# DTUWindEnergy/WindGym

Hardware: AMD Instinct MI355X
Metric: env-steps/sec (whole node), 16-turbine farm x 4096 envs (higher is better)
Workload: dtype f32

## Files before the change

### windgym_amd/build.py

```python
from __future__ import annotations

import glob
import os
import subprocess

HERE = os.path.dirname(os.path.abspath(__file__))
CSRC = os.path.join(HERE, "csrc")
LIB = os.path.join(HERE, "libwindgym_hip.so")
SOURCES = ["wg_flow.hip", "wg_env.hip", "wg_envb.hip", "wg_kernels.hip", "wg_api.hip", "wg_mann.hip", "wg_steady.hip", "wg_policy.hip", "wg_ppo.hip"]


def _headers():
    hs = sorted(glob.glob(os.path.join(CSRC, "*.h")) + glob.glob(os.path.join(CSRC, "*.inc")))
    return hs + [os.path.join(HERE, "..", "include", "windgym_hip.h")]


def needs_build() -> bool:
    if not os.path.exists(LIB):
        return True
    t = os.path.getmtime(LIB)
    return any(os.path.getmtime(f) > t for f in [os.path.join(CSRC, f) for f in SOURCES] + _headers())


def build(force: bool = False, verbose: bool = False, out: str | None = None) -> str:
    if out is None:
        if not force and not needs_build():
            return LIB
        out = LIB
    import tempfile
    hipcc = os.environ.get("HIPCC", "/opt/rocm/bin/hipcc")
    extra = os.environ.get("WG_HIPCC_FLAGS", "").split()
    flags = ["--offload-arch=gfx950", "-O3", "-std=c++17", "-fPIC"] + extra + ["-Wno-unused-result", "-Wno-unused-value"]
    if verbose:
        flags.insert(0, "-Rpass-analysis=kernel-resource-usage")
    with tempfile.TemporaryDirectory(prefix="wg_build_") as tmp:
        objs, procs = [], []
        for src in SOURCES:
            obj = os.path.join(tmp, src.replace(".hip", ".o"))
            cmd = [hipcc] + flags + ["-c", os.path.join(CSRC, src), "-o", obj]
            if verbose:
                print(" ".join(cmd))
            procs.append((cmd, subprocess.Popen(cmd)))
            objs.append(obj)
        for cmd, pr in procs:
            if pr.wait() != 0:
                for _, other in procs:
                    if other.poll() is None:
                        other.kill()
                raise subprocess.CalledProcessError(pr.returncode, cmd)
        subprocess.run([hipcc, "--offload-arch=gfx950", "-shared", "-fPIC", "-o", out] + objs + ["-lhipfft"], check=True)
    return out


if __name__ == "__main__":
    import argparse
    ap = argparse.ArgumentParser(description=__doc__)
    ap.add_argument("-v", action="store_true", help="print the compile commands and every kernel's resource usage")
    ap.add_argument("--out", metavar="PATH", help="write a variant library to PATH instead of the in-tree one")
    args = ap.parse_args()
    print(build(force=True, verbose=args.v, out=args.out))
```

### windgym_amd/csrc/wg_api.hip

```cpp
#include <hip/hip_runtime.h>

#include <algorithm>
#include <cmath>
#include <cstdio>
#include <cstdlib>
#include <cstring>
#include <memory>
#include <mutex>
#include <string>
#include <vector>

#include "wg_plan.h"
#include "wg_steady.h"
#include "wg_policy.h"
#include "wg_internal.h"

static const char* wg_hook(const char* name) {
    static const bool on = [] { const char* v = getenv("WG_DEBUG_HOOKS"); return v && v[0] == '1' && v[1] == 0; }();
    if (!on) return nullptr;
    const char* v = getenv(name);
    if (v) {
        static std::string seen;
        static std::mutex seen_mu;
        std::lock_guard<std::mutex> lock(seen_mu);
        const std::string tag = std::string(name) + "=" + v + ";";
        if (seen.find(tag) == std::string::npos) {
            seen += tag;
            fprintf(stderr, "[windgym] WG_DEBUG_HOOKS: %s=%s\n", name, v);
        }
    }
    return v;
}
static WgHooks wg_hooks_read() {
    WgHooks k;
    const auto num = [](const char* name) { WgHookInt r; if (const char* v = wg_hook(name)) { r.set = true; r.v = atoi(v); } return r; };
    k.flow_block = num("WG_FLOW_BLOCK"); k.flow_res = num("WG_FLOW_RES"); k.flow_env = num("WG_FLOW_ENV");
    k.env_wpe = num("WG_ENV_WPE"); k.env_split = num("WG_ENV_SPLIT"); k.step_fused = num("WG_STEP_FUSED");
    k.sums = num("WG_SUMS"); k.lds_pad = num("WG_LDS_PAD"); k.lf_cap = num("WG_LF_CAP"); k.pstride_pad = num("WG_PSTRIDE_PAD");
    k.step_graph = num("WG_STEP_GRAPH");
    k.first_obs_gl_only = wg_hook("WG_FIRST_OBS_GL_ONLY") != nullptr;
    k.no_box8 = wg_hook("WG_NO_BOX8") != nullptr;
    k.debug = wg_hook("WG_DEBUG") != nullptr;
    if (const char* v = wg_hook("WG_TIMELINE_OUT")) { k.timeline = true; k.timeline_out = v; }
    return k;
}

static thread_local std::string g_err;
static int fail(int code, const std::string& msg) {
    g_err = msg;
    return code;
}
extern "C" int wg_set_last_error_(int code, const char* msg) { return fail(code, msg ? msg : ""); }
#define HIPCHK(x)                                                                                   \
    do {                                                                                            \
        hipError_t _e = (x);                                                                        \
        if (_e != hipSuccess)                                                                       \
            return fail(WG_ERR_HIP, std::string(#x) + ": " + hipGetErrorString(_e));                \
    } while (0)

struct Alloc {
    void* ptr;
    size_t bytes;
};

struct wg_env_s {
    WgPlan plan;
    WgHooks hooks;
    WgParams p;
    WgPtrs d;
    FlowP fp;
    FlowPtrs fd;
    unsigned long long flow_steps_mark = 0, particles_mark = 0, added_mark = 0;
    double added_per_launch = 0.0;
    long n_step_launches = 0;
    void* box4 = nullptr;
    void* box4c = nullptr;
    int* box_ids_dev = nullptr;
    void* abox4 = nullptr;
    void* box8 = nullptr;
    void* abox8 = nullptr;
    double* wind_dev = nullptr;
    int device;
    std::vector<Alloc> allocs;
    std::vector<size_t> state_idx;
    uint8_t* mask_dev = nullptr;
    uint64_t* seeds_dev = nullptr;
    bool timing = false;
    int timing_period = 1, timing_phase = 0;
    std::vector<hipEvent_t> ev;
    std::vector<int> ev_kind;
    size_t ev_used = 0;
    struct StepGraph {
        const void* key[5];
        hipGraph_t graph;
        hipGraphExec_t exec;
        unsigned long long last_use;
    };
    std::vector<StepGraph> graphs;
    hipStream_t cap_stream = nullptr;
    int graph_mode = 0;
    unsigned long long graph_clock = 0;
    int* unready_dev = nullptr;
    WgParams* p_dev = nullptr;
    WgPtrs* d_dev = nullptr;
    float* flat_scratch = nullptr;
};

static const size_t WG_MAX_STEP_GRAPHS = 32;
static const size_t WG_MAX_TIMING_EVENTS = 4096;

static void drop_step_graphs(wg_env_s* h) {
    if (!h->graphs.empty()) { hipSetDevice(h->device); hipDeviceSynchronize(); }
    for (auto& g : h->graphs) {
        hipGraphExecDestroy(g.exec);
        hipGraphDestroy(g.graph);
    }
    h->graphs.clear();
}

static int sync_dev_params(wg_env_s* h) {
    hipError_t e = hipMemcpy(h->p_dev, &h->p, sizeof(WgParams), hipMemcpyHostToDevice);
    if (e == hipSuccess) e = hipMemcpy(h->d_dev, &h->d, sizeof(WgPtrs), hipMemcpyHostToDevice);
    if (e != hipSuccess) return fail(WG_ERR_HIP, std::string("hipMemcpy(params): ") + hipGetErrorString(e));
    return 0;
}

static int use_device(wg_env_s* h) {
    int cur = -1;
    if (hipGetDevice(&cur) != hipSuccess || cur != h->device) {
        hipError_t e = hipSetDevice(h->device);
        if (e != hipSuccess) return fail(WG_ERR_HIP, std::string("hipSetDevice: ") + hipGetErrorString(e));
    }
    return 0;
}

template <typename T>
static int dev_alloc(wg_env_s* h, T** out, size_t n, bool state, bool zero = true) {
    size_t bytes = sizeof(T) * (n ? n : 1);
    void* ptr = nullptr;
    hipError_t e = hipMalloc(&ptr, bytes);
    if (e != hipSuccess) return fail(WG_ERR_NOMEM, std::string("hipMalloc: ") + hipGetErrorString(e));
    if (zero) {
        e = hipMemset(ptr, 0, bytes);
        if (e != hipSuccess) return fail(WG_ERR_HIP, std::string("hipMemset: ") + hipGetErrorString(e));
    }
    h->allocs.push_back({ptr, bytes});
    if (state) h->state_idx.push_back(h->allocs.size() - 1);
    *out = (T*)ptr;
    return 0;
}
template <typename T, typename S>
static int dev_upload(wg_env_s* h, const T** out, const S* src, size_t n) {
    std::vector<T> tmp(n ? n : 1);
    for (size_t i = 0; i < n; ++i) tmp[i] = (T)src[i];
    T* p = nullptr;
    int rc = dev_alloc(h, &p, n, false, false);
    if (rc) return rc;
    HIPCHK(hipMemcpy(p, tmp.data(), sizeof(T) * (n ? n : 1), hipMemcpyHostToDevice));
    *out = p;
    return 0;
}

extern "C" const char* wg_last_error(void) { return g_err.c_str(); }
extern "C" int wg_abi_version(void) { return WG_ABI_VERSION; }

struct HandleGuard {
    void operator()(wg_env_s* h) const { wg_destroy(h); }
};

static int create_alloc(wg_env_s* h) {
    const WgParams& p = h->p;
    WgPtrs& d = h->d;
    const size_t n_slots = (size_t)p.B * 2 * p.F, n_ctx = (size_t)p.B * 2, pstride = (size_t)h->fp.pstride;
    int rc = 0;
#define A(field, n, st) if (!rc) rc = dev_alloc(h, &d.field, (n), (st))
    A(py, n_slots * pstride, true);
    if (p.turb_mode != WG_TURB_NONE) {
        A(pz, n_slots * pstride, true); A(vlp, n_slots * pstride, true); A(wlp, n_slots * pstride, true);
    }
    A(yaw, n_slots * p.N, true); A(u, n_slots * p.N, true); A(v, n_slots * p.N, true); A(w, n_slots * p.N, true);
    A(ti_loc, n_slots * p.N, true); A(power, n_slots * p.N, true); A(ct, n_slots * p.N, true);
    A(bnd, n_slots * p.N * 4, true);
    A(slot, n_slots, true); A(ctx, n_ctx, true); A(env, (size_t)p.B, true);
    A(xr, n_ctx * p.N, true); A(yr, n_ctx * p.N, true); A(jneed, n_ctx * p.N, true);
    A(roff, n_ctx * (p.N + 1), true); A(qown, n_ctx * (size_t)(p.NP / 4), true);
    A(ring, n_ctx * p.ring_stride, true); A(fring, n_ctx * p.fring_stride, true);
    A(cur_ws, n_ctx * p.N, true); A(cur_wd, n_ctx * p.N, true);
    A(pend_farm, n_ctx * p.power_avg, true); A(pend_base, n_ctx * p.power_avg, true);
    A(farm_pow, (size_t)p.B * p.power_avg, true); A(base_pow, (size_t)p.B * p.power_avg, true);
    A(old_yaw, (size_t)p.B * p.N, true);
    A(step_farm_pow, (size_t)p.B, true); A(step_base_pow, (size_t)p.B, true);
    A(last_pow_agent, (size_t)p.B, true); A(last_pow_base, (size_t)p.B, true);
    A(metrics, (size_t)p.B * WG_N_METRICS, true);
    if (h->plan.first_obs) { A(next_obs, n_ctx * (size_t)p.obs_dim, false); A(next_obs_ok, n_ctx, false); }
    if (p.sums_mode) A(wsum, n_ctx * WG_N_SUMS * (size_t)(p.N + 1), true);
    A(status, 1, true);
#undef A
    if (!rc) rc = dev_alloc(h, &h->mask_dev, (size_t)p.B, false);
    if (!rc) rc = dev_alloc(h, &h->seeds_dev, (size_t)p.B, false);
    if (!rc) rc = dev_alloc(h, &h->unready_dev, 1, false);
    if (!rc) rc = dev_alloc(h, &h->p_dev, 1, false);
    if (!rc) rc = dev_alloc(h, &h->d_dev, 1, false);
    return rc;
}

static int create_alloc_record(wg_env_s* h) {
    const size_t n = (size_t)h->p.B * 2 * h->p.F * (size_t)h->fp.pstride;
    if (h->fp.rec_il) {
        if (int rc = dev_alloc(h, &h->d.rec_a, 2 * n, true)) return rc;
        h->d.rec_b = h->d.rec_a + 1;
        return 0;
    }
    if (int rc = dev_alloc(h, &h->d.rec_a, n, true)) return rc;
    return dev_alloc(h, &h->d.rec_b, n, true);
}

static int create_upload(wg_env_s* h, const wg_config* c) {
    const WgParams& p = h->p;
    WgPtrs& d = h->d;
    int rc = dev_upload<double>(h, &d.x_pos, c->x_pos, p.N);
    if (!rc) rc = dev_upload<double>(h, &d.y_pos, c->y_pos, p.N);
    if (!rc && c->yaw_defined) rc = dev_upload<double>(h, &d.yaw_defined, c->yaw_defined, p.N);
    if (!rc) {
        const int kmax = std::max(p.N, 3);
        std::vector<uint64_t> jump((size_t)(kmax + 1) * 4);
        wg_u128 A = 1, G = 0;
        for (int k = 0; k <= kmax; ++k) {
            jump[4 * (size_t)k] = (uint64_t)A; jump[4 * (size_t)k + 1] = (uint64_t)(A >> 64);
            jump[4 * (size_t)k + 2] = (uint64_t)G; jump[4 * (size_t)k + 3] = (uint64_t)(G >> 64);
            A = A * WG_PCG_MULT; G = G * WG_PCG_MULT + 1;
        }
        rc = dev_upload<uint64_t>(h, &d.pcg_jump, jump.data(), jump.size());
    }
    if (!rc) rc = dev_upload<float>(h, &d.rotor_dy, c->rotor_dy, p.S);
    if (!rc) rc = dev_upload<float>(h, &d.rotor_dz, c->rotor_dz, p.S);
    if (!rc) rc = dev_upload<float>(h, &d.tab_ws, c->tab_ws, p.n_tab);
    if (!rc) rc = dev_upload<float>(h, &d.tab_power, c->tab_power, p.n_tab);
    if (!rc) rc = dev_upload<float>(h, &d.tab_ct, c->tab_ct, p.n_tab);
    if (!rc) rc = dev_upload<double>(h, &d.tab_ws_d, c->tab_ws, p.n_tab);
    if (!rc) rc = dev_upload<double>(h, &d.tab_power_d, c->tab_power, p.n_tab);
    if (rc) return rc;
    std::vector<float> pu, cu;
    double x0 = 0, dx = 0;
    wg_uniform_table(c, &pu, &cu, &x0, &dx);
    rc = dev_upload<float>(h, &h->fd.tab_power, pu.data(), pu.size());
    if (!rc) rc = dev_upload<float>(h, &h->fd.tab_ct, cu.data(), cu.size());
    return rc;
}

static void create_flow_ptrs(wg_env_s* h) {
    const WgPtrs& d = h->d;
    FlowPtrs& g = h->fd;
    g.py = d.py; g.rec_a = d.rec_a; g.rec_b = d.rec_b;
    g.pz = d.pz; g.vlp = d.vlp; g.wlp = d.wlp;
    g.bnd = d.bnd;
    g.yaw = d.yaw; g.u = d.u; g.v = d.v; g.w = d.w; g.ti_loc = d.ti_loc; g.power = d.power; g.ct = d.ct;
    g.slot = d.slot; g.ctx = d.ctx; g.env = d.env; g.xr = d.xr; g.yr = d.yr; g.jneed = d.jneed;
    g.ring = d.ring; g.fring = d.fring; g.cur_ws = d.cur_ws; g.cur_wd = d.cur_wd;
    g.pend_farm = d.pend_farm; g.pend_base = d.pend_base; g.old_yaw = d.old_yaw;
    g.step_farm_pow = d.step_farm_pow; g.step_base_pow = d.step_base_pow;
    g.rotor_dy = d.rotor_dy; g.rotor_dz = d.rotor_dz;
    g.gp = h->p_dev; g.gd = h->d_dev; g.env_rw = d.env;
    g.roff = d.roff; g.qown = d.qown; g.status = d.status;
}

static void apply_step_path(wg_env_s* h) {
    wg_plan_step_path(h->plan, h->fp.box_cells, (long long)h->fp.anx * h->fp.any * h->fp.anz, &h->fp.envw, &h->fp.env_fused);
}

extern "C" int wg_create(const wg_config* c, int device, wg_handle* out) {
    if (!c || !out) return fail(WG_ERR_INVALID, "null argument");
    std::string err;
    if (int rc = wg_validate_config(c, &err)) return fail(rc, err);
    HIPCHK(hipSetDevice(device));
    int lds_limit = 65536;
    {
        int v = 0;
        if (hipDeviceGetAttribute(&v, hipDeviceAttributeMaxSharedMemoryPerBlock, device) == hipSuccess && v > 0)
            lds_limit = std::min(v, 65536);
    }
    std::unique_ptr<wg_env_s, HandleGuard> owner(new wg_env_s());
    wg_env_s* h = owner.get();
    h->device = device;
    h->hooks = wg_hooks_read();
    if (int rc = wg_plan_create(c, h->hooks, lds_limit, &h->plan, &err)) return fail(rc, err);
    h->p = h->plan.p;
    h->fp = h->plan.f;
    apply_step_path(h);

    if (int rc = create_alloc(h)) return rc;
    if (int rc = create_upload(h, c)) return rc;
    if (int rc = create_alloc_record(h)) return rc;
    create_flow_ptrs(h);
    if (h->hooks.timeline) {
        long long* dbgp = nullptr;
        if (!dev_alloc(h, &dbgp, (size_t)h->p.B * 2 * h->p.F * 16, false)) h->fd.dbg = dbgp;
    }
    wg_launch_create(&h->p, &h->d, nullptr);
    if (sync_dev_params(h)) return WG_ERR_HIP;
    {
        hipError_t e = hipDeviceSynchronize();
        if (e == hipSuccess) e = hipStreamCreateWithFlags(&h->cap_stream, hipStreamNonBlocking);
        if (e != hipSuccess) return fail(WG_ERR_HIP, std::string("wg_create: ") + hipGetErrorString(e));
    }
    if (h->hooks.step_graph.set) h->graph_mode = h->hooks.step_graph.v != 0;
    if (h->hooks.debug) {
        const FlowP& f = h->fp;
        fprintf(stderr, "[windgym] k_flow variant: %s%s, %d threads, LDS %d B per workgroup, slot stride %d floats\n",
                f.envw ? (f.turb_mode == WG_TURB_NONE ? "compact rings / pair-major, one wave per env (k_flow_env)" : "compact rings / sample-major, one wave per env (k_flow_envb)")
                       : (f.res ? "compact rings / pair-major" : "uniform rings / sample-major"),
                f.envw && f.env_split ? " + a pass wave for the running episode's context" : "",
                f.block, f.envw ? f.env_lds : f.lds_bytes, f.pstride);
        fprintf(stderr, "[windgym] plan: res %d block %d gl %d rec_il %d target_chunk %d lf_cap %d lds_bytes %d | envw %d env_wpe %d env_split %d env_fused %d "
                        "env_lds %d env_off_tab %d | sums_mode %d first_obs %d reset_launches %d\n",
                f.res, f.block, f.gl, f.rec_il, f.target_chunk, f.lf_cap, f.lds_bytes, f.envw, f.env_wpe, f.env_split, f.env_fused, f.env_lds,
                f.env_off_tab, h->p.sums_mode, h->plan.first_obs, h->plan.reset_launches);
    }
    *out = owner.release();
    return 0;
}

extern "C" int wg_destroy(wg_handle h) {
    if (!h) return 0;
    hipSetDevice(h->device);
    hipDeviceSynchronize();
    if (h->fd.dbg && h->hooks.timeline) {
        const size_t n = (size_t)h->p.B * 2 * h->p.F * 16;
        std::vector<long long> host(n);
        if (hipMemcpy(host.data(), h->fd.dbg, n * sizeof(long long), hipMemcpyDeviceToHost) == hipSuccess) {
            if (FILE* f = fopen(h->hooks.timeline_out.c_str(), "wb")) { fwrite(host.data(), sizeof(long long), n, f); fclose(f); }
        }
    }
    drop_step_graphs(h);
    if (h->cap_stream) hipStreamDestroy(h->cap_stream);
    for (auto& e : h->ev) hipEventDestroy(e);
    for (auto& a : h->allocs) hipFree(a.ptr);
    if (h->box4) hipFree(h->box4);
    if (h->box4c) hipFree(h->box4c);
    if (h->abox4) hipFree(h->abox4);
    if (h->box8) hipFree(h->box8);
    if (h->abox8) hipFree(h->abox8);
    delete h;
    return 0;
}

extern "C" int wg_obs_dim(wg_handle h, int* obs_dim, int* obs_dim_multi) {
    if (!h) return fail(WG_ERR_INVALID, "null handle");
    if (obs_dim) *obs_dim = h->p.obs_dim;
    if (obs_dim_multi) *obs_dim_multi = h->p.obs_dim_multi;
    return 0;
}
extern "C" int wg_hist_max(wg_handle h, int* hist_max) {
    if (!h || !hist_max) return fail(WG_ERR_INVALID, "null argument");
    *hist_max = h->p.hist_max;
    return 0;
}

static int build_stencil_records(wg_env_s* h, void** owned, const float4** kernel_ptr, const void* box4, int n_boxes, int nx, int ny, int nz) {
    *kernel_ptr = nullptr;
    if (!(h->fp.envw && h->fp.turb_mode != WG_TURB_NONE)) return 0;
    const auto skip = [h](const char* why) {
        if (h->hooks.debug) fprintf(stderr, "[windgym] stencil records not built (%s): k_flow_envb reads the brick-ordered box\n", why);
        return 0;
    };
    if (wg_hooks_read().no_box8) return skip("WG_NO_BOX8");
    const size_t n_cells = (size_t)nx * ny * nz, bytes = n_cells * 128 * (size_t)n_boxes;
    size_t free_b = 0, total_b = 0;
    if (hipMemGetInfo(&free_b, &total_b) != hipSuccess) return skip("hipMemGetInfo failed");
    if (n_cells >= ((size_t)1 << 28)) return skip("a box of 2^28 cells or more");
    if (bytes > total_b / 4 || bytes > free_b / 2) return skip("the pool's records exceed a quarter of the device memory or half of what is free");
    if (hipMalloc(owned, bytes) != hipSuccess) { *owned = nullptr; (void)hipGetLastError(); return skip("hipMalloc failed"); }
    for (int k = 0; k < n_boxes; ++k)
        wg_launch_box_stencil((const char*)box4 + (size_t)k * n_cells * 16, (char*)*owned + (size_t)k * n_cells * 128, nx, ny, nz, nullptr);
    HIPCHK(hipDeviceSynchronize());
    *kernel_ptr = (const float4*)*owned;
    return 0;
}

extern "C" int wg_set_turbulence_boxes(wg_handle h, const float* const* boxes_dev, int n_boxes, int nx, int ny, int nz,
                                       double dx, double dy, double dz) {
    if (!h) return fail(WG_ERR_INVALID, "null handle");
    if (!boxes_dev || n_boxes < 1 || n_boxes > 64 || nx < 2 || ny < 2 || nz < 2 || !(dx > 0) || !(dy > 0) || !(dz > 0))
        return fail(WG_ERR_INVALID, "turbulence box: null pointer, bad pool size (1..64) or bad dimensions");
    for (int k = 0; k < n_boxes; ++k)
        if (!boxes_dev[k]) return fail(WG_ERR_INVALID, "turbulence box: null pointer in the pool");
    HIPCHK(hipSetDevice(h->device));
    HIPCHK(hipDeviceSynchronize());
    drop_step_graphs(h);
    h->d.box = nullptr; h->fd.box4 = nullptr; h->fd.box4c = nullptr; h->fd.box8 = nullptr; h->fp.coarse = 0;
    if (h->box8) { void* q = h->box8; h->box8 = nullptr; HIPCHK(hipFree(q)); }
    if (h->box4) { void* q = h->box4; h->box4 = nullptr; HIPCHK(hipFree(q)); }
    if (h->box4c) { void* q = h->box4c; h->box4c = nullptr; HIPCHK(hipFree(q)); }
    const size_t n_cells = (size_t)nx * ny * nz;
    HIPCHK(hipMalloc(&h->box4, n_cells * 16 * (size_t)n_boxes));
    for (int k = 0; k < n_boxes; ++k)
        wg_launch_box_repack(boxes_dev[k], (char*)h->box4 + (size_t)k * n_cells * 16, nx, ny, nz, nullptr);
    HIPCHK(hipDeviceSynchronize());
    h->d.box = boxes_dev[0];
    h->p.n_boxes = n_boxes;
    h->p.bnx = nx; h->p.bny = ny; h->p.bnz = nz; h->p.bdx = dx; h->p.bdy = dy; h->p.bdz = dz;
    h->fd.box4 = (const float4*)h->box4;
    h->fp.bnx = nx; h->fp.bny = ny; h->fp.bnz = nz; h->fp.box_cells = (long long)n_cells;
    apply_step_path(h);
    h->fp.box_pow2 = ((nx & (nx - 1)) == 0) && ((ny & (ny - 1)) == 0) && ((nz & (nz - 1)) == 0);
    h->fp.coarse = (nx % 4 == 0 && ny % 4 == 0 && nz % 4 == 0 && nx >= 8 && ny >= 8 && nz >= 8);
    h->fd.box4c = nullptr;
    if (h->fp.coarse) {
        const int cx = nx / 4, cy = ny / 4, cz = nz / 4;
        const size_t c_cells = (size_t)cx * cy * cz;
        HIPCHK(hipMalloc(&h->box4c, c_cells * 16 * (size_t)n_boxes));
        for (int k = 0; k < n_boxes; ++k)
            wg_launch_box_coarsen((const char*)h->box4 + (size_t)k * n_cells * 16, (char*)h->box4c + (size_t)k * c_cells * 16,
                                  nx, ny, nz, nullptr);
        HIPCHK(hipDeviceSynchronize());
        h->fp.cnx = cx; h->fp.cny = cy; h->fp.cnz = cz; h->fp.cbox_cells = (long long)c_cells;
        h->fp.cbox_pow2 = ((cx & (cx - 1)) == 0) && ((cy & (cy - 1)) == 0) && ((cz & (cz - 1)) == 0);
        h->fd.box4c = (const float4*)h->box4c;
    }
    h->fp.inv_bdx = 1.0 / dx; h->fp.inv_bdy = 1.0 / dy; h->fp.inv_bdz = 1.0 / dz;
    h->fp.inv_bn[0] = 1.0 / nx; h->fp.inv_bn[1] = 1.0 / ny; h->fp.inv_bn[2] = 1.0 / nz;
    if (int rc = build_stencil_records(h, &h->box8, &h->fd.box8, h->box4, n_boxes, nx, ny, nz)) return rc;
    return sync_dev_params(h);
}

extern "C" int wg_set_added_turbulence_box(wg_handle h, const float* box_dev, int nx, int ny, int nz, double dx,
                                           double dy, double dz) {
    if (!h || !box_dev || nx < 2 || ny < 2 || nz < 2 || !(dx > 0) || !(dy > 0) || !(dz > 0))
        return fail(WG_ERR_INVALID, "added-turbulence box: null pointer or bad dimensions");
    HIPCHK(hipSetDevice(h->device));
    HIPCHK(hipDeviceSynchronize());
    drop_step_graphs(h);
    h->fd.abox4 = nullptr; h->fd.abox8 = nullptr;
    if (h->abox8) { void* q = h->abox8; h->abox8 = nullptr; HIPCHK(hipFree(q)); }
    if (h->abox4) { void* q = h->abox4; h->abox4 = nullptr; HIPCHK(hipFree(q)); }
    const size_t n_cells = (size_t)nx * ny * nz;
    HIPCHK(hipMalloc(&h->abox4, n_cells * 16));
    wg_launch_box_repack(box_dev, h->abox4, nx, ny, nz, nullptr);
    HIPCHK(hipDeviceSynchronize());
    h->fd.abox4 = (const float4*)h->abox4;
    h->fp.anx = nx; h->fp.any = ny; h->fp.anz = nz;
    apply_step_path(h);
    h->fp.abox_pow2 = ((nx & (nx - 1)) == 0) && ((ny & (ny - 1)) == 0) && ((nz & (nz - 1)) == 0);
    h->fp.inv_adx = 1.0 / dx; h->fp.inv_ady = 1.0 / dy; h->fp.inv_adz = 1.0 / dz;
    h->fp.inv_an[0] = 1.0 / nx; h->fp.inv_an[1] = 1.0 / ny; h->fp.inv_an[2] = 1.0 / nz;
    if (int rc = build_stencil_records(h, &h->abox8, &h->fd.abox8, h->abox4, 1, nx, ny, nz)) return rc;
    return 0;
}

extern "C" int wg_set_deficit_table(wg_handle h, const float* table_dev, int n_ct, double ct0, double ct1, int n_ti, double ti0,
                                    double ti1, int n_x, double x_max_D, int n_r, double r_max_R) {
    if (!h || !table_dev || n_ct < 2 || n_ti < 2 || n_x < 2 || n_r < 2 || !(ct1 > ct0) || !(ti0 > 0) || !(ti1 > ti0) || !(x_max_D > 0) ||
        !(r_max_R > 0))
        return fail(WG_ERR_INVALID, "wg_set_deficit_table: null pointer or bad grid");
    if ((long long)n_ct * n_ti * n_x * n_r >= (1ll << 30)) return fail(WG_ERR_INVALID, "wg_set_deficit_table: table too large");
    HIPCHK(hipSetDevice(h->device));
    HIPCHK(hipDeviceSynchronize());
    drop_step_graphs(h);
    FlowP& f = h->fp;
    h->fd.dtab = table_dev;
    f.an_ct = n_ct; f.an_ti = n_ti; f.an_x = n_x; f.an_r = n_r;
    f.an_ct0 = (float)ct0; f.an_inv_dct = (float)((n_ct - 1) / (ct1 - ct0));
    f.an_lti0 = (float)std::log(ti0); f.an_inv_dlti = (float)((n_ti - 1) / (std::log(ti1) - std::log(ti0)));
    f.an_inv_dx = (float)((n_x - 1) / x_max_D); f.an_inv_dr = (float)((n_r - 1) / r_max_R);
    return 0;
}

extern "C" int wg_set_turbulence_box(wg_handle h, const float* box_dev, int nx, int ny, int nz, double dx,
                                     double dy, double dz) {
    const float* one[1] = {box_dev};
    if (!box_dev) return fail(WG_ERR_INVALID, "turbulence box: null pointer or bad dimensions");
    return wg_set_turbulence_boxes(h, one, 1, nx, ny, nz, dx, dy, dz);
}

extern "C" int wg_set_wind(wg_handle h, const double* wind_host) {
    if (!h) return fail(WG_ERR_INVALID, "null handle");
    HIPCHK(hipSetDevice(h->device));
    HIPCHK(hipDeviceSynchronize());
    drop_step_graphs(h);
    if (!wind_host) { h->d.wind_override = nullptr; return sync_dev_params(h); }
    if (!h->wind_dev) {
        double* w = nullptr;
        int rc = dev_alloc(h, &w, (size_t)h->p.B * 3, false);
        if (rc) return rc;
        h->wind_dev = w;
    }
    HIPCHK(hipMemcpy(h->wind_dev, wind_host, sizeof(double) * 3 * (size_t)h->p.B, hipMemcpyHostToDevice));
    h->d.wind_override = h->wind_dev;
    return sync_dev_params(h);
}

extern "C" int wg_set_box_ids(wg_handle h, const int32_t* ids_host) {
    if (!h) return fail(WG_ERR_INVALID, "null handle");
    HIPCHK(hipSetDevice(h->device));
    HIPCHK(hipDeviceSynchronize());
    drop_step_graphs(h);
    if (!ids_host) { h->d.box_override = nullptr; return sync_dev_params(h); }
    if (h->p.turb_mode != WG_TURB_BOX_POOL || h->p.n_boxes < 1)
        return fail(WG_ERR_INVALID, "wg_set_box_ids: the handle has no box pool (turb_mode WG_TURB_BOX_POOL + wg_set_turbulence_boxes first)");
    for (int b = 0; b < h->p.B; ++b)
        if (ids_host[b] >= h->p.n_boxes)
            return fail(WG_ERR_INVALID, "wg_set_box_ids: env " + std::to_string(b) + " asks for box " + std::to_string(ids_host[b]) +
                                            " of a pool of " + std::to_string(h->p.n_boxes));
    if (!h->box_ids_dev) {
        int* w = nullptr;
        int rc = dev_alloc(h, &w, (size_t)h->p.B, false);
        if (rc) return rc;
        h->box_ids_dev = w;
    }
    HIPCHK(hipMemcpy(h->box_ids_dev, ids_host, sizeof(int) * (size_t)h->p.B, hipMemcpyHostToDevice));
    h->d.box_override = h->box_ids_dev;
    return sync_dev_params(h);
}

extern "C" int wg_set_wind_device(wg_handle h, const double* wind_dev) {
    if (!h) return fail(WG_ERR_INVALID, "null handle");
    if (h->d.wind_override != wind_dev) drop_step_graphs(h);
    h->d.wind_override = wind_dev;
    if (int rc = use_device(h)) return rc;
    return sync_dev_params(h);
}

extern "C" int wg_set_flow_script(wg_handle h, const float* uvw_dev, const float* power_dev, int n_rows) {
    if (!h) return fail(WG_ERR_INVALID, "null handle");
    drop_step_graphs(h);
    h->d.script_uvw = uvw_dev;
    h->d.script_power = power_dev;
    h->p.script_rows = n_rows;
    h->fd.script_uvw = uvw_dev;
    h->fd.script_power = power_dev;
    h->fp.script_rows = n_rows;
    if (int rc = use_device(h)) return rc;
    return sync_dev_params(h);
}

static bool time_begin(wg_env_s* h, int kind, hipStream_t st) {
    if (!h->timing || h->ev_used + 2 > h->ev.size()) return false;
    h->ev_kind[h->ev_used / 2] = kind;
    hipEventRecord(h->ev[h->ev_used], st);
    return true;
}
static void time_end(wg_env_s* h, hipStream_t st) {
    hipEventRecord(h->ev[h->ev_used + 1], st);
    h->ev_used += 2;
}

extern "C" int wg_reset(wg_handle h, const uint8_t* env_mask_host, const uint64_t* seeds_host, float* obs_dev,
                        void* stream) {
    if (!h) return fail(WG_ERR_INVALID, "null handle");
    hipStream_t st = (hipStream_t)stream;
    HIPCHK(hipSetDevice(h->device));
    if (h->p.turb_mode >= WG_TURB_BOX && !h->d.box)
        return fail(WG_ERR_INVALID, "turbtype Mann*: call wg_set_turbulence_box before wg_reset");
    if (h->fp.added && !h->fd.abox4)
        return fail(WG_ERR_INVALID, "added_turbulence: call wg_set_added_turbulence_box before wg_reset");
    if (h->fp.deficit_model == 2 && !h->fd.dtab)
        return fail(WG_ERR_INVALID, "deficit_model 2: call wg_set_deficit_table before wg_reset");
    const uint8_t* mask = nullptr;
    const uint64_t* seeds = nullptr;
    bool all = true;
    if (env_mask_host) {
        for (int b = 0; b < h->p.B; ++b) all = all && env_mask_host[b] != 0;
        HIPCHK(hipMemcpyAsync(h->mask_dev, env_mask_host, (size_t)h->p.B, hipMemcpyHostToDevice, st));
        mask = h->mask_dev;
    }
    if (seeds_host) {
        HIPCHK(hipMemcpyAsync(h->seeds_dev, seeds_host, sizeof(uint64_t) * (size_t)h->p.B, hipMemcpyHostToDevice, st));
        seeds = h->seeds_dev;
    }
    if (all) HIPCHK(hipMemsetAsync(h->d.status, 0, sizeof(int), st));
    wg_launch_init(&h->p, &h->d, mask, seeds, st);
    const int n_plan = h->d.script_uvw ? ((h->p.K * (std::max(h->p.fill_a, h->p.fill_b) + 1)) / h->plan.reset_chunk + 2)
                                       : h->plan.reset_launches;
    long launched = 0;
    int batch = n_plan;
    for (;;) {
        for (int i = 0; i < batch; ++i) wg_launch_flow(&h->fp, &h->fd, WG_MODE_RESET, nullptr, mask, h->plan.reset_chunk, st);
        {
            const hipError_t le = hipGetLastError();
            if (le != hipSuccess) return fail(WG_ERR_HIP, std::string("wg_reset: k_flow launch failed: ") + hipGetErrorString(le));
        }
        launched += batch;
        int unready = 0;
        HIPCHK(hipMemsetAsync(h->unready_dev, 0, sizeof(int), st));
        wg_launch_unready(&h->p, &h->d, mask, h->unready_dev, st);
        HIPCHK(hipMemcpyAsync(&unready, h->unready_dev, sizeof(int), hipMemcpyDeviceToHost, st));
        HIPCHK(hipStreamSynchronize(st));
        if (unready == 0) break;
        if (launched > 4000000L / h->plan.reset_chunk)
            return fail(WG_ERR_STATE, "wg_reset: episode development does not terminate (wind speed override ~ 0?)");
        batch = std::max(8, n_plan / 4);
    }
    wg_launch_glue(&h->p, &h->d, 1, mask, obs_dev, nullptr, nullptr, nullptr, st, h->p_dev, h->d_dev);
    HIPCHK(hipGetLastError());
    return 0;
}

static bool count_step(wg_env_s* h) {
    h->n_step_launches++;
    return h->timing && (h->timing_phase++ % h->timing_period == 0);
}

static void launch_step(wg_env_s* h, const float* actions_dev, float* obs_dev, float* reward_dev, uint8_t* truncated_dev,
                        float* final_obs_dev, hipStream_t st, bool sample) {
    if (h->fp.env_fused && h->fd.script_uvw == nullptr) {
        if (sample) sample = time_begin(h, 0, st);
        if (h->fp.turb_mode == WG_TURB_NONE) wg_launch_step_env(&h->fp, &h->fd, &h->p, &h->d, actions_dev, obs_dev, reward_dev, truncated_dev, final_obs_dev, st);
        else wg_launch_step_envb(&h->fp, &h->fd, &h->p, &h->d, actions_dev, obs_dev, reward_dev, truncated_dev, final_obs_dev, st);
        if (sample) time_end(h, st);
        return;
    }
    if (sample) sample = time_begin(h, 0, st);
    wg_launch_flow(&h->fp, &h->fd, WG_MODE_STEP, actions_dev, nullptr, 0, st);
    if (sample) { time_end(h, st); sample = time_begin(h, 1, st); }
    wg_launch_glue(&h->p, &h->d, 0, nullptr, obs_dev, reward_dev, truncated_dev, final_obs_dev, st, h->p_dev, h->d_dev);
    if (sample) time_end(h, st);
}

extern "C" int wg_step(wg_handle h, const float* actions_dev, float* obs_dev, float* reward_dev,
// ... 448 lines not shown
```

### windgym_amd/csrc/wg_device.h

```cpp
#pragma once
#include <hip/hip_runtime.h>

#include "wg_state.h"

#define WG_PI_D 3.14159265358979323846
#define WG_DEG2RAD_F 0.017453292519943295f
#define WG_RAD2DEG_F 57.29577951308232f


__device__ inline uint32_t wg_ss_hashmix(uint32_t value, uint32_t& hc) {
    value ^= hc;
    hc *= 0x931e8875u;
    value *= hc;
    value ^= value >> 16;
    return value;
}
__device__ inline uint32_t wg_ss_mix(uint32_t x, uint32_t y) {
    uint32_t r = 0xca01f9ddu * x - 0x4973f715u * y;
    r ^= r >> 16;
    return r;
}
template <class R>
__device__ inline void wg_pcg_seed(R& e, uint64_t seed) {
    uint32_t ent[2] = {(uint32_t)(seed & 0xffffffffu), (uint32_t)(seed >> 32)};
    int n_ent = ent[1] != 0 ? 2 : 1;
    uint32_t pool[4];
    uint32_t hc = 0x43b0d7e5u;
    for (int i = 0; i < 4; ++i) pool[i] = wg_ss_hashmix(i < n_ent ? ent[i] : 0u, hc);
    for (int s = 0; s < 4; ++s)
        for (int dd = 0; dd < 4; ++dd)
            if (s != dd) pool[dd] = wg_ss_mix(pool[dd], wg_ss_hashmix(pool[s], hc));
    uint32_t hb = 0x8b51f9ddu;
    uint64_t st[4];
    for (int i = 0; i < 4; ++i) {
        uint32_t w2[2];
        for (int h = 0; h < 2; ++h) {
            uint32_t v = pool[(2 * i + h) & 3];
            v ^= hb;
            hb *= 0x58f38dedu;
            v *= hb;
            v ^= v >> 16;
            w2[h] = v;
        }
        st[i] = (uint64_t)w2[0] | ((uint64_t)w2[1] << 32);
    }
    wg_u128 initstate = ((wg_u128)st[0] << 64) | st[1];
    wg_u128 initseq = ((wg_u128)st[2] << 64) | st[3];
    e.rng_inc = (initseq << 1) | 1;
    e.rng_state = (wg_u128)0 * WG_PCG_MULT + e.rng_inc;
    e.rng_state += initstate;
    e.rng_state = e.rng_state * WG_PCG_MULT + e.rng_inc;
    e.rng_has32 = 0;
    e.rng_u32 = 0;
}
template <class R>
__device__ inline uint64_t wg_pcg_next64(R& e) {
    e.rng_state = e.rng_state * WG_PCG_MULT + e.rng_inc;
    uint64_t hi = (uint64_t)(e.rng_state >> 64), lo = (uint64_t)e.rng_state;
    uint64_t x = hi ^ lo;
    unsigned rot = (unsigned)(e.rng_state >> 122);
    return (x >> rot) | (x << ((-rot) & 63));
}
template <class R>
__device__ inline uint32_t wg_pcg_next32(R& e) {
    if (e.rng_has32) {
        e.rng_has32 = 0;
        return e.rng_u32;
    }
    uint64_t n = wg_pcg_next64(e);
    e.rng_has32 = 1;
    e.rng_u32 = (uint32_t)(n >> 32);
    return (uint32_t)(n & 0xffffffffu);
}
template <class R>
__device__ inline double wg_pcg_uniform(R& e, double low, double high) {
#pragma clang fp contract(off)
    const double u = (double)(wg_pcg_next64(e) >> 11) * (1.0 / 9007199254740992.0);
    const double scaled = (high - low) * u;
    return low + scaled;
}
template <class R>
__device__ inline uint32_t wg_pcg_integers(R& e, uint32_t high) {
    uint32_t rng = high - 1;
    if (rng == 0) return 0;
    uint32_t rng_excl = rng + 1;
    uint64_t m = (uint64_t)wg_pcg_next32(e) * (uint64_t)rng_excl;
    uint32_t leftover = (uint32_t)m;
    if (leftover < rng_excl) {
        uint32_t threshold = (0xffffffffu - rng) % rng_excl;
        while (leftover < threshold) {
            m = (uint64_t)wg_pcg_next32(e) * (uint64_t)rng_excl;
            leftover = (uint32_t)m;
        }
    }
    return (uint32_t)(m >> 32);
}

__device__ inline float wg_noise_normal(uint64_t key, uint32_t push_idx, uint32_t turbine, uint32_t channel,
                                        uint32_t episode) {
    uint32_t c0 = push_idx, c1 = turbine, c2 = channel, c3 = episode;
    uint32_t k0 = (uint32_t)key, k1 = (uint32_t)(key >> 32);
#pragma unroll
    for (int r = 0; r < 10; ++r) {
        uint64_t p0 = (uint64_t)0xD2511F53u * c0;
        uint64_t p1 = (uint64_t)0xCD9E8D57u * c2;
        uint32_t n0 = (uint32_t)(p1 >> 32) ^ c1 ^ k0;
        uint32_t n1 = (uint32_t)p1;
        uint32_t n2 = (uint32_t)(p0 >> 32) ^ c3 ^ k1;
        uint32_t n3 = (uint32_t)p0;
        c0 = n0; c1 = n1; c2 = n2; c3 = n3;
        k0 += 0x9E3779B9u;
        k1 += 0xBB67AE85u;
    }
    const float u1 = ((float)(c0 >> 8) + 1.0f) * (1.0f / 16777216.0f);
    const float u2 = (float)(c1 >> 8) * (1.0f / 16777216.0f);
    return sqrtf(-2.0f * __logf(u1)) * __cosf(6.2831853071795864f * u2);
}

__device__ inline void wg_philox_turb(uint32_t turb_seed, uint32_t c0, uint32_t c1, uint32_t c2, uint32_t c3,
                                      uint32_t& o0, uint32_t& o1) {
    uint32_t k0 = turb_seed, k1 = 0x57474d30u;
#pragma unroll
    for (int r = 0; r < 10; ++r) {
        uint64_t p0 = (uint64_t)0xD2511F53u * c0;
        uint64_t p1 = (uint64_t)0xCD9E8D57u * c2;
        uint32_t n0 = (uint32_t)(p1 >> 32) ^ c1 ^ k0;
        uint32_t n1 = (uint32_t)p1;
        uint32_t n2 = (uint32_t)(p0 >> 32) ^ c3 ^ k1;
        uint32_t n3 = (uint32_t)p0;
        c0 = n0; c1 = n1; c2 = n2; c3 = n3;
        k0 += 0x9E3779B9u;
        k1 += 0xBB67AE85u;
    }
    o0 = c0; o1 = c1;
}
__device__ inline float wg_turb_normal(uint32_t turb_seed, uint32_t step, uint32_t index, uint32_t comp, uint32_t kind) {
    uint32_t a, b;
    wg_philox_turb(turb_seed, step, index, comp, kind, a, b);
    const float u1 = ((float)(a >> 8) + 1.0f) * (1.0f / 16777216.0f);
    const float u2 = (float)(b >> 8) * (1.0f / 16777216.0f);
    return sqrtf(-2.0f * __logf(u1)) * __cosf(6.2831853071795864f * u2);
}

template <typename T>
__device__ inline T wg_tab_interp(const T* xs, const T* ys, int n, T x) {
    if (!(x >= xs[0]) || x > xs[n - 1]) return (T)0;
    int lo = 0, hi = n - 1;
    while (hi - lo > 1) {
        int mid = (lo + hi) >> 1;
        if (xs[mid] <= x) lo = mid; else hi = mid;
    }
    T f = (x - xs[lo]) / (xs[hi] - xs[lo]);
    return ys[lo] + f * (ys[hi] - ys[lo]);
}

template <class T>
__device__ inline T wg_tab_interp_wave(const T* xs, const T* ys, int n, T x, int lane) {
    int cnt = 0;
    for (int i0 = 0; i0 < n - 1; i0 += 64) {
        const int i = i0 + lane;
        const bool le = (i < n - 1) && (xs[i] <= x);
        cnt += __popcll(__ballot(le));
    }
    if (!(x >= xs[0]) || x > xs[n - 1]) return (T)0;
    const int lo = cnt - 1, hi = lo + 1;
    const T f = (x - xs[lo]) / (xs[hi] - xs[lo]);
    return ys[lo] + f * (ys[hi] - ys[lo]);
}

template <int CTRL>
__device__ __forceinline__ float wg_dpp_f(float v) {
    return __int_as_float(__builtin_amdgcn_update_dpp(0, __float_as_int(v), CTRL, 0xf, 0xf, true));
}
#define WG_ROW_REDUCE(v, OP)                                                 \
    v = OP(v, wg_dpp_f<0xB1>(v));                 \
    v = OP(v, wg_dpp_f<0x4E>(v));                 \
    v = OP(v, wg_dpp_f<0x141>(v));                    \
    v = OP(v, wg_dpp_f<0x140>(v));
__device__ __forceinline__ float wg_addf(float a, float b) { return a + b; }
__device__ inline float wg_row_sum(float v) {
    WG_ROW_REDUCE(v, wg_addf)
    return v;
}
__device__ inline float wg_wave_sum(float v) {
    WG_ROW_REDUCE(v, wg_addf)
    v += __shfl_xor(v, 16, 64);
    v += __shfl_xor(v, 32, 64);
    return v;
}
__device__ inline int wg_wave_sum_i(int v) {
#pragma unroll
    for (int o = 32; o > 0; o >>= 1) v += __shfl_xor(v, o, 64);
    return v;
}
template <int CTRL, int ROW_MASK>
__device__ __forceinline__ int wg_dpp_i(int v) {
    return __builtin_amdgcn_update_dpp(0, v, CTRL, ROW_MASK, 0xf, true);
}
__device__ __forceinline__ int wg_wave_scan_i(int v) {
    v += wg_dpp_i<0x111, 0xf>(v);
    v += wg_dpp_i<0x112, 0xf>(v);
    v += wg_dpp_i<0x114, 0xf>(v);
    v += wg_dpp_i<0x118, 0xf>(v);
    v += wg_dpp_i<0x142, 0xa>(v);
    v += wg_dpp_i<0x143, 0xc>(v);
    return v;
}
__device__ inline float wg_wave_max(float v) {
#pragma unroll
    for (int o = 32; o > 0; o >>= 1) v = fmaxf(v, __shfl_xor(v, o, 64));
    return v;
}
__device__ inline double wg_wave_min_d(double v) {
#pragma unroll
    for (int o = 32; o > 0; o >>= 1) v = fmin(v, __shfl_xor(v, o, 64));
    return v;
}
__device__ inline double wg_wave_max_d(double v) {
#pragma unroll
    for (int o = 32; o > 0; o >>= 1) v = fmax(v, __shfl_xor(v, o, 64));
    return v;
}

struct WgRng {
    wg_u128 rng_state, rng_inc;
    uint32_t rng_has32, rng_u32;
};

#ifdef WG_TIMELINE
__shared__ long long wg_stamps[20];
__shared__ int wg_counts[8];
#define WG_STAMP(k) do { if (threadIdx.x == 0) wg_stamps[k] = clock64(); } while (0)
#define WG_STAMP2(k) WG_STAMP(k)
#define WG_ICLK0() long long wg_iclk_ = clock64()
#define WG_ICLK(i) do { if (threadIdx.x == 0) { const long long c_ = clock64(); wg_counts[i] = (int)(c_ - wg_iclk_); wg_iclk_ = c_; } } while (0)
#else
#define WG_STAMP(k) do { } while (0)
#define WG_ICLK0() do { } while (0)
#define WG_ICLK(i) do { } while (0)
#endif

#ifndef WG_SHADOW_MARGIN
#define WG_SHADOW_MARGIN 2
#endif
__device__ inline int wg_shadow_share(const int work, long left, const int steps_done, const int e, const uint32_t phase = 0u) {
    if (work <= 0) return 0;
    left -= WG_SHADOW_MARGIN;
    if (left < 1) left = 1;
    const uint32_t phi24 = ((uint32_t)steps_done * 2654435769u + (uint32_t)e * 0x9E3779B1u + phase) >> 8;
    const float share = (float)work * __builtin_amdgcn_rcpf((float)left) + (float)phi24 * (1.0f / 16777216.0f);
    int it = (int)share;
    if (left == 1) it = work;
    return it > work ? work : it;
}

__device__ inline double wg_tab_interp_lanes(const double xs_l, const double ys_l, const int n, const double x, const int lane) {
    const int cnt = __popcll(__ballot((lane < n - 1) && (xs_l <= x)));
    const double x_first = __shfl(xs_l, 0, 64), x_last = __shfl(xs_l, n - 1, 64);
    const int lo = cnt > 0 ? cnt - 1 : 0, hi = lo + 1;
    const double xl = __shfl(xs_l, lo, 64), xh = __shfl(xs_l, hi, 64), yl = __shfl(ys_l, lo, 64), yh = __shfl(ys_l, hi, 64);
    if (!(x >= x_first) || x > x_last) return 0.0;
    const double f = (x - xl) / (xh - xl);
    return yl + f * (yh - yl);
}

template <class P, class D, class R>
__device__ inline void wg_ctx_init(const P& __restrict__ p, const D& __restrict__ d, R& rng, const int e, const int c, const int lane,
                                   const int episode_tag, const int f_lo, const int f_hi) {
    const int N = p.N, F = p.F;
    const int ctx_id = e * 2 + c;
    WgCtx& cx = d.ctx[ctx_id];
    WG_ICLK0();
    const int tl = lane < N ? lane : 0;
    const double xp_l = d.x_pos[tl], yp_l = d.y_pos[tl];
    const int n_tab = p.n_tab;
    const int il = lane < n_tab ? lane : n_tab - 1;
    const double tws_l = d.tab_ws_d[il], tpw_l = d.tab_power_d[il];
    const uint64_t* const jmp = d.pcg_jump;
    const int kmax = N > 3 ? N : 3;
    uint64_t jl[4], jn[4], j3[4];
    {
        const int kl = lane <= kmax ? lane : 0;
#pragma unroll
        for (int i = 0; i < 4; ++i) { jl[i] = jmp[4 * (size_t)kl + i]; jn[i] = jmp[4 * (size_t)N + i]; j3[i] = jmp[4 * (size_t)3 + i]; }
    }
    const bool yaw_rnd = p.yaw_init == WG_YAWINIT_RANDOM, yaw_def = p.yaw_init == WG_YAWINIT_DEFINED && p.has_yaw_defined;
    const double ydef_l = yaw_def ? d.yaw_defined[tl] : 0.0;
    double ov[3] = {0.0, 0.0, 0.0};
    const bool has_ov = d.wind_override != nullptr;
    if (has_ov) { ov[0] = d.wind_override[(size_t)e * 3]; ov[1] = d.wind_override[(size_t)e * 3 + 1]; ov[2] = d.wind_override[(size_t)e * 3 + 2]; }

    const wg_u128 inc = rng.rng_inc;
    auto ahead = [&](const uint64_t* j, const wg_u128 s) {
        const wg_u128 A = ((wg_u128)j[1] << 64) | j[0], G = ((wg_u128)j[3] << 64) | j[2];
        return A * s + G * inc;
    };
    auto draw = [&](const wg_u128 s, const double lo, const double hi) {
        struct { wg_u128 rng_state, rng_inc; } one{s, inc};
        return wg_pcg_uniform(one, lo, hi);
    };
    double ws, ti, wd;
    {
        const wg_u128 s_l = rng.rng_state;
        uint32_t iw[4] = {(uint32_t)s_l, (uint32_t)(s_l >> 32), (uint32_t)(s_l >> 64), (uint32_t)(s_l >> 96)};
#pragma unroll
        for (int i = 0; i < 4; ++i) iw[i] = (uint32_t)__shfl((int)iw[i], 0, 64);
        const wg_u128 s_in = ((wg_u128)iw[3] << 96) | ((wg_u128)iw[2] << 64) | ((wg_u128)iw[1] << 32) | (wg_u128)iw[0];
        const double lo = lane == 0 ? p.ws_min : lane == 1 ? p.ti_min : p.wd_min;
        const double hi = lane == 0 ? p.ws_max : lane == 1 ? p.ti_max : p.wd_max;
        const double u = draw(ahead(jl, s_in), lo, hi);
        ws = __shfl(u, 0, 64); ti = __shfl(u, 1, 64); wd = __shfl(u, 2, 64);
        if (lane == 0) rng.rng_state = ahead(j3, s_in);
    }
    if (has_ov) {
        if (ov[0] == ov[0]) ws = ov[0];
        if (ov[1] == ov[1]) wd = ov[1];
        if (ov[2] == ov[2]) ti = ov[2];
    }
    wg_u128 s_head = 0;
    if (lane == 0) {
        uint32_t tseed = 0;
        if (p.turb_mode == WG_TURB_RANDOM || p.turb_mode == WG_TURB_BOX_SHIFT)
            tseed = wg_pcg_integers(rng, 100000);
        cx.box_ox = 0.0; cx.box_oy = 0.0; cx.box_id = 0;
        if (p.turb_mode == WG_TURB_BOX_POOL) {
            const int fixed = d.box_override ? d.box_override[e] : -1;
            if (fixed >= 0) cx.box_id = fixed < p.n_boxes ? fixed : 0;
            else cx.box_id = (int)wg_pcg_integers(rng, (uint32_t)(p.n_boxes > 0 ? p.n_boxes : 1));
        }
        if (p.turb_mode == WG_TURB_BOX_SHIFT && p.bnx > 0) {
            if (p.n_boxes > 1) cx.box_id = (int)(tseed % (uint32_t)p.n_boxes);
            uint32_t a, b;
            wg_philox_turb(tseed, 0u, 0u, 0u, 0x4fu, a, b);
            cx.box_ox = (double)a * (1.0 / 4294967296.0) * p.bnx * p.bdx;
            cx.box_oy = (double)b * (1.0 / 4294967296.0) * p.bny * p.bdy;
        }
        s_head = rng.rng_state;
        cx.ws = ws; cx.ti = ti; cx.wd = wd; cx.turb_seed = tseed;
        if (f_lo == 0) { cx.n_pushed = 0; cx.pend_farm_n = 0; }
        if (f_hi == F) cx.pend_base_n = 0;
        cx.episode_tag = episode_tag;
    }
    {
        uint32_t sw[4] = {(uint32_t)s_head, (uint32_t)(s_head >> 32), (uint32_t)(s_head >> 64), (uint32_t)(s_head >> 96)};
#pragma unroll
        for (int i = 0; i < 4; ++i) sw[i] = (uint32_t)__shfl((int)sw[i], 0, 64);
        const wg_u128 s0 = ((wg_u128)sw[3] << 96) | ((wg_u128)sw[2] << 64) | ((wg_u128)sw[1] << 32) | (wg_u128)sw[0];
        const double ys = p.yaw_start;
        float* const yaw_c = d.yaw + (size_t)ctx_id * F * N;
        for (int t = lane; t < N; t += WG_WAVE) {
            float y0 = 0.f;
            if (yaw_rnd) {
                uint64_t jt[4];
                if (t < WG_WAVE) { jt[0] = jl[0]; jt[1] = jl[1]; jt[2] = jl[2]; jt[3] = jl[3]; }
                else { for (int i = 0; i < 4; ++i) jt[i] = jmp[4 * (size_t)t + i]; }
                y0 = (float)draw(ahead(jt, s0), -ys, ys);
            } else if (yaw_def) y0 = (float)(t < WG_WAVE ? ydef_l : d.yaw_defined[t]);
            for (int f = f_lo; f < f_hi; ++f) yaw_c[(size_t)f * N + t] = y0;
        }
        if (yaw_rnd && lane == 0) rng.rng_state = ahead(jn, s0);
    }
    WG_ICLK(5);
    {
        const double rp = n_tab <= WG_WAVE ? wg_tab_interp_lanes(tws_l, tpw_l, n_tab, ws, lane)
                                            : wg_tab_interp_wave<double>(d.tab_ws_d, d.tab_power_d, n_tab, ws, lane);
        if (lane == 0) cx.rated_power = (float)rp;
    }
    const double th = (270.0 - wd) * (WG_PI_D / 180.0);
    const double cth = cos(th), sth = sin(th);
    const double cx0 = p.cx0, cy0 = p.cy0;
    double* const xr_c = d.xr + (size_t)ctx_id * N;
    double* const yr_c = d.yr + (size_t)ctx_id * N;
    double xmin = 1e300, xmax = -1e300;
    for (int t = lane; t < N; t += WG_WAVE) {
        const double dx = (t < WG_WAVE ? xp_l : d.x_pos[t]) - cx0, dy = (t < WG_WAVE ? yp_l : d.y_pos[t]) - cy0;
        const double xr = cx0 + dx * cth + dy * sth;
        const double yr = cy0 - dx * sth + dy * cth;
        xr_c[t] = xr;
        yr_c[t] = yr;
        xmin = fmin(xmin, xr); xmax = fmax(xmax, xr);
    }
    xmin = wg_wave_min_d(xmin); xmax = wg_wave_max_d(xmax);
    const int P_ = p.P, full_chains = p.full_chains, compact = p.compact;
    const double dpart = p.dpart;
    int* const jneed_c = d.jneed + (size_t)ctx_id * N;
    int* const ro = d.roff + (size_t)ctx_id * (N + 1);
    uint8_t* const own = d.qown + (size_t)ctx_id * (p.NP >> 2);
    int base = 0;
    for (int t0 = 0; t0 < N; t0 += WG_WAVE) {
        const int t = t0 + lane;
        int len = 0;
        if (t < N) {
            const double dx = (t < WG_WAVE ? xp_l : d.x_pos[t]) - cx0, dy = (t < WG_WAVE ? yp_l : d.y_pos[t]) - cy0;
            const double dxm = xmax - (cx0 + dx * cth + dy * sth);
            const int jn_ = full_chains ? P_ : (int)(dxm / dpart) + 2;
            jneed_c[t] = jn_;
            len = (jn_ + 1 + 3) & ~3;
            if (len > P_) len = P_;
        }
        if (compact) {
            int incl = len;
#pragma unroll
            for (int o = 1; o < WG_WAVE; o <<= 1) {
                const int v = __shfl_up(incl, o, 64);
                if (lane >= o) incl += v;
            }
            if (t < N) {
                ro[t] = base + incl - len;
                const int q0 = (base + incl - len) >> 2, q1 = (base + incl) >> 2;
                for (int q = q0; q < q1; ++q) own[q] = (uint8_t)t;
            }
            base += __shfl(incl, WG_WAVE - 1, 64);
        }
    }
    if (compact && lane == 0) ro[N] = base;
    WG_ICLK(6);
    const bool scripted = d.script_uvw != nullptr;
    if (lane == 0) {
        cx.dist = xmax - xmin;
        const double t_inflow = (xmax - xmin) / ws;
        cx.t_inflow = t_inflow;
        const int t_developed = (int)(t_inflow * 2);
        cx.t_developed = t_developed;
        cx.time_max = p.never_truncate ? 9999999 : (int)(t_inflow * p.n_passthrough);
        int n_dev = (int)ceil((double)t_developed / p.dt_d - 1e-9);
        if (scripted) n_dev = 0;
        for (int f = f_lo; f < f_hi; ++f) {
            WgSlot& s = d.slot[ctx_id * F + f];
            s.head = P_ - 1; s.n_valid = 0; s.s_off = 0.0; s.time = 0.0; s.istep = 0; s.n_emitted = 0;
            s.dev_remaining = n_dev;
            s.fill_remaining = f == 0 ? p.fill_a : p.fill_b;
        }
    }
    for (int f = f_lo; f < f_hi; ++f) {
        const size_t tb = (size_t)(ctx_id * F + f) * N;
        const int cursor = scripted ? d.slot[ctx_id * F + f].cursor : 0;
        float* const u_ = d.u + tb; float* const v_ = d.v + tb; float* const w_ = d.w + tb;
        float* const ti_ = d.ti_loc + tb; float* const pw_ = d.power + tb; float* const ct_ = d.ct + tb;
        float4* const bnd_ = reinterpret_cast<float4*>(d.bnd) + tb;
        for (int t = lane; t < N; t += WG_WAVE) {
            float u = (float)ws, v = 0.f, w = 0.f, pw = 0.f;
            if (scripted) {
                int row = cursor < p.script_rows ? cursor : p.script_rows - 1;
                size_t sbase = (((size_t)f * p.script_rows + row) * p.B + e) * N;
                u = d.script_uvw[(sbase + t) * 3]; v = d.script_uvw[(sbase + t) * 3 + 1];
                w = d.script_uvw[(sbase + t) * 3 + 2]; pw = d.script_power[sbase + t];
            }
            u_[t] = u; v_[t] = v; w_[t] = w;
            ti_[t] = (float)ti; pw_[t] = pw; ct_[t] = 0.f;
            bnd_[t] = make_float4(0.f, 0.f, 0.f, 0.f);
        }
    }
    WG_ICLK(7);
}

struct WgRing {
    const float* data;
    int n_pushed, hlen;
    int n_avail, start;
    int stride, cap;
    __device__ WgRing() {}
    __device__ WgRing(const float* d_, int n_pushed_, int hlen_, int stride_, int cap_)
        : data(d_), n_pushed(n_pushed_), hlen(hlen_), stride(stride_), cap(cap_) {
        n_avail = n_pushed < hlen ? n_pushed : hlen;
        start = (n_pushed - n_avail) % cap;
    }
    __device__ int avail() const { return n_avail; }
    __device__ float at(int q) const {
        int phys = start + q;
        if (phys >= cap) phys -= cap;
        return data[phys * stride];
    }
};

__device__ inline float wg_ring_sum(const WgRing& r, const int lo, const int hi) {
    float s = 0.f;
    for (int q = lo; q < hi; q += 8) {
        float v[8];
#pragma unroll
        for (int k = 0; k < 8; ++k) v[k] = r.at(min(q + k, hi - 1));
#pragma unroll
        for (int k = 0; k < 8; ++k)
            if (q + k < hi) s += v[k];
    }
    return s;
}

__device__ inline float wg_scale(float v, float mn, float rng) {
    float t = v - mn;
    t = 2.0f * t;
    t = t / rng;
    return t - 1.0f;
}

__device__ inline int wg_mes_get(const wg_channel& c, bool cur_on, bool rol_on, const WgRing& r, float mn,
                                 float rng, float* out) {
    int n = 0;
    const int avail = r.avail();
    if (avail == 0) return 0;
    if (cur_on) out[n++] = wg_scale(r.at(avail - 1), mn, rng);
    if (rol_on) {
        const int W = c.window_len;
        for (int i = 0; i < c.history_n; ++i) {
            int lo, hi;
            if (i == 0) {
                lo = avail - W; if (lo < 0) lo = 0; hi = avail;
            } else if (i == c.history_n - 1 && avail >= W) {
                lo = 0; hi = W;
            } else if (avail < W) {
                lo = 0; hi = avail;
            } else {
                int spacing = (avail - W) / (c.history_n - 1);
                if (spacing < 1) spacing = 1;
                int pos = i * spacing;
                if (pos > avail - W) pos = avail - W;
                lo = pos; hi = pos + W;
            }
            const float s = wg_ring_sum(r, lo, hi);
            out[n++] = wg_scale(s / (float)(hi - lo), mn, rng);
        }
    }
    return n;
}

__device__ inline float wg_calc_ti(const WgRing& r) {
    const int avail = r.avail();
    float U = wg_ring_sum(r, 0, avail);
    U /= (float)avail;
    float m2 = 0.f;
    for (int q = 0; q < avail; q += 8) {
        float v[8];
#pragma unroll
        for (int k = 0; k < 8; ++k) v[k] = r.at(min(q + k, avail - 1));
#pragma unroll
        for (int k = 0; k < 8; ++k)
            if (q + k < avail) { const float dv = v[k] - U; m2 += dv * dv; }
    }
    return sqrtf(m2 / (float)avail) / U;
// ... 38 lines not shown
```

### windgym_amd/csrc/wg_env.hip

```cpp
#include <hip/hip_runtime.h>

#ifndef WG_ENV_ABLATE
#define WG_ENV_ABLATE 0
#endif
#include "wg_env_common.h"
#include "wg_internal.h"

struct __attribute__((aligned(16))) EnvSlotLds {
    int dev_rem, fill_rem, sub, budget;
    double s_new;
    int n_emit, n_valid, new_valid;
    unsigned n_emitted;
    float s_off_f, near_f, move_max, ti_pow;
    double s_off, ws;
    float ws_f, ti_f, wd_env, base_acc;
    int n_pushed, pend_farm_n, pend_base_n, n_flow;
    double c_time;
    int c_head;
    unsigned c_part, c_flow, c_istep, c_tag, n_emitted0;
    float out_pw;
    unsigned c_add;
    int bg_init;
    int pad_[3];
};
static_assert(sizeof(EnvSlotLds) == WG_ENV_SLOT_LDS_BYTES, "keep WG_ENV_SLOT_LDS_BYTES in sync (wg_flow.h)");
#define WG_ENV_OFF_SRC4 0
#define WG_ENV_OFF_REC4 1024
#define WG_ENV_OFF_RING 2048
#define WG_ENV_OFF_XR 3072
#define WG_ENV_OFF_SRC2 3584
#define WG_ENV_OFF_SL 4096
#define WG_ENV_OFF_HDR (WG_ENV_OFF_SL + 4 * WG_ENV_SLOT_LDS_BYTES)
#define WG_ENV_OFF_STAGE (WG_ENV_OFF_HDR + 128)
static_assert(WG_ENV_OFF_STAGE == WG_ENV_FIXED_LDS_BYTES, "keep WG_ENV_FIXED_LDS_BYTES in sync (wg_flow.h)");

__device__ __forceinline__ float env_slot_sums(const float v, const int N, const int NS, const int k, const int tid) {
    if (N == 16) return wg_row_sum(v);
    if (N < 16) {
        const int r = tid >> 4, i = tid & 15;
        const float x = __shfl(v, (r * N + i) & 63, 64);
        const float s = wg_row_sum((i < N && r < NS) ? x : 0.f);
        return __shfl(s, k << 4, 64);
    }
    const int h = tid >> 5, i = tid & 31;
    const float x = __shfl(v, (h * N + i) & 63, 64);
    float s = (i < N && h < NS) ? x : 0.f;
    WG_ROW_REDUCE(s, wg_addf)
    s += __shfl_xor(s, 16, 64);
    return __shfl(s, k << 5, 64);
}

template <bool NOISE, int WPE, int GLUE, int SPLIT>
__device__ __forceinline__ void env_flow(char* const smem, char* const smem_pass, float* const zone, const int wv, const int role, const int mode,
                                         const float* __restrict__ actions, const uint8_t* __restrict__ mask, const int chunk, EnvFlowOut& out) {
    const int tid = threadIdx.x & 63, e = blockIdx.x;
    int N, F, NS, NL;
    float inv_N;
    {
        const KArgsPtr ka = wg_cold_args();
        N = ka->p.N; F = ka->p.F; inv_N = ka->p.inv_N;
        NS = WPE == 2 ? F : 2 * F; NL = NS * N;
    }
    const int kbase = WPE == 2 ? wv * F : 0;
    const bool valid = tid < NL;
    const int g = valid ? tid : 0;
    const int k = (int)(((float)g + 0.5f) * inv_N);
    const int t = g - k * N;
    const int c = WPE == 2 ? wv : (F == 2 ? (k >> 1) : k), farm = F == 2 ? (k & 1) : 0;

    float4* const Lsrc4 = reinterpret_cast<float4*>(smem + WG_ENV_OFF_SRC4);
    uint4* const Lrec4 = reinterpret_cast<uint4*>(smem + WG_ENV_OFF_REC4);
    int4* const Lring = reinterpret_cast<int4*>(smem + WG_ENV_OFF_RING);
    double* const Lxr = reinterpret_cast<double*>(smem + WG_ENV_OFF_XR);
    float2* const Lsrc2 = reinterpret_cast<float2*>(smem + WG_ENV_OFF_SRC2);
    EnvSlotLds* const SL = reinterpret_cast<EnvSlotLds*>(smem + WG_ENV_OFF_SL);
    float* const def = reinterpret_cast<float*>(smem + WG_ENV_OFF_STAGE);
    float* const tiav = def + WG_ENV_CAP;
    unsigned short* const cl = reinterpret_cast<unsigned short*>(tiav + WG_ENV_CAP);
    unsigned short* const ql = reinterpret_cast<unsigned short*>(smem + WG_ENV_OFF_STAGE);
    EnvSlotLds& my = SL[k];

    WG_STAMP(0);
    typedef const __attribute__((address_space(4))) WgEnv* CEnvPtr;
    int env_live;
    bool role_live = false, role_dev = false, defer_init = false, split_on = false;
    float yaw, tu, tti, oyaw;
    {
        const KArgsPtr k0 = wg_cold_args();
        static_assert(sizeof(WgEnv) == 128, "the env header is loaded as 32 words");
        const int hw = reinterpret_cast<const int*>(k0->d.env + e)[tid & 31];
        if (GLUE != 0 && tid < 32) reinterpret_cast<int*>(smem + WG_ENV_OFF_HDR)[tid] = hw;
        out.bg_init_pending = 0; out.rounds = 0; out.first_obs = 0;
        const bool use_mask = mode == WG_MODE_RESET && mask != nullptr;
        const uint8_t mask_byte = *(use_mask ? mask + e : reinterpret_cast<const uint8_t*>(k0->d.env + e));
        const bool masked_out = use_mask && mask_byte == 0;
        const unsigned ctx_id = (unsigned)(e * 2 + c), slot_id = (unsigned)(e * 2 * F + kbase + k);
        const unsigned tb = (unsigned)((e * 2 * F + kbase) * N + g);
        const unsigned tcx = ctx_id * (unsigned)N + (unsigned)t;

        int dev_rem, fill_rem, n_pushed, pend_farm_n, pend_base_n, init_pending, time_max_c, n_valid, c_head;
        unsigned n_emitted, c_part, c_flow, c_istep, c_tag, c_add;
        double s_off, ws, l_xr, l_yr, c_time;
        float ti_f, wd_env, l_yaw, l_u, l_ti, l_act;
        float4 l_bnd;
        int l_roff, l_rnext;
        auto load_state = [&]() __attribute__((always_inline)) {
            const KArgsPtr kl = wg_cold_args();
            const WgSlot& slot = kl->d.slot[slot_id];
            const WgCtx& cx = kl->d.ctx[ctx_id];
            dev_rem = slot.dev_remaining; fill_rem = slot.fill_remaining;
            s_off = slot.s_off; c_time = slot.time; c_head = slot.head; n_valid = slot.n_valid; c_istep = slot.istep;
            n_emitted = slot.n_emitted; c_part = slot.part_count; c_flow = slot.flow_count; c_add = slot.add_count;
            ws = cx.ws; ti_f = (float)cx.ti; wd_env = (float)cx.wd;
            n_pushed = cx.n_pushed; pend_farm_n = cx.pend_farm_n; pend_base_n = cx.pend_base_n;
            c_tag = (unsigned)cx.episode_tag; init_pending = cx.init_pending; time_max_c = cx.time_max;
            const int* ro = kl->d.roff + ctx_id * (unsigned)(N + 1);
            l_roff = ro[(unsigned)t]; l_rnext = ro[(unsigned)t + 1u];
            l_xr = kl->d.xr[tcx]; l_yr = kl->d.yr[tcx];
            l_yaw = kl->d.yaw[tb]; l_u = kl->d.u[tb]; l_ti = kl->d.ti_loc[tb];
            l_bnd = reinterpret_cast<const float4*>(kl->d.bnd)[tb];
        };
        load_state();
        const int n_tab = k0->p.n_tab, S = k0->p.S;
        const unsigned i_tab = (unsigned)min(tid, n_tab - 1), i_s = (unsigned)min(tid, S - 1);
        const float pf_tp = k0->d.tab_power[i_tab], pf_tc = k0->d.tab_ct[i_tab];
        const float pf_dy = k0->d.rotor_dy[i_s], pf_dz = k0->d.rotor_dz[i_s];
        {
            const bool has_act = mode == WG_MODE_STEP && farm == 0;
            const float a = *(has_act ? actions + (unsigned)(e * N + t) : k0->d.tab_ct);
            l_act = has_act ? a : 0.f;
        }

#define WG_HDR_I(f) __builtin_amdgcn_readlane(hw, (int)(offsetof(WgEnv, f) / 4))
        env_live = WG_HDR_I(live);
        int env_done = WG_HDR_I(done), env_shadow_iters = WG_HDR_I(shadow_iters), env_steps_done = WG_HDR_I(steps_done);
        int env_timestep = WG_HDR_I(timestep), env_time_max_live = WG_HDR_I(time_max_live);
#undef WG_HDR_I
        if (SPLIT && role == 1) {
            if (tid == 0) { *reinterpret_cast<int*>(smem + WG_ENV_OFF_HDR) = 0; if (GLUE != 0 && (SPLIT == 1 || wv == 0)) reinterpret_cast<int*>(zone)[LEAN_PRE_FLAG] = 0; }
            asm volatile("s_waitcnt vmcnt(0) lgkmcnt(0)" ::: "memory");
        }
        if (WPE == 2) {
            asm volatile("" : "+s"(env_live), "+s"(env_done), "+s"(env_shadow_iters), "+s"(env_steps_done), "+s"(env_timestep), "+s"(env_time_max_live) : : "memory");
            asm volatile("s_barrier" ::: "memory");
        }
        if (SPLIT && role == 1 && GLUE != 0 && c == env_live) {
            const EnvKArgsPtr kz = (EnvKArgsPtr)wg_cold_args();
            const WgParams& zp = *(const WgParams*)&kz->gp;
            const WgPtrs& zd = *(const WgPtrs*)&kz->gd;
#define WG_HDR_Z(f) __builtin_amdgcn_readlane(hw, (int)(offsetof(WgEnv, f) / 4))
            const int z_np = WG_HDR_Z(n_pushed_live), z_fn = WG_HDR_Z(farm_pow_n), z_bn = WG_HDR_Z(base_pow_n);
#undef WG_HDR_Z
            const int PA = zp.power_avg;
            const SumsRaw zr = wg_sums_load<false, false>(zp, zd, e, e * 2 + env_live, tid < N ? tid : 0, z_np);
            const float z_fo = zd.farm_pow[(size_t)e * PA + z_fn % PA];
            const float z_bo = F == 2 ? zd.base_pow[(size_t)e * PA + z_bn % PA] : 0.f;
            const float z_met = tid < WG_N_METRICS ? zd.metrics[(size_t)e * WG_N_METRICS + tid] : 0.f;
            double* const zs = reinterpret_cast<double*>(zone);
#pragma unroll
            for (int sI = 0; sI < WG_N_CH; ++sI) { zs[LEAN_PRE_S(sI, tid)] = zr.S[sI]; zone[LEAN_PRE_LV(sI, tid)] = zr.lv[sI]; }
            zone[LEAN_PRE_MET(tid)] = z_met;
            if (tid == 0) { zone[LEAN_PRE_FOLD] = z_fo; zone[LEAN_PRE_BOLD] = z_bo; }
            asm volatile("s_waitcnt lgkmcnt(0)" ::: "memory");
            if (tid == 0) env_flag_set(reinterpret_cast<int*>(zone) + LEAN_PRE_FLAG);
        }
        out.env_live = env_live;
        out.truncates = env_timestep >= env_time_max_live;
        out.steps_done = env_steps_done; out.time_max_live = env_time_max_live;

        const bool is_live_c = (c == env_live);
        const int autoreset = k0->p.autoreset;
        int budget = 0;
        if (mode == WG_MODE_STEP) {
            role_live = is_live_c && !env_done;
            role_dev = !is_live_c && autoreset != 0;
            const int bg_pending = WPE == 2 ? (is_live_c ? 0 : __shfl(init_pending, 0, 64)) : __shfl(init_pending, (env_live ^ 1) * F * N, 64);
            out.bg_init_pending = autoreset && bg_pending;
            if (SPLIT == 2 && role == 1 && out.bg_init_pending) return;
            if (autoreset && bg_pending && WPE == 1 && !out.truncates) {
                defer_init = true;
                budget = 0;
            } else if (autoreset && bg_pending) {
                const KArgsPtr ki = wg_cold_args();
                const WgParams& gp = *ki->d.gp;
                env_init_episode<GLUE != 0>(e, env_live ^ 1, tid);
                full_barrier<64>();
                load_state();
                const int fill_max = F == 2 ? max(gp.fill_a, gp.fill_b) : gp.fill_a;
                const int inc = 1 + (gp.extra_inc ? 1 : 0);
                const int tm = WPE == 2 ? ki->d.ctx[e * 2 + env_live].time_max : __shfl(time_max_c, env_live * F * N, 64);
                const long total = (long)((tm + inc - 1) / inc) + 1;
                const int dev0 = __shfl(dev_rem, WPE == 2 ? 0 : (env_live ^ 1) * F * N, 64);
                budget = wg_shadow_share(dev0 + gp.K * fill_max, total - env_steps_done, env_steps_done, e);
                budget = wg_shadow_share(dev_rem + gp.K * fill_rem, total - env_steps_done, env_steps_done, e, farm ? 0x80000000u : 0u);
            } else {
                const int inc = k0->p.env_inc;
                const long total = (long)((env_time_max_live + inc - 1) / inc) + 1;
                budget = role_dev ? wg_shadow_share(dev_rem + k0->p.K * fill_rem, total - env_steps_done, env_steps_done, e, farm ? 0x80000000u : 0u) : 0;
            }
        } else {
            role_dev = is_live_c && !masked_out;
            budget = chunk;
        }
        if (SPLIT) {
            const bool two = valid && role_dev && budget >= 2;
            split_on = mode == WG_MODE_STEP && k0->p.K == 1 && (is_live_c || (SPLIT == 2 && !out.bg_init_pending)) && !defer_init && !__ballot(two);
            if (role == 1 && !split_on) return;
        }
        if (WPE == 2 && valid && t == 0) {
            my.dev_rem = dev_rem; my.fill_rem = fill_rem; my.bg_init = out.bg_init_pending; my.n_flow = 0; my.out_pw = 0.f;
        }
        {
            const bool any_work = valid && (role_live || (role_dev && budget > 0 && (dev_rem > 0 || fill_rem > 0)));
            if (!__ballot(any_work)) {
                if (WPE == 2 && mode == WG_MODE_STEP && !is_live_c && autoreset && role == 0) {
                    const int d0 = __shfl(dev_rem, 0, 64), f0 = __shfl(fill_rem, 0, 64), np0 = __shfl(n_pushed, 0, 64);
                    const KArgsPtr kf = wg_cold_args();
                    if (d0 == 0 && f0 == 0 && kf->d.gd->next_obs_ok != nullptr && kf->d.gd->next_obs_ok[ctx_id] == 0) {
                        out.first_obs = 1;
                        env_first_obs<GLUE != 0>((int)ctx_id, np0, tid);
                    }
                }
                return;
            }
        }

        const KArgsPtr k1 = wg_cold_args();
        const int rlen = l_rnext - l_roff;
        const int head = n_emitted == 0u ? rlen - 1 : fast_mod((int)(n_emitted - 1u), rlen, __builtin_amdgcn_rcpf((float)rlen));
        const float ws_f = (float)ws;
        if (valid) {
            Lxr[g] = l_xr;
            Lsrc4[g] = make_float4((float)l_xr, (float)l_yr, l_bnd.y, l_bnd.z);
            Lsrc2[g] = make_float2(l_bnd.x, l_bnd.w);
            Lring[g] = make_int4(l_roff, rlen, head, k);
            Lrec4[g] = make_uint4(0u, 0u, 0u, __float_as_uint(1.f));
            if (t == 0) {
                my.dev_rem = dev_rem; my.fill_rem = fill_rem; my.sub = 0; my.budget = budget;
                my.n_valid = n_valid; my.n_emitted = n_emitted; my.n_emitted0 = n_emitted;
                my.move_max = fabsf(k1->p.hill) * ws_f * k1->p.dt; my.ti_pow = fast_pow(ti_f, k1->p.tic);
                my.s_off = s_off; my.ws = ws; my.ws_f = ws_f; my.ti_f = ti_f; my.wd_env = wd_env; my.base_acc = 0.f;
                my.n_pushed = n_pushed; my.pend_farm_n = pend_farm_n; my.pend_base_n = pend_base_n; my.n_flow = 0;
                my.bg_init = out.bg_init_pending;
                my.c_time = c_time; my.c_head = c_head; my.c_part = c_part; my.c_flow = c_flow; my.c_istep = c_istep; my.c_tag = c_tag; my.c_add = c_add;
            }
        }
        float* const tabp = reinterpret_cast<float*>(smem + k1->p.env_off_tab);
        float* const tabct = tabp + n_tab;
        float2* const rpt = reinterpret_cast<float2*>(tabct + n_tab);
        const float hub = k1->p.hub;
        auto rp = [&](const float dy_, const float dz_) __attribute__((always_inline)) {
            const float dz = hub + dz_ - hub;
            return make_float2(dy_, dz * dz);
        };
        if (tid < n_tab) { tabp[tid] = pf_tp; tabct[tid] = pf_tc; }
        if (tid < S) rpt[tid] = rp(pf_dy, pf_dz);
        for (int i = tid + 64; i < n_tab; i += 64) { tabp[i] = k1->d.tab_power[i]; tabct[i] = k1->d.tab_ct[i]; }
        for (int i = tid + 64; i < S; i += 64) rpt[i] = rp(k1->d.rotor_dy[i], k1->d.rotor_dz[i]);

        yaw = l_yaw; tu = l_u; tti = l_ti; oyaw = l_yaw;
        if (role_live && farm == 0 && valid) {
            const float a = l_act, ymin = k1->p.yaw_min, ymax = k1->p.yaw_max, ystep = k1->p.yaw_step;
            if (k1->p.action_method == WG_ACT_YAW) {
                yaw = fminf(fmaxf(yaw + a * ystep, ymin), ymax);
            } else {
                float tf = a + 1.0f;
                tf = tf * 0.5f;
                tf = tf * (ymax - ymin);
                tf = tf + ymin;
                const float ny = fminf(fmaxf(tf, yaw - ystep), yaw + ystep);
                yaw = fminf(fmaxf(ny, ymin), ymax);
            }
        }
    }
    float tpow = 0.f, tct = 0.f, cg = 1.f;
    float sws = 0.f, swd = 0.f, syaw = 0.f, sp_ = 0.f;
    int part_acc = 0, stream_acc = 0;
    bool stepped = false;
    lds_barrier<64>();
    WG_STAMP(1);

    for (int round = 0;; ++round) {
        bool stepping, is_dev;
        int sub, K;
        {
            const KArgsPtr kr = wg_cold_args();
            K = kr->p.K;
            const int4 sch = *reinterpret_cast<const int4*>(&my.dev_rem);
            const bool active = sch.x > 0 || sch.y > 0;
            stepping = valid && (role_live ? (round < K) : (role_dev && active && (sch.w > 0 || sch.z != 0)));
            is_dev = !role_live && sch.x > 0;
            sub = sch.z;
            if (!__ballot(stepping)) break;
        out.rounds = round + 1;
            if (round > 0) full_barrier<64>();

            if (role_live && farm == 1 && stepping) {
                const float ystep = kr->p.yaw_step;
                if (kr->p.base_controller == WG_CTRL_LOCAL) {
                    const float off = 0.f - yaw;
                    const float sgn = (float)((off > 0.f) - (off < 0.f));
                    yaw = yaw + sgn * fminf(fabsf(off), ystep);
                } else {
                    const float sgn = (float)((yaw > 0.f) - (yaw < 0.f));
                    yaw = yaw - sgn * fminf(fabsf(yaw), ystep);
                }
            }

            if (stepping && t == 0) {
                const double dpart = kr->p.dpart;
                const int P = kr->p.P;
                const double s_off = my.s_off, adv = my.ws * kr->p.dt_d;
                double s_new = s_off + adv;
                int n_emit = 0;
                while (s_new >= dpart) { s_new -= dpart; ++n_emit; }
                if (n_emit > P) n_emit = P;
                int new_valid = my.n_valid + n_emit; if (new_valid > P) new_valid = P;
                my.s_new = s_new; my.n_emit = n_emit; my.new_valid = new_valid;
                my.s_off_f = (float)s_off;
                my.near_f = (float)(s_off + adv + dpart) + 0.01f;
            }
        }
        lds_barrier<64>();
        WG_STAMP(4);

        unsigned cmask = 0u;
        {
            const KArgsPtr kp = wg_cold_args();
            const float D = kp->p.D, inv_D = kp->p.inv_D, eps_max = kp->p.env_eps_max;
            const int gs0 = k * N;
            const float lim0 = kp->p.R_rot + 1.0e-3f * D;
            const float near_f = my.near_f, move_max = my.move_max;
            const float xt_f = Lsrc4[g].x, yt_f = Lsrc4[g].y;
#pragma unroll 4
            for (int s2 = 0; s2 < N; ++s2) {
                const float4 a = Lsrc4[gs0 + s2];
                const float2 b = Lsrc2[gs0 + s2];
                const float dxf = xt_f - a.x;
                const bool nearp = dxf < near_f;
                const float kb_ = nearp ? fmaxf(WG_K_MAX, a.z) : a.z, eb_ = nearp ? fmaxf(eps_max, a.w) : a.w;
                const float sig_max = (kb_ * (dxf * inv_D) + eb_) * D;
                const float bdv = b.x + (((__float_as_uint(b.y) != 0u) | nearp) ? move_max : 0.f);
                const float gap = fabsf(yt_f - a.y) - (5.0f * sig_max + bdv);
                const bool cd = (s2 != t) & (dxf >= 0.f) & (gap <= lim0);
                cmask |= cd ? (1u << s2) : 0u;
            }
            if (!stepping || (SPLIT && role == 1)) cmask = 0u;
        }
        int cbeg, nc;
        {
            const int cnt = __popc(cmask);
            const int inc = wg_wave_scan_i(cnt);
            cbeg = inc - cnt;
            nc = __builtin_amdgcn_readlane(inc, 63);
            unsigned m = cmask;
            int o = cbeg;
            while (m) { cl[o++] = (unsigned short)((g << 5) | __builtin_ctz(m)); m &= m - 1u; }
        }
        lds_barrier<64>();
        WG_STAMP(5);

        struct Cand { uint2 q0, q1; float y0, y1, xd, wgt; int en, jp0; bool ok, rest; };
        float dsum = 0.f, tia_max = 0.f;
        {
            const KArgsPtr kp = wg_cold_args();
            const unsigned pstride = (unsigned)kp->p.pstride;
            const size_t pb_env = (size_t)(e * 2 * F + kbase) * pstride;
            const uint2* const rc_env = reinterpret_cast<const uint2*>(kp->d.rec_a + 2 * pb_env);
            const float* const py_env = kp->d.py + pb_env;
            const double inv_dpart = kp->p.inv_dpart;
            const float inv_D = kp->p.inv_D;
            auto issue = [&](Cand& cd, const int cidx, const int c0, const int c1) __attribute__((always_inline)) {
                cd.ok = false; cd.rest = false;
                if (cidx >= c1) return;
                def[cidx - c0] = 0.f; tiav[cidx - c0] = 0.f;
                const unsigned en = cl[cidx];
                cd.en = (int)en;
                const int gt = (int)(en >> 5);
                const int4 rt = Lring[gt];
                const int gs = rt.w * N + (int)(en & 31u);
                const EnvSlotLds& q = SL[rt.w];
                const double dx = Lxr[gt] - Lxr[gs];
                if (!(dx > 0.0)) return;
                cd.xd = (float)dx * inv_D;
                const double xi = (dx - q.s_new) * inv_dpart;
                const double jf = floor(xi);
                cd.wgt = (float)(xi - jf);
                int j = (int)jf;
                if (j < 0) { j = 0; cd.wgt = 0.f; }
                if (j + 1 > q.new_valid - 1) return;
                const int4 rg = Lring[gs];
                const int Rs = rg.y, hd = rg.z;
                const unsigned mv = __float_as_uint(Lsrc2[gs].y);
                cd.rest = !(mv != 0u && (int)(q.n_emitted - mv) < Rs);
                cd.jp0 = j - q.n_emit;
                int r0 = hd - cd.jp0; if (r0 < 0) r0 += Rs;
                int r1 = hd - cd.jp0 - 1; if (r1 < 0) r1 += Rs;
                if (cd.jp0 < 0) r0 = 0;
                if (cd.jp0 + 1 < 0) r1 = 0;
                const unsigned sb = (unsigned)rg.w * pstride + (unsigned)rg.x;
                cd.q0 = rc_env[sb + (unsigned)r0]; cd.q1 = rc_env[sb + (unsigned)r1];
                cd.y0 = 0.f; cd.y1 = 0.f;
                if (!cd.rest) { cd.y0 = py_env[sb + (unsigned)r0]; cd.y1 = py_env[sb + (unsigned)r1]; }
#if WG_ENV_ABLATE & 1
                cd.q0 = make_uint2(Lrec4[gs].x, Lrec4[gs].y); cd.q1 = cd.q0; cd.y0 = cd.y1 = Lsrc4[gs].y;
#endif
                cd.ok = true;
            };
            Cand ca, cb_;
            issue(ca, tid, 0, min(nc, WG_ENV_CAP));
            WG_STAMP(11);

            if (stepping) {
                const KArgsPtr kq = wg_cold_args();
                const int n_tab = kq->p.n_tab;
                const float* const tabct = reinterpret_cast<const float*>(smem + kq->p.env_off_tab) + n_tab;
                const float gy = yaw * WG_DEG2RAD_F;
                const float sg = __sinf(gy);
                cg = __cosf(gy);
                const float wsn = fmaxf(tu * cg, 0.0f);
                const float ctx = fminf(fmaxf(env_tab(tabct, kq->p.tab_x0, kq->p.tab_inv_dx, n_tab, wsn) * cg * cg, 0.0f), 0.96f);
                const float rq = __builtin_amdgcn_sqrtf(1.0f - ctx);
                const float beta = 0.5f * (1.0f + rq) * __builtin_amdgcn_rcpf(rq);
                const float rk = kq->p.ka * tti + kq->p.kb;
                const float reps = kq->p.eps0 * __builtin_amdgcn_sqrtf(beta);
                const float rhv = -kq->p.hill * sg * tu;
                if (rk > WG_K_MAX || fabsf(rhv) > WG_HV_MAX) atomicOr(kq->d.status, WG_STATUS_BIT_RANGE);
                const unsigned na_ = pack_a(ctx, rk), nb_ = pack_b(tu * __builtin_amdgcn_rcpf(kq->p.ue_scale * my.ws_f), rhv);
                float4 s4 = Lsrc4[g];
                s4.z = fmaxf(s4.z, rk + WG_K_MAX / 65535.0f);
                s4.w = fmaxf(s4.w, reps + 1.0f / 65535.0f);
                Lsrc4[g] = s4;
                const int n_emit = my.n_emit;
                if (n_emit > 0 && rec_moves(nb_)) Lsrc2[g].y = __uint_as_float(my.n_emitted + (unsigned)n_emit);
                Lrec4[g] = make_uint4(na_, nb_, __float_as_uint(tu), __float_as_uint(cg));
            }
            lds_barrier<64>();
            WG_STAMP(2);

            const KArgsPtr ke2 = wg_cold_args();
            const float dpart_f = ke2->p.dpart_f, D = ke2->p.D, dt = ke2->p.dt, R_rot = ke2->p.R_rot, eps0 = ke2->p.eps0, ue_scale = ke2->p.ue_scale;
            const float tia = ke2->p.no_ti_fold ? 0.f : ke2->p.tia, tib = ke2->p.tib, tid_ = ke2->p.tid, inv_S = ke2->p.inv_S;
            const int S = ke2->p.S;
            const float2* const rpt = reinterpret_cast<const float2*>(smem + ke2->p.env_off_tab + 8 * ke2->p.n_tab);
            auto eval_cand = [&](const Cand& cd, const int pos) __attribute__((always_inline)) {
                    if (!cd.ok) return;
#ifdef WG_TIMELINE
                    atomicAdd(&wg_counts[1], 1);
#endif
                    const int gt = cd.en >> 5;
                    const int kt = Lring[gt].w;
                    const int gs = kt * N + (cd.en & 31);
                    const float4 st = Lsrc4[gt];
                    const float ysrc = Lsrc4[gs].y;
                    const EnvSlotLds& q = SL[kt];
                    const int jp0 = cd.jp0, jp1 = jp0 + 1;
                    float py0 = cd.rest ? ysrc : cd.y0, py1 = cd.rest ? ysrc : cd.y1;
                    unsigned a0 = cd.q0.x, b0_ = cd.q0.y, a1 = cd.q1.x, b1_ = cd.q1.y;
                    if (jp0 < 0) {
                        const uint4 rn = Lrec4[gs];
                        py0 = ysrc; a0 = rn.x; b0_ = rn.y;
                        if (jp1 < 0) { py1 = ysrc; a1 = rn.x; b1_ = rn.y; }
                    }
                    const float ue_max = ue_scale * q.ws_f;
                    const float u0 = rec_uf(b0_) * ue_max, u1 = rec_uf(b1_) * ue_max;
                    {
                        const int nv = q.n_valid;
                        const float sof = q.s_off_f;
                        if (!cd.rest && jp0 >= 0 && jp0 < nv) py0 = m0_advect(py0, a0, b0_, jp0, sof, dpart_f, inv_D, dt, eps0);
                        if (!cd.rest && jp1 >= 0 && jp1 < nv) py1 = m0_advect(py1, a1, b1_, jp1, sof, dpart_f, inv_D, dt, eps0);
                    }
                    const float wgt = cd.wgt;
                    const float w0 = 1.0f - wgt, w1 = wgt;
                    const float yc = w0 * py0 + w1 * py1;
                    const float kv = w0 * rec_k(a0) + w1 * rec_k(a1);
                    const float epv = w0 * rec_eps(a0, eps0) + w1 * rec_eps(a1, eps0);
                    const float xd = cd.xd;
                    const float sp = kv * xd + epv;
                    const float sig = sp * D;
                    const float yt = st.y;
                    const float rc2 = (yt - yc) * (yt - yc);
                    const float rcut = R_rot + 5.0f * sig;
                    if (rc2 > rcut * rcut) return;
#ifdef WG_TIMELINE
                    atomicAdd(&wg_counts[2], 1);
                    if (rc2 <= (R_rot + 3.0f * sig) * (R_rot + 3.0f * sig)) atomicAdd(&wg_counts[3], 1);
#endif
                    const float ctv = w0 * rec_ct(a0) + w1 * rec_ct(a1);
                    const float uev = w0 * u0 + w1 * u1;
                    const float inv2s2 = __builtin_amdgcn_rcpf(2.0f * sig * sig);
                    const float cf = m0_cfrac(ctv, sp);
                    const float ind = 0.5f * (1.0f - __builtin_amdgcn_sqrtf(1.0f - ctv));
                    tiav[pos] = tia * fast_pow(ind, tib) * q.ti_pow * fast_pow(fmaxf(xd, 1.0f), tid_) * __expf(-rc2 * inv2s2);
                    const float cgt = __uint_as_float(Lrec4[gt].w), amp = uev * cf;
                    const float ninv = -inv2s2;
                    float acc = 0.f;
#pragma unroll 4
                    for (int sI = 0; sI < ((WG_ENV_ABLATE & 8) ? 1 : S); ++sI) {
                        const float2 rp = rpt[sI];
                        const float dy = yt + rp.x * cgt - yc;
                        acc += amp * __expf((dy * dy + rp.y) * ninv);
                    }
                    def[pos] = acc * inv_S;
            };
#ifdef WG_TIMELINE
            if (tid == 0) atomicAdd(&wg_counts[0], nc);
#endif
            for (int c0 = 0; c0 < nc; c0 += WG_ENV_CAP) {
                const int c1 = min(nc, c0 + WG_ENV_CAP);
                if (c0 > 0) { lds_barrier<64>(); issue(ca, c0 + tid, c0, c1); }
                for (int cb = c0; cb < c1; cb += 64) {
                    cb_ = ca;
                    issue(ca, cb + 64 + tid, c0, c1);
                    eval_cand(cb_, cb - c0 + tid);
                }
                lds_barrier<64>();
                if (stepping) {
                    const int b0 = max(cbeg, c0), b1 = min(cbeg + __popc(cmask), c1);
                    for (int cc = b0; cc < b1; ++cc) {
                        dsum += def[cc - c0];
                        tia_max = fmaxf(tia_max, tiav[cc - c0]);
                    }
                }
            }
        }
        if (SPLIT && split_on && role == 0) {
            __builtin_amdgcn_s_waitcnt(0x0070);
            if (tid == 0) env_flag_set(reinterpret_cast<int*>(smem_pass + WG_ENV_OFF_HDR));
            if (stepping) {
                const int4 rg = Lring[g];
                const unsigned mvl = __float_as_uint(Lsrc2[g].y);
                const int n_emit = my.n_emit;
                const bool full = (mvl != 0u && (int)(my.n_emitted - mvl) < rg.y) || n_emit >= 4 || n_emit >= rg.y;
                stream_acc += full ? rg.y : n_emit;
            }
        }
        if (stepping) {
            const float ti_f = my.ti_f;
            tu = my.ws_f;
            tu -= dsum;
            tti = __builtin_amdgcn_sqrtf(ti_f * ti_f + tia_max * tia_max);
        }
        lds_barrier<64>();
        WG_STAMP(9);

        if (!(SPLIT && split_on && role == 0)) {
            const KArgsPtr kp = wg_cold_args();
            const unsigned pstride = (unsigned)kp->p.pstride;
            const size_t pb_env = (size_t)(e * 2 * F + kbase) * pstride;
            float* const py_env = kp->d.py + pb_env;
            unsigned* const ra_env = kp->d.rec_a + 2 * pb_env;
            int nlist;
            {
                int cnt = 0, nqd = 0;
                bool full = false;
                if (stepping) {
                    const int4 rg = Lring[g];
                    const int rlen = rg.y, n_emit = my.n_emit;
                    const unsigned mvl = __float_as_uint(Lsrc2[g].y);
                    nqd = rlen >> 2;
                    const bool moving = mvl != 0u && (int)(my.n_emitted - mvl) < rlen;
                    full = moving || n_emit >= 4 || n_emit >= rlen;
                    stream_acc += full ? rlen : n_emit;
                    if (full) cnt = nqd;
                    else if (n_emit > 0) {
                        const unsigned sb = (unsigned)k * pstride + (unsigned)rg.x;
                        const uint4 rn = Lrec4[g];
                        const float y0 = Lsrc4[g].y;
#pragma unroll
                        for (int em = 0; em < 3; ++em) {
                            if (em < n_emit) {
                                int r = rg.z + 1 + em; if (r >= rlen) r -= rlen;
                                const unsigned ix = sb + (unsigned)r;
                                py_env[ix] = y0;
                                reinterpret_cast<uint2*>(ra_env)[ix] = make_uint2(rn.x, rn.y);
                            }
                        }
                    }
                }
                const int inc = wg_wave_scan_i(cnt);
                nlist = (WG_ENV_ABLATE & 2) ? 0 : __builtin_amdgcn_readlane(inc, 63);
                if (full) {
                    const int base = inc - cnt;
                    const unsigned tag = (unsigned)g << 10;
                    for (int i = 0; i < nqd; ++i) ql[base + i] = (unsigned short)(tag | (unsigned)i);
                }
            }
            lds_barrier<64>();
            WG_STAMP(10);
#ifdef WG_TIMELINE
            if (tid == 0) atomicAdd(&wg_counts[4], nlist);
#endif

            const float dpart_f = kp->p.dpart_f, inv_D = kp->p.inv_D, dt = kp->p.dt, eps0 = kp->p.eps0;
            struct QuadReq { float4 py; uint4 ra, rb; int g, kq; unsigned q; };
            auto request = [&](QuadReq& r, const int cidx) __attribute__((always_inline)) {
                const bool v = cidx < nlist;
                const unsigned en = v ? ql[cidx] : 0u;
                r.g = (int)(en >> 10); r.kq = (int)(en & 1023u);
                const int4 rg = Lring[r.g];
                r.q = (((unsigned)rg.w * pstride + (unsigned)rg.x) >> 2) + (unsigned)r.kq;
                if (v) {
                    r.py = reinterpret_cast<const float4*>(py_env)[r.q];
                    r.ra = reinterpret_cast<const uint4*>(ra_env)[2u * r.q];
                    r.rb = reinterpret_cast<const uint4*>(ra_env)[2u * r.q + 1u];
                }
            };
            auto advect_quad = [&](const QuadReq& cur, const int cidx) __attribute__((always_inline)) {
                if (cidx >= nlist) return;
                const int gq = cur.g, kq = cur.kq;
                const unsigned q = cur.q;
                const int4 rg = Lring[gq];
                const EnvSlotLds& sl = SL[rg.w];
                const int n_emit_q = sl.n_emit, n_valid_q = sl.n_valid;
                const float sof = sl.s_off_f;
                const int R = rg.y, hd = rg.z;
                const int r0 = 4 * kq;
                int j0 = hd - r0; if (j0 < 0) j0 += R;
                int e0 = r0 - hd - 1; if (e0 < 0) e0 += R;
                const bool emits = (e0 < n_emit_q) || (n_emit_q > 0 && e0 + 3 >= R);
                float pyv[4] = {cur.py.x, cur.py.y, cur.py.z, cur.py.w};
                unsigned rav[4] = {cur.ra.x, cur.ra.z, cur.rb.x, cur.rb.z};
                unsigned rbv[4] = {cur.ra.y, cur.ra.w, cur.rb.y, cur.rb.w};
#pragma unroll
                for (int i = 0; i < 4; ++i) {
                    int j = j0 - i; if (j < 0) j += R;
                    const float adv = m0_advect(pyv[i], rav[i], rbv[i], j, sof, dpart_f, inv_D, dt, eps0);
                    pyv[i] = j < n_valid_q ? adv : pyv[i];
                }
                const float y0 = Lsrc4[gq].y;
                if (emits) {
                    const uint4 rn = Lrec4[gq];
#pragma unroll
                    for (int i = 0; i < 4; ++i) {
                        int ei = e0 + i; if (ei >= R) ei -= R;
                        if (ei < n_emit_q) {
                            pyv[i] = y0; rav[i] = rn.x; rbv[i] = rn.y;
                        }
                    }
                    reinterpret_cast<uint4*>(ra_env)[2u * q] = make_uint4(rav[0], rbv[0], rav[1], rbv[1]);
                    reinterpret_cast<uint4*>(ra_env)[2u * q + 1u] = make_uint4(rav[2], rbv[2], rav[3], rbv[3]);
                }
                reinterpret_cast<float4*>(py_env)[q] = make_float4(pyv[0], pyv[1], pyv[2], pyv[3]);
                float ex = 0.f;
#pragma unroll
                for (int i = 0; i < 4; ++i) {
                    int j = j0 - i; if (j < 0) j += R;
                    if (j < n_valid_q) ex = fmaxf(ex, fabsf(pyv[i] - y0));
                }
                if (ex > Lsrc2[gq].x) atomicMax(reinterpret_cast<int*>(&Lsrc2[gq].x), __float_as_int(ex));
            };
            QuadReq qa, qb;
            qa.py = qb.py = make_float4(0.f, 0.f, 0.f, 0.f); qa.ra = qa.rb = qb.ra = qb.rb = make_uint4(0u, 0u, 0u, 0u);
            request(qa, tid);
            if (SPLIT && role == 1) {
                if (!env_flag_wait(reinterpret_cast<int*>(smem + WG_ENV_OFF_HDR))) atomicOr(kp->d.status, WG_STATUS_BIT_STATE);
            }
            for (int base = 0; base < nlist; base += 64) {
                qb = qa;
                request(qa, base + 64 + tid);
                advect_quad(qb, base + tid);
            }
        }
        lds_barrier<64>();
        WG_STAMP(3);
        if (SPLIT && role == 1) {
            if (stepping) reinterpret_cast<float4*>(wg_cold_args()->d.bnd)[(unsigned)((e * 2 * F + kbase) * N + g)].x = Lsrc2[g].x;
            return;
        }

        const bool measuring = stepping && !is_dev;
        const bool unit_end = measuring && (sub + 1 == K);
        const KArgsPtr kc = wg_cold_args();
        const float inv_k = 1.0f / (float)K;
        const unsigned ctx_id = (unsigned)(e * 2 + c);
        if (stepping) {
            {
                int4 rg = Lring[g];
                const int n_emit = my.n_emit;
                rg.z += n_emit;
                if (n_emit >= rg.y) rg.z %= rg.y; else if (rg.z >= rg.y) rg.z -= rg.y;
                Lring[g].z = rg.z;
                part_acc += min(my.new_valid, rg.y);
            }
            stepped = true;
            const int n_tab = kc->p.n_tab;
            const float tab_x0 = kc->p.tab_x0, tab_inv_dx = kc->p.tab_inv_dx;
            const float* const tabp = reinterpret_cast<const float*>(smem + kc->p.env_off_tab);
            const float wsn = fmaxf(tu * cg, 0.0f);
            tpow = env_tab(tabp, tab_x0, tab_inv_dx, n_tab, wsn);
            tct = env_tab(tabp + n_tab, tab_x0, tab_inv_dx, n_tab, wsn) * cg * cg;
            if (measuring && farm == 0) {
                const float wsm = __builtin_amdgcn_sqrtf(tu * tu);
                const float wdm = 0.f + my.wd_env;
                float val[WG_N_CH] = {sws + wsm, swd + wdm, syaw + yaw, sp_ + tpow};
                if (unit_end) {
                    const int n_pushed = my.n_pushed;
                    const unsigned tcx = ctx_id * (unsigned)N + (unsigned)t;
                    kc->d.cur_ws[tcx] = wsm;
                    kc->d.cur_wd[tcx] = wdm;
                    if (K != 1) {
#pragma unroll
                        for (int ch = 0; ch < WG_N_CH; ++ch) val[ch] *= inv_k;
                    }
                    if (NOISE) {
                        const uint64_t noise_key = ((CEnvPtr)(kc->d.env + e))->noise_key;
                        const uint32_t episode_tag = my.c_tag;
#pragma unroll
                        for (int ch = 0; ch < WG_N_CH; ++ch)
                            if (kc->p.noise_sigma[ch] != 0.f)
                                val[ch] += kc->p.noise_sigma[ch] * wg_noise_normal(noise_key, (uint32_t)n_pushed, (uint32_t)t,
                                                                                   (uint32_t)ch, episode_tag);
                    }
                    float* __restrict__ rbase = kc->d.ring + (size_t)ctx_id * kc->p.ring_stride;
#pragma unroll
                    for (int ch = 0; ch < WG_N_CH; ++ch) {
                        const int H = kc->p.hlen[ch];
                        rbase[(unsigned)(kc->p.ring_off[ch] + fast_mod(n_pushed, H, kc->p.inv_hlen[ch]) * N + t)] = val[ch];
                    }
                    if (SPLIT) {
#pragma unroll
                        for (int ch = 0; ch < WG_N_CH; ++ch) out.g_nw[ch] = val[ch];
                    }
                    sws = val[0]; swd = val[1]; sp_ = val[3];
                } else {
                    sws = val[0]; swd = val[1]; syaw = val[2]; sp_ = val[3];
                }
            }
        }
        float a_ws = 0.f, a_wd = 0.f, a_pw = 0.f;
        if (__ballot(measuring)) {
            a_ws = env_slot_sums((measuring && farm == 0) ? sws : 0.f, N, NS, k, tid);
            a_wd = env_slot_sums((measuring && farm == 0) ? swd : 0.f, N, NS, k, tid);
            a_pw = env_slot_sums(measuring ? (farm == 0 ? sp_ : tpow) : 0.f, N, NS, k, tid);
        }
        if (stepping && t == 0) {
            const int n_emit = my.n_emit;
            my.n_valid = my.new_valid; my.s_off = my.s_new; my.n_emitted += (unsigned)n_emit;
            my.n_flow += 1; my.budget -= 1;
            float base_acc = my.base_acc;
            if (measuring && farm == 1) base_acc += a_pw;
            if (unit_end) {
                const FlowP __attribute__((address_space(4)))& pc = kc->p;
                if (farm == 0) {
                    const int n_pushed = my.n_pushed, pend_farm_n = my.pend_farm_n;
                    float* fbase = kc->d.fring + (size_t)ctx_id * pc.fring_stride;
                    fbase[pc.fring_off[WG_CH_WS] + umod_small(n_pushed, pc.hlen[WG_CH_WS], pc.hmagic[WG_CH_WS])] = a_ws * pc.inv_N;
                    fbase[pc.fring_off[WG_CH_WD] + umod_small(n_pushed, pc.hlen[WG_CH_WD], pc.hmagic[WG_CH_WD])] = a_wd * pc.inv_N;
                    fbase[pc.fring_off[WG_CH_POWER] + umod_small(n_pushed, pc.hlen[WG_CH_POWER], pc.hmagic[WG_CH_POWER])] = a_pw;
                    my.out_pw = a_pw;
                    if (role_live) kc->d.step_farm_pow[e] = a_pw;
                    else {
                        kc->d.pend_farm[(size_t)ctx_id * pc.power_avg + umod_small(pend_farm_n, pc.power_avg, pc.pavg_magic)] = a_pw;
                        my.pend_farm_n = pend_farm_n + 1;
                    }
                    my.n_pushed = n_pushed + 1;
                } else {
                    const float bp = K == 1 ? base_acc : base_acc * inv_k;
                    my.out_pw = bp;
                    if (role_live) kc->d.step_base_pow[e] = bp;
                    else {
                        const int pend_base_n = my.pend_base_n;
                        kc->d.pend_base[(size_t)ctx_id * pc.power_avg + umod_small(pend_base_n, pc.power_avg, pc.pavg_magic)] = bp;
                        my.pend_base_n = pend_base_n + 1;
                    }
                    base_acc = 0.f;
                }
            }
            my.base_acc = base_acc;
            if (is_dev) my.dev_rem -= 1;
            else if (sub + 1 >= K) { my.sub = 0; if (!role_live) my.fill_rem -= 1; }
            else my.sub = sub + 1;
        }
        if (unit_end && farm == 0) { sws = 0.f; swd = 0.f; syaw = 0.f; sp_ = 0.f; }
        lds_barrier<64>();
        WG_STAMP(6);
    }

    WG_STAMP(7);
    const KArgsPtr ke = wg_cold_args();
    const float part_slot = env_slot_sums((float)part_acc, N, NS, k, tid);
    const float stream_slot = env_slot_sums((float)stream_acc, N, NS, k, tid);
    if (valid && stepped) {
        const unsigned tb = (unsigned)((e * 2 * F + kbase) * N + g);
        const float4 s4 = Lsrc4[g];
        const float2 s2 = Lsrc2[g];
        ke->d.yaw[tb] = yaw; ke->d.u[tb] = tu; ke->d.v[tb] = 0.f; ke->d.w[tb] = 0.f;
        ke->d.ti_loc[tb] = tti; ke->d.power[tb] = tpow; ke->d.ct[tb] = tct;
        if (SPLIT && split_on) {
            float4* const bp = reinterpret_cast<float4*>(ke->d.bnd) + tb;
            bp->y = s4.z; bp->z = s4.w; bp->w = s2.y;
        } else reinterpret_cast<float4*>(ke->d.bnd)[tb] = make_float4(s2.x, s4.z, s4.w, s2.y);
        if (role_live && farm == 0) ke->d.old_yaw[(unsigned)(e * N + t)] = oyaw;
        if (t == 0) {
            const int n_flow = my.n_flow, P = ke->p.P;
            const double dt_d = ke->p.dt_d;
            double tm = my.c_time;
            for (int i = 0; i < n_flow; ++i) tm += dt_d;
            const unsigned n_emitted = my.n_emitted;
            int hd = my.c_head + (int)((n_emitted - my.n_emitted0) % (unsigned)P); if (hd >= P) hd -= P;
            WgSlot& slot = ke->d.slot[(unsigned)(e * 2 * F + kbase + k)];
            slot.part_count = my.c_part + (unsigned)part_slot;
            slot.add_count = my.c_add + (unsigned)stream_slot;
            slot.head = hd; slot.n_valid = my.n_valid; slot.s_off = my.s_off; slot.time = tm;
            slot.istep = my.c_istep + (unsigned)n_flow; slot.n_emitted = n_emitted;
            slot.dev_remaining = my.dev_rem; slot.fill_remaining = my.fill_rem;
            slot.flow_count = my.c_flow + (unsigned)n_flow;
            WgCtx& cx = ke->d.ctx[(unsigned)(e * 2 + c)];
            if (farm == 0) { cx.n_pushed = my.n_pushed; cx.pend_farm_n = my.pend_farm_n; }
            if (farm == F - 1) cx.pend_base_n = my.pend_base_n;
        }
    }
    if (SPLIT) {
        out.g_yaw = yaw; out.g_old = oyaw; out.g_pw = tpow;
        out.g_pwb = F == 2 ? __shfl(tpow, min(tid + N, 63), 64) : 0.f;
    }
    WG_STAMP(8);
    if (mode == WG_MODE_STEP && (WPE == 1 || c != env_live) && !defer_init) {
        const EnvSlotLds& bs = SL[WPE == 2 ? 0 : (env_live ^ 1) * F];
        const int bctx = e * 2 + (env_live ^ 1);
        bool build = false;
        if (ke->p.autoreset && bs.dev_rem == 0 && bs.fill_rem == 0)
            build = bs.n_flow == 0 ? (ke->d.gd->next_obs_ok != nullptr && ke->d.gd->next_obs_ok[bctx] == 0) : out.truncates != 0;
        if (build) {
            const int np = bs.n_pushed;
            out.first_obs = 1;
            full_barrier<64>();
            env_first_obs<GLUE != 0>(bctx, np, tid);
        }
    }
    if (defer_init) {
        env_init_episode<GLUE != 0>(e, env_live ^ 1, tid);
        full_barrier<64>();
        if (valid && t == 0 && c != env_live) {
            const WgSlot& slot = ke->d.slot[(unsigned)(e * 2 * F + kbase + k)];
            my.dev_rem = slot.dev_remaining; my.fill_rem = slot.fill_remaining;
        }
        lds_barrier<64>();
    }
}


template <bool NOISE, int GLUE, int WPE, int SPLIT = 0>
__global__ void __launch_bounds__(64 * (WPE + SPLIT), WG_ENV_WAVES)
k_flow_env(const FlowP p_, const FlowPtrs d_, const int mode, const float* __restrict__ actions,
           const uint8_t* __restrict__ mask, const int chunk, const WgParams gp_, const WgPtrs gd_,
           float* __restrict__ obs_out, float* __restrict__ reward_out, uint8_t* __restrict__ trunc_out,
           float* __restrict__ final_obs_out) {
    extern __shared__ __attribute__((aligned(16))) char smem[];
#ifdef WG_TIMELINE
    if (threadIdx.x == 0) { for (int i = 0; i < 20; ++i) wg_stamps[i] = 0; wg_stamps[14] = wall_clock64(); for (int i = 0; i < 8; ++i) wg_counts[i] = 0; }
    __syncthreads();
#endif
    const int wv4 = WPE == 2 ? __builtin_amdgcn_readfirstlane((int)(threadIdx.x >> 6)) : 0;
    int wv = wv4, role = 0;
    if (SPLIT == 1 && wv4 == 2) {
        role = 1;
        wv = __builtin_amdgcn_readfirstlane(reinterpret_cast<const int*>(wg_cold_args()->d.env + blockIdx.x)[offsetof(WgEnv, live) / 4]) & 1;
    }
    if (SPLIT == 2) { wv = wv4 & 1; role = wv4 >> 1; }
    const int lds_wave = WPE == 2 ? wg_cold_args()->p.env_lds : 0;
    char* const sm = smem + wv4 * lds_wave;
    char* const sm_pass = smem + (SPLIT == 2 ? 2 + wv : 2) * lds_wave;
    float* const zone = SPLIT ? reinterpret_cast<float*>(smem + (2 + SPLIT) * lds_wave) : nullptr;
    EnvFlowOut fo;
    env_flow<NOISE, WPE, GLUE, SPLIT>(sm, sm_pass, zone, wv, role, mode, actions, mask, chunk, fo);
    if (SPLIT && role == 1) {
        if (GLUE != 0 && fo.truncates) { __builtin_amdgcn_s_waitcnt(0x0070); __syncthreads(); }
        return;
    }
    if (GLUE != 0) {
        full_barrier<64>();
        if (WPE == 2) {
            if (wv != fo.env_live) {
                const EnvKArgsPtr kb = (EnvKArgsPtr)wg_cold_args();
                const int e = (int)blockIdx.x;
                if (kb->p.autoreset && !fo.truncates && (threadIdx.x & 63) == 0) {
                    const int F = kb->p.F, K = kb->p.K;
                    const EnvSlotLds* const SLb = reinterpret_cast<const EnvSlotLds*>(sm + WG_ENV_OFF_SL);
                    int work = 0;
                    for (int f = 0; f < F; ++f) work = max(work, SLb[f].dev_rem + K * SLb[f].fill_rem);
                    env_bg_plan(kb, work, fo, e);
                }
                if (fo.bg_init_pending && (threadIdx.x & 63) == 0) kb->d.ctx[e * 2 + wv].init_pending = 0;
                if (fo.truncates) __builtin_amdgcn_s_waitcnt(0x0070);
            }
            if (fo.truncates) __syncthreads();
        }
        if (WPE == 1 || wv == fo.env_live) {
            const EnvKArgsPtr kg = (EnvKArgsPtr)wg_cold_args();
            const int F = kg->p.F, K = kg->p.K;
            const EnvSlotLds* const SLa = reinterpret_cast<const EnvSlotLds*>(sm + WG_ENV_OFF_SL);
            const int la = WPE == 2 ? 0 : fo.env_live * F, lb = (fo.env_live ^ 1) * F;
            const float fp = SLa[la].out_pw, bp = F == 2 ? SLa[la + 1].out_pw : 0.f;
            int work = 0;
            if (WPE == 1) for (int f = 0; f < F; ++f) work = max(work, SLa[lb + f].dev_rem + K * SLa[lb + f].fill_rem);
            const int hw = reinterpret_cast<const int*>(sm + WG_ENV_OFF_HDR)[threadIdx.x & 31];
            LeanFused fz;
            fz.pre = nullptr;
            if (SPLIT) {
                if (!env_flag_wait(reinterpret_cast<int*>(zone) + LEAN_PRE_FLAG)) atomicOr(kg->d.status, WG_STATUS_BIT_STATE);
                const int gl = (int)(threadIdx.x & 63), own = gl < kg->p.N ? gl : 0;
                fz.pre = zone;
#pragma unroll
                for (int ch = 0; ch < WG_N_CH; ++ch) fz.nw[ch] = __shfl(fo.g_nw[ch], own, 64);
                fz.yaw = fo.g_yaw; fz.old_yaw = fo.g_old; fz.pw = fo.g_pw; fz.pwb = fo.g_pwb;
            }
            WG_STAMP(12);
            env_glue<GLUE, WPE>(kg, fz, fp, bp, work, fo, hw);
            WG_STAMP(13);
        }
    }
#ifdef WG_TIMELINE
    {
        const KArgsPtr kt = wg_cold_args();
        if (threadIdx.x == 0 && kt->d.dbg) {
            wg_stamps[15] = wall_clock64();
            long long* row = kt->d.dbg + (size_t)blockIdx.x * 32;
            for (int kq = 0; kq < 16; ++kq) row[kq] = wg_stamps[kq];
            row[16] = fo.bg_init_pending; row[17] = fo.rounds; row[18] = fo.first_obs;
            row[19] = GLUE != 0 ? (long long)kt->d.env[blockIdx.x].timestep : 0;
            for (int kq = 0; kq < 8; ++kq) row[20 + kq] = wg_counts[kq];
            for (int kq = 0; kq < 4; ++kq) row[28 + kq] = wg_stamps[16 + kq];
        }
    }
#endif
}

template <bool NZ, int G>
static EnvKernel env_kernel(const int wpe, const int split) {
    if constexpr (G != 0) {
        if (split == 2) return k_flow_env<NZ, G, 2, 2>;
        if (split == 1) return k_flow_env<NZ, G, 2, 1>;
    }
    return wpe == 2 ? k_flow_env<NZ, G, 2> : k_flow_env<NZ, G, 1>;
}
static void env_launch(const FlowP* p, const FlowPtrs* d, const int glue, const int mode, const float* actions, const uint8_t* mask,
                       const int chunk, const WgParams* gp, const WgPtrs* gd, float* obs, float* reward, uint8_t* trunc,
                       float* final_obs, hipStream_t st) {
    const int wpe = p->env_wpe == 2 ? 2 : 1;
    const int split = glue != 0 && wpe == 2 && (p->env_split == 1 || p->env_split == 2) ? p->env_split : 0;
    const size_t lds = (size_t)p->env_lds * (wpe + split) + (split ? LEAN_PRE_BYTES : 0);
    const EnvKernel k = glue == 2 ? (p->noise ? env_kernel<true, 2>(wpe, split) : env_kernel<false, 2>(wpe, split))
                      : glue == 1 ? (p->noise ? env_kernel<true, 1>(wpe, split) : env_kernel<false, 1>(wpe, split))
                                  : (p->noise ? env_kernel<true, 0>(wpe, split) : env_kernel<false, 0>(wpe, split));
    hipLaunchKernelGGL(k, dim3(p->B), dim3(64 * (wpe + split)), lds, st, *p, *d, mode, actions, mask, chunk, *gp, *gd, obs, reward, trunc, final_obs);
}

extern "C" void wg_launch_flow_env(const FlowP* p, const FlowPtrs* d, int mode, const float* actions, const uint8_t* mask,
                                   int chunk, hipStream_t st) {
    static const WgParams gp0{};
    static const WgPtrs gd0{};
    env_launch(p, d, 0, mode, actions, mask, chunk, &gp0, &gd0, nullptr, nullptr, nullptr, nullptr, st);
}

extern "C" void wg_launch_step_env(const FlowP* p, const FlowPtrs* d, const WgParams* gp, const WgPtrs* gd, const float* actions,
                                   float* obs, float* reward, uint8_t* trunc, float* final_obs, hipStream_t st) {
    env_launch(p, d, gd->multi_out ? 2 : 1, WG_MODE_STEP, actions, nullptr, 0, gp, gd, obs, reward, trunc, final_obs, st);
}
```

### windgym_amd/csrc/wg_env_common.h

```cpp
#pragma once
#include <hip/hip_runtime.h>

#include "wg_flow_dev.h"
#include "wg_glue_lean.h"

#ifndef WG_ENV_WAVES
#define WG_ENV_WAVES 4
#endif

static __device__ __attribute__((noinline)) void env_init_episode_mem(const WgParams* gp, const WgPtrs* gd, WgEnv* env_rw,
                                                                      const int e, const int c, const int lane) {
    const WgCtx& cx = gd->ctx[e * 2 + c];
    WgRng rng{cx.snap_state, cx.snap_inc, cx.snap_has32, cx.snap_u32};
    wg_ctx_init(*gp, *gd, rng, e, c, lane, cx.episode_tag, 0, gp->F);
    if (lane == 0) {
        env_rw->rng_state = rng.rng_state; env_rw->rng_inc = rng.rng_inc;
        env_rw->rng_has32 = rng.rng_has32; env_rw->rng_u32 = rng.rng_u32;
    }
}
struct EnvKArgs;
template <bool KARG>
__device__ __forceinline__ void env_init_episode(const int e, const int c, const int lane);

__device__ __forceinline__ float env_tab(const float* __restrict__ ys, const float x0, const float inv_dx, const int n_tab, const float x) {
    const float fx = (x - x0) * inv_dx;
    if (!(fx >= 0.0f) || fx > (float)(n_tab - 1)) return 0.0f;
    int i = (int)fx;
    if (i > n_tab - 2) i = n_tab - 2;
    const float f = fx - (float)i;
    return ys[i] + f * (ys[i + 1] - ys[i]);
}

__device__ __forceinline__ bool role_dev_any(const int autoreset, const int dev_rem, const int fill_rem) {
    return autoreset != 0 && (dev_rem > 0 || fill_rem > 0);
}
struct EnvKArgs {
    FlowP p; FlowPtrs d; int mode; const float* actions; const uint8_t* mask; int chunk; WgParams gp; WgPtrs gd;
    float* obs; float* reward; uint8_t* trunc; float* final_obs;
};
typedef const __attribute__((address_space(4))) EnvKArgs* EnvKArgsPtr;
template <bool KARG>
__device__ __forceinline__ void env_init_episode(const int e, const int c, const int lane) {
    const EnvKArgsPtr kg = (EnvKArgsPtr)wg_cold_args();
    if (!KARG) { env_init_episode_mem(kg->d.gp, kg->d.gd, kg->d.env_rw + e, e, c, lane); return; }
    const WgCtx& cx = kg->gd.ctx[e * 2 + c];
    WgRng rng{cx.snap_state, cx.snap_inc, cx.snap_has32, cx.snap_u32};
    wg_ctx_init(kg->gp, kg->gd, rng, e, c, lane, cx.episode_tag, 0, kg->gp.F);
    if (lane == 0) {
        WgEnv* const env_rw = kg->d.env_rw + e;
        env_rw->rng_state = rng.rng_state; env_rw->rng_inc = rng.rng_inc;
        env_rw->rng_has32 = rng.rng_has32; env_rw->rng_u32 = rng.rng_u32;
    }
}
template <bool KARG>
__device__ __forceinline__ void env_first_obs(const int ctx_id, const int n_pushed, const int lane) {
    const EnvKArgsPtr kg = (EnvKArgsPtr)wg_cold_args();
    bool lean = false;
    if (KARG) {
        const auto& p = kg->gp;
        lean = p.sums_mode && !(p.turb_ti || p.farm_ti || p.farm_obs > 0 || (p.sum_mask_f | p.cur_mask_f) != 0u) && p.N <= 32 &&
               kg->gd.next_obs != nullptr;
    }
    if (!lean) { wg_first_obs(kg->d.gp, kg->d.gd, ctx_id, n_pushed, lane); return; }
    const auto& p = kg->gp;
    const auto& d = kg->gd;
    const int N = p.N, NS = N + 1;
    int Lg = 1, lgs = 0;
    while (Lg < 8 && N * (Lg * 2) <= WG_WAVE) { Lg *= 2; ++lgs; }
    const int sub = lane & (Lg - 1), ent = lane >> lgs;
    const bool have = ent < N;
    const unsigned entc = have ? (unsigned)ent : 0u;
    const float* const rb = d.ring + (size_t)ctx_id * p.ring_stride;
    double* const ws_ = d.wsum + (size_t)ctx_id * WG_N_SUMS * NS + entc;
    float* const o = d.next_obs + (size_t)ctx_id * p.obs_dim + (size_t)entc * p.turb_obs;
    const unsigned sm = p.sum_mask_t, cmask = p.oc.cur_mask, rmask = p.oc.rol_mask;
    float v0[WG_N_CH][8], cv[WG_N_CH];
#pragma unroll
    for (int sl = 0; sl < WG_N_CH; ++sl) {
        const int off = p.ring_off[sl], cap = p.ring_cap[sl];
        const int cnt = p.sum_w[sl] < n_pushed ? p.sum_w[sl] : n_pushed;
        const int r0 = (n_pushed - cnt) % cap;
        const int last = n_pushed > 0 ? (n_pushed - 1) % cap : 0;
        cv[sl] = rb[(unsigned)(off + last * N) + entc];
#pragma unroll
        for (int u = 0; u < 8; ++u) {
            int row = r0 + max(min(sub + u * Lg, cnt - 1), 0); if (row >= cap) row -= cap;
            v0[sl][u] = rb[(unsigned)(off + row * N) + entc];
        }
    }
    int n = 0;
#pragma unroll
    for (int sl = 0; sl < WG_N_CH; ++sl) {
        const bool on = have && ((sm >> sl) & 1u);
        const int off = p.ring_off[sl], cap = p.ring_cap[sl];
        const int cnt = p.sum_w[sl] < n_pushed ? p.sum_w[sl] : n_pushed;
        const int r0 = (n_pushed - cnt) % cap;
        double acc = 0.0;
        if (on) {
#pragma unroll
            for (int u = 0; u < 8; ++u)
                if (sub + u * Lg < cnt) acc += (double)v0[sl][u];
#pragma nounroll
            for (int k = sub + 8 * Lg; k < cnt; k += 8 * Lg) {
                float v[8];
#pragma unroll
                for (int u = 0; u < 8; ++u) {
                    int row = r0 + min(k + u * Lg, cnt - 1); if (row >= cap) row -= cap;
                    v[u] = rb[(unsigned)(off + row * N) + entc];
                }
#pragma unroll
                for (int u = 0; u < 8; ++u)
                    if (k + u * Lg < cnt) acc += (double)v[u];
            }
        }
        for (int s2 = 1; s2 < Lg; s2 <<= 1) acc += __shfl_xor(acc, s2, 64);
        if (on && sub == 0) ws_[(size_t)sl * NS] = acc;
        if (have && sub == 0 && n_pushed > 0) {
            if ((cmask >> sl) & 1u) o[n++] = wg_scale_r(cv[sl], p.oc.mn[sl], p.oc.inv_rng[sl]);
            if ((rmask >> sl) & 1u) o[n++] = wg_scale_r(wg_sums_mean(p.oc, acc, sl, n_pushed), p.oc.mn[sl], p.oc.inv_rng[sl]);
        }
    }
    if (lane == 0) d.next_obs_ok[ctx_id] = 1;
}

__device__ __forceinline__ void env_flag_set(int* const f) {
    __atomic_store_n(f, 1, __ATOMIC_RELAXED);
    asm volatile("s_waitcnt lgkmcnt(0)" ::: "memory");
}
__device__ __forceinline__ bool env_flag_wait(int* const f) {
    for (int n = 0; n < (1 << 22); ++n) {
        if (__atomic_load_n(f, __ATOMIC_RELAXED) != 0) { asm volatile("" ::: "memory"); return true; }
        __builtin_amdgcn_s_sleep(2);
    }
    return false;
}

struct EnvFlowOut {
    int env_live, bg_init_pending;
    int truncates;
    int steps_done, time_max_live;
    int rounds, first_obs;
    float g_nw[WG_N_CH], g_yaw, g_old, g_pw, g_pwb;
};


__device__ __forceinline__ void env_bg_plan(const EnvKArgsPtr kb, const int work, const EnvFlowOut& fo, const int e) {
    const int steps_done = fo.steps_done + 1, time_max = fo.time_max_live;
    const int inc = 1 + (kb->gp.extra_inc ? 1 : 0);
    const long total = (long)((time_max + inc - 1) / inc) + 1;
    kb->d.env_rw[e].shadow_iters = work == 0 ? 0 : wg_shadow_share(work, total - steps_done, steps_done, e);
}

template <int GLUE, int WPE>
__device__ __forceinline__ void env_glue(const EnvKArgsPtr kg, LeanFused& fz, const float fp, const float bp, const int work,
                                         const EnvFlowOut& fo, const int hw) {
    fz.fp = fp; fz.bp = bp; fz.work = work;
    fz.bg_init_pending = WPE >= 2 ? 0 : fo.bg_init_pending;
    fz.plan_elsewhere = WPE >= 2;
    fz.hw = hw;
    lean_step<GLUE == 2, false, true>(*(const WgParams*)&kg->gp, *(const WgPtrs*)&kg->gd, kg->d.gp, kg->d.gd, (int)blockIdx.x,
                                      (int)(threadIdx.x & 63), kg->obs, kg->reward, kg->trunc, kg->final_obs, nullptr, fz);
}

typedef void (*EnvKernel)(FlowP, FlowPtrs, int, const float*, const uint8_t*, int, WgParams, WgPtrs, float*, float*, uint8_t*, float*);
```

### windgym_amd/csrc/wg_envb.hip

```cpp
#include <hip/hip_runtime.h>

#include "wg_env_common.h"
#include "wg_box_dev.h"
#include "wg_internal.h"

#ifndef WG_ENVB_U
#define WG_ENVB_U 2
#endif
#ifndef WG_ENVB_ABLATE
#define WG_ENVB_ABLATE 0
#endif
#ifndef WG_ENVB_WAVES
#define WG_ENVB_WAVES 4
#endif

struct __attribute__((aligned(16))) EnvbSlotLds {
    int dev_rem, fill_rem, sub, budget;
    double s_new;
    int n_emit, n_valid, new_valid;
    unsigned n_emitted;
    float s_off_f, ti_pow, sig, alpha;
    double s_off, ws;
    float ws_f, ti_f, wd_env, base_acc;
    int n_pushed, pend_farm_n, pend_base_n, n_flow;
// ... 672 lines not shown
                            const float4* const abox = kb->d.abox4;
                            const float4* const box8 = kb->d.box8;
                            const float4* const abox8 = kb->d.abox8;
                            const int rho = r0 + (tid >> sshift);
                            const bool live = rho < rho_hi && s < S;
                            const int gt = Lrow[min(rho, max(rho_hi - 1, 0))];
                            const int kt = gt & (NS - 1);
                            const EnvbSlotLds& q = SL[kt];
                            float amb[3] = {0.f, 0.f, 0.f}, g3[3] = {0.f, 0.f, 0.f};
                            float acc = 0.f, accw = 0.f, tia_max = 0.f;
                            bool addl = false;
                            if (live) {
                                const float cgt = __uint_as_float(Lrec4[gt].w);
                                const double xr = Lxr[gt], yr = Lyr[gt];
                                const int2 cr = Lcr[gt];
                                addl = ADDED && cr.y > 0;
                                const double bx = xr - q.ws * q.time + q.ox;
                                const double by = yr + (double)(rdy_s * cgt) + q.oy, bz = hub_d + (double)rdz_s;
                                const long long cell0 = WPE >= 2 ? ucell0 : q.box_cell0;
                                float4 va[8], vb[8];
                                float ax, ay, az, gx = 0.f, gy_ = 0.f, gz = 0.f;
                                if (box8) {
                                    const unsigned ra_ = envb_stencil_record(kb->p.bnx, kb->p.bny, kb->p.bnz, kb->p.inv_bdx, kb->p.inv_bdy, kb->p.inv_bdz,
                                                                             kb->p.inv_bn[0], kb->p.inv_bn[1], kb->p.inv_bn[2], bx, by, bz, ax, ay, az);
                                    const float4* const rec = box8 + cell0 * 8;
#pragma unroll
                                    for (int i = 0; i < 8; ++i) va[i] = (WG_ENVB_ABLATE & 2) ? make_float4(ax, ay, az, (float)ra_) : rec[ra_ * 8u + (unsigned)i];
                                } else {
                                    const float4* const fb = kb->d.box4 + cell0;
                                    unsigned oa[8];
                                    envb_box_corners<POW2>(kb->p.bnx, kb->p.bny, kb->p.bnz, kb->p.inv_bdx, kb->p.inv_bdy, kb->p.inv_bdz, bx, by, bz, oa, ax, ay, az);
#pragma unroll
                                    for (int i = 0; i < 8; ++i) va[i] = (WG_ENVB_ABLATE & 2) ? make_float4(ax, ay, az, (float)oa[i]) : fb[oa[i]];
                                }
                                if (addl) {
                                    if (abox8) {
                                        const unsigned rb_ = envb_stencil_record(kb->p.anx, kb->p.any, kb->p.anz, kb->p.inv_adx, kb->p.inv_ady, kb->p.inv_adz,
                                                                                 kb->p.inv_an[0], kb->p.inv_an[1], kb->p.inv_an[2], bx, by, bz, gx, gy_, gz);
#pragma unroll
                                        for (int i = 0; i < 8; ++i) vb[i] = (WG_ENVB_ABLATE & 4) ? make_float4(gx, gy_, gz, (float)rb_) : abox8[rb_ * 8u + (unsigned)i];
                                    } else {
                                        unsigned ob[8];
                                        envb_box_corners<APOW2>(kb->p.anx, kb->p.any, kb->p.anz, kb->p.inv_adx, kb->p.inv_ady, kb->p.inv_adz, bx, by, bz, ob, gx, gy_, gz);
#pragma unroll
                                        for (int i = 0; i < 8; ++i) vb[i] = (WG_ENVB_ABLATE & 4) ? make_float4(gx, gy_, gz, (float)ob[i]) : abox[ob[i]];
                                    }
                                }
                                const float ys = (float)yr + rdy_s * cgt, zs = hub + rdz_s;
                                for (int cq = cr.x; cq < cr.x + cr.y; ++cq) {
                                    const float4 pw = pp[cq - base];
                                    tia_max = fmaxf(tia_max, tiap[cq - base]);
                                    const float dy = ys - pw.x, dz = zs - pw.y;
                                    const float r2 = dy * dy + dz * dz;
                                    const float du = pw.w * __expf(-r2 * pw.z);
                                    acc += du;
                                    if (ADDED) accw += du * (km1 + km2r * pw.z * __builtin_amdgcn_sqrtf(r2));
                                }
                                envb_tri3(va, ax, ay, az, amb);
                                if (addl) envb_tri3(vb, gx, gy_, gz, g3);
                            }
                            float a0 = accw * g3[0], a1 = accw * g3[1], a2 = accw * g3[2];
                            if (S_pad == 16) {
                                acc = wg_row_sum(acc); amb[0] = wg_row_sum(amb[0]); amb[1] = wg_row_sum(amb[1]); amb[2] = wg_row_sum(amb[2]);
                                if (ADDED) { a0 = wg_row_sum(a0); a1 = wg_row_sum(a1); a2 = wg_row_sum(a2); }
                            } else {
                                for (int o = S_pad >> 1; o > 0; o >>= 1) {
                                    acc += __shfl_xor(acc, o, 64);
                                    amb[0] += __shfl_xor(amb[0], o, 64); amb[1] += __shfl_xor(amb[1], o, 64); amb[2] += __shfl_xor(amb[2], o, 64);
                                    if (ADDED) { a0 += __shfl_xor(a0, o, 64); a1 += __shfl_xor(a1, o, 64); a2 += __shfl_xor(a2, o, 64); }
                                }
                            }
                            if (live && s == 0) {
                                const float sig = q.sig, ti_f = q.ti_f;
                                Luvw[gt] = make_float4(q.ws_f + sig * amb[0] * inv_S - acc * inv_S + a0 * inv_S,
                                                       sig * amb[1] * inv_S + a1 * inv_S, sig * amb[2] * inv_S + a2 * inv_S,
                                                       __builtin_amdgcn_sqrtf(ti_f * ti_f + tia_max * tia_max));
                                if (addl) atomicAdd(&SL[kt].add_acc, S);
                            }
                        }
                    };
                    if (kp->p.box_pow2) { if (kp->p.abox_pow2) rows(std::true_type{}, std::true_type{}); else rows(std::true_type{}, std::false_type{}); }
                    else { if (kp->p.abox_pow2) rows(std::false_type{}, std::true_type{}); else rows(std::false_type{}, std::false_type{}); }
                }
                lds_barrier<64>();
                g_lo = g_hi; base = top;
                if (base >= nc && g_hi >= 64) break;
                if (g_hi >= 64) break;
            }
        }

        const bool measuring = stepping && !is_dev;
        const bool unit_end = measuring && (sub + 1 == K);
        const KArgsPtr kc = wg_cold_args();
        const float inv_k = 1.0f / (float)K;
        const unsigned ctx_id = (unsigned)(e * 2 + c);
        {
            const float4 pa = Lpark[g], pb = Lpark[NLP + g], pc = Lpark[2 * NLP + g], r = Luvw[g];
            yaw = pa.x; oyaw = pa.y; mvl_bits = pa.z; sg = pa.w;
            sws = pb.x; swd = pb.y; syaw = pb.z; sp_ = pb.w;
            tpow = pc.x; tct = pc.y; part_acc = __float_as_int(pc.z); cg = pc.w;
            tu = r.x; tv = r.y; tw = r.z; tti = r.w;
        }
        if (stepping) {
            Lring[g].z = Lring[g].w;
            stepped = true;
            const int n_tab = kc->p.n_tab;
            const float tab_x0 = kc->p.tab_x0, tab_inv_dx = kc->p.tab_inv_dx;
            const float* const tabp = reinterpret_cast<const float*>(smem + kc->p.env_off_tab);
            const float wsn = fmaxf(tu * cg + tv * sg, 0.0f);
            tpow = env_tab(tabp, tab_x0, tab_inv_dx, n_tab, wsn);
            tct = env_tab(tabp + n_tab, tab_x0, tab_inv_dx, n_tab, wsn) * cg * cg;
            if (measuring && farm == 0) {
                const float wsm = __builtin_amdgcn_sqrtf(tu * tu + tv * tv + tw * tw);
                const float wdm = atanf(tv / tu) * WG_RAD2DEG_F + my.wd_env;
                float val[WG_N_CH] = {sws + wsm, swd + wdm, syaw + yaw, sp_ + tpow};
                if (unit_end) {
                    const int n_pushed = my.n_pushed;
                    const unsigned tcx = ctx_id * (unsigned)N + (unsigned)t;
                    kc->d.cur_ws[tcx] = wsm;
                    kc->d.cur_wd[tcx] = wdm;
                    if (K != 1) {
#pragma unroll
                        for (int ch = 0; ch < WG_N_CH; ++ch) val[ch] *= inv_k;
                    }
                    if (NOISE) {
                        const uint64_t noise_key = ((CEnvPtr)(kc->d.env + e))->noise_key;
                        const uint32_t episode_tag = my.c_tag;
#pragma unroll
                        for (int ch = 0; ch < WG_N_CH; ++ch)
                            if (kc->p.noise_sigma[ch] != 0.f)
                                val[ch] += kc->p.noise_sigma[ch] * wg_noise_normal(noise_key, (uint32_t)n_pushed, (uint32_t)t,
                                                                                   (uint32_t)ch, episode_tag);
                    }
                    float* __restrict__ rbase = kc->d.ring + (size_t)ctx_id * kc->p.ring_stride;
#pragma unroll
                    for (int ch = 0; ch < WG_N_CH; ++ch) {
                        const int H = kc->p.hlen[ch];
                        rbase[(unsigned)(kc->p.ring_off[ch] + fast_mod(n_pushed, H, kc->p.inv_hlen[ch]) * N + t)] = val[ch];
                    }
                    sws = val[0]; swd = val[1]; sp_ = val[3];
                } else {
                    sws = val[0]; swd = val[1]; syaw = val[2]; sp_ = val[3];
                }
            }
        }
        float a_ws = 0.f, a_wd = 0.f, a_pw = 0.f;
        if (__ballot(measuring)) {
            a_ws = envb_slot_sums((measuring && farm == 0) ? sws : 0.f, NS);
            a_wd = envb_slot_sums((measuring && farm == 0) ? swd : 0.f, NS);
            a_pw = envb_slot_sums(measuring ? (farm == 0 ? sp_ : tpow) : 0.f, NS);
        }
        if (stepping && t == 0) {
            const int n_emit = my.n_emit;
            my.n_valid = my.new_valid; my.s_off = my.s_new; my.n_emitted += (unsigned)n_emit;
            my.n_flow += 1; my.budget -= 1;
            float base_acc = my.base_acc;
            if (measuring && farm == 1) base_acc += a_pw;
            if (unit_end) {
                const FlowP __attribute__((address_space(4)))& pc = kc->p;
                if (farm == 0) {
                    const int n_pushed = my.n_pushed, pend_farm_n = my.pend_farm_n;
                    float* fbase = kc->d.fring + (size_t)ctx_id * pc.fring_stride;
                    fbase[pc.fring_off[WG_CH_WS] + umod_small(n_pushed, pc.hlen[WG_CH_WS], pc.hmagic[WG_CH_WS])] = a_ws * pc.inv_N;
                    fbase[pc.fring_off[WG_CH_WD] + umod_small(n_pushed, pc.hlen[WG_CH_WD], pc.hmagic[WG_CH_WD])] = a_wd * pc.inv_N;
                    fbase[pc.fring_off[WG_CH_POWER] + umod_small(n_pushed, pc.hlen[WG_CH_POWER], pc.hmagic[WG_CH_POWER])] = a_pw;
                    my.out_pw = a_pw;
                    if (role_live) kc->d.step_farm_pow[e] = a_pw;
                    else {
                        kc->d.pend_farm[(size_t)ctx_id * pc.power_avg + umod_small(pend_farm_n, pc.power_avg, pc.pavg_magic)] = a_pw;
                        my.pend_farm_n = pend_farm_n + 1;
                    }
                    my.n_pushed = n_pushed + 1;
                } else {
                    const float bp = K == 1 ? base_acc : base_acc * inv_k;
                    my.out_pw = bp;
                    if (role_live) kc->d.step_base_pow[e] = bp;
                    else {
                        const int pend_base_n = my.pend_base_n;
                        kc->d.pend_base[(size_t)ctx_id * pc.power_avg + umod_small(pend_base_n, pc.power_avg, pc.pavg_magic)] = bp;
                        my.pend_base_n = pend_base_n + 1;
                    }
                    base_acc = 0.f;
                }
            }
            my.base_acc = base_acc;
            if (is_dev) my.dev_rem -= 1;
            else if (sub + 1 >= K) { my.sub = 0; if (!role_live) my.fill_rem -= 1; }
            else my.sub = sub + 1;
        }
        if (unit_end && farm == 0) { sws = 0.f; swd = 0.f; syaw = 0.f; sp_ = 0.f; }
        lds_barrier<64>();
    }

    const KArgsPtr ke = wg_cold_args();
    const float part_slot = envb_slot_sums(valid ? (float)part_acc : 0.f, NS);
    if (valid && stepped) {
        const unsigned tb = (unsigned)(e * 2 * F + kbase + k) * (unsigned)N + (unsigned)t;
        const float4 s4 = Lsrc4[g];
        ke->d.yaw[tb] = yaw; ke->d.u[tb] = tu; ke->d.v[tb] = tv; ke->d.w[tb] = tw;
        ke->d.ti_loc[tb] = tti; ke->d.power[tb] = tpow; ke->d.ct[tb] = tct;
        reinterpret_cast<float4*>(ke->d.bnd)[tb] = make_float4(Lbd[g], s4.z, s4.w, mvl_bits);
        if (role_live && farm == 0) ke->d.old_yaw[(unsigned)(e * N + t)] = oyaw;
        if (t == 0) {
            const int n_flow = my.n_flow, P = ke->p.P;
            const unsigned n_emitted = my.n_emitted;
            int hd = my.c_head + (int)((n_emitted - my.n_emitted0) % (unsigned)P); if (hd >= P) hd -= P;
            WgSlot& slot = ke->d.slot[(unsigned)(e * 2 * F + kbase + k)];
            slot.part_count = my.c_part + (unsigned)part_slot;
            slot.add_count = my.c_add + (unsigned)my.add_acc;
            slot.head = hd; slot.n_valid = my.n_valid; slot.s_off = my.s_off; slot.time = my.time;
            slot.istep = my.c_istep + (unsigned)n_flow; slot.n_emitted = n_emitted;
            slot.dev_remaining = my.dev_rem; slot.fill_remaining = my.fill_rem;
            slot.flow_count = my.c_flow + (unsigned)n_flow;
            WgCtx& cx = ke->d.ctx[(unsigned)(e * 2 + c)];
            if (farm == 0) { cx.n_pushed = my.n_pushed; cx.pend_farm_n = my.pend_farm_n; }
            if (farm == F - 1) cx.pend_base_n = my.pend_base_n;
        }
    }
    if (mode == WG_MODE_STEP && (WPE == 1 || (c != env_live && (WPE == 2 || farm == 0))) && !defer_init) {
        const EnvbSlotLds& bs = SL[WPE >= 2 ? 0 : (env_live ^ 1) * F];
        const int bctx = e * 2 + (env_live ^ 1);
        bool build = false;
        if (ke->p.autoreset && bs.dev_rem == 0 && bs.fill_rem == 0)
            build = bs.n_flow == 0 ? (ke->d.gd->next_obs_ok != nullptr && ke->d.gd->next_obs_ok[bctx] == 0) : out.truncates != 0;
        if (build) {
            const int np = bs.n_pushed;
            out.first_obs = 1;
            full_barrier<64>();
            env_first_obs<GLUE != 0>(bctx, np, tid);
        }
    }
    if (defer_init) {
        env_init_episode<GLUE != 0>(e, env_live ^ 1, tid);
        full_barrier<64>();
        if (valid && t == 0 && c != env_live) {
            const WgSlot& slot = ke->d.slot[(unsigned)(e * 2 * F + kbase + k)];
            my.dev_rem = slot.dev_remaining; my.fill_rem = slot.fill_remaining;
        }
        lds_barrier<64>();
    }
}

template <bool NOISE, int GLUE, int WPE>
__global__ void __launch_bounds__(64 * WPE, WG_ENVB_WAVES)
k_flow_envb(const FlowP p_, const FlowPtrs d_, const int mode, const float* __restrict__ actions,
            const uint8_t* __restrict__ mask, const int chunk, const WgParams gp_, const WgPtrs gd_,
            float* __restrict__ obs_out, float* __restrict__ reward_out, uint8_t* __restrict__ trunc_out,
            float* __restrict__ final_obs_out) {
    extern __shared__ __attribute__((aligned(16))) char smem[];
    typedef EnvbLds<(WPE == 4 ? 16 : 64)> LO;
    const int wv = WPE >= 2 ? __builtin_amdgcn_readfirstlane((int)(threadIdx.x >> 6)) : 0;
    const int lds_wave = WPE >= 2 ? wg_cold_args()->p.env_lds : 0;
    char* const sm = smem + wv * lds_wave;
    char* const shared = smem + WPE * lds_wave;
    int* const flags = reinterpret_cast<int*>(shared);
    if (WPE == 4 && threadIdx.x < 8) flags[threadIdx.x] = 0;
    EnvFlowOut fo;
    envb_flow<NOISE, WPE, GLUE>(sm, shared, wv, mode, actions, mask, chunk, fo);
    if (GLUE != 0) {
        full_barrier<64>();
        const EnvKArgsPtr kb = (EnvKArgsPtr)wg_cold_args();
        const int e = (int)blockIdx.x, F = kb->p.F, K = kb->p.K;
        const int c_w = WPE == 4 ? (wv >> 1) : wv, farm_w = WPE == 4 ? (wv & 1) : 0;
        const bool lane0 = (threadIdx.x & 63) == 0;
        if (WPE == 4 && lane0) envb_flag_set(flags + wv);
        if (WPE >= 2) {
            if (c_w != fo.env_live && farm_w == 0) {
                if (kb->p.autoreset && !fo.truncates && lane0) {
                    int work = 0;
                    if (WPE == 4) {
                        if (!envb_flag_wait(flags + wv + 1)) atomicOr(kb->d.status, WG_STATUS_BIT_STATE);
                        for (int f = 0; f < F; ++f) {
                            const EnvbSlotLds* const s_ = reinterpret_cast<const EnvbSlotLds*>(smem + (wv + f) * lds_wave + LO::SL);
                            work = max(work, s_->dev_rem + K * s_->fill_rem);
                        }
                    } else {
                        const EnvbSlotLds* const SLb = reinterpret_cast<const EnvbSlotLds*>(sm + LO::SL);
                        for (int f = 0; f < F; ++f) work = max(work, SLb[f].dev_rem + K * SLb[f].fill_rem);
                    }
                    env_bg_plan(kb, work, fo, e);
                }
                if (fo.bg_init_pending && lane0) kb->d.ctx[e * 2 + c_w].init_pending = 0;
            }
            if (c_w != fo.env_live && fo.truncates) __builtin_amdgcn_s_waitcnt(0x0070);
            if (fo.truncates) __syncthreads();
        }
        if (WPE == 1 || (c_w == fo.env_live && farm_w == 0)) {
            const EnvKArgsPtr kg = (EnvKArgsPtr)wg_cold_args();
            float fp, bp;
            int work = 0;
            if (WPE == 4) {
                if (F == 2 && !envb_flag_wait(flags + wv + 1)) { if (lane0) atomicOr(kg->d.status, WG_STATUS_BIT_STATE); }
                fp = reinterpret_cast<const EnvbSlotLds*>(sm + LO::SL)->out_pw;
                bp = F == 2 ? reinterpret_cast<const EnvbSlotLds*>(sm + lds_wave + LO::SL)->out_pw : 0.f;
            } else {
                const EnvbSlotLds* const SLa = reinterpret_cast<const EnvbSlotLds*>(sm + LO::SL);
                const int la = WPE == 2 ? 0 : fo.env_live * F, lb = (fo.env_live ^ 1) * F;
                fp = SLa[la].out_pw;
                bp = F == 2 ? SLa[la + 1].out_pw : 0.f;
                if (WPE == 1) for (int f = 0; f < F; ++f) work = max(work, SLa[lb + f].dev_rem + K * SLa[lb + f].fill_rem);
            }
            LeanFused fz;
            fz.pre = nullptr;
            env_glue<GLUE, WPE>(kg, fz, fp, bp, work, fo, reinterpret_cast<const int*>(sm + LO::HDR)[threadIdx.x & 31]);
        }
    }
}

template <bool NZ, int G>
static EnvKernel envb_kernel(const int wpe) {
    return wpe == 4 ? k_flow_envb<NZ, G, 4> : wpe == 2 ? k_flow_envb<NZ, G, 2> : k_flow_envb<NZ, G, 1>;
}
static void envb_launch(const FlowP* p, const FlowPtrs* d, const int glue, const int mode, const float* actions, const uint8_t* mask,
                        const int chunk, const WgParams* gp, const WgPtrs* gd, float* obs, float* reward, uint8_t* trunc,
                        float* final_obs, hipStream_t st) {
    const int wpe = p->env_wpe == 4 ? 4 : (p->env_wpe == 2 ? 2 : 1);
    const size_t lds = (size_t)p->env_lds * wpe + (wpe == 4 ? WG_ENVB_FLAG_BYTES : 0);
    const EnvKernel k = glue == 2 ? (p->noise ? envb_kernel<true, 2>(wpe) : envb_kernel<false, 2>(wpe))
                      : glue == 1 ? (p->noise ? envb_kernel<true, 1>(wpe) : envb_kernel<false, 1>(wpe))
                                  : (p->noise ? envb_kernel<true, 0>(wpe) : envb_kernel<false, 0>(wpe));
    hipLaunchKernelGGL(k, dim3(p->B), dim3(64 * wpe), lds, st, *p, *d, mode, actions, mask, chunk, *gp, *gd, obs, reward, trunc, final_obs);
}

extern "C" void wg_launch_flow_envb(const FlowP* p, const FlowPtrs* d, int mode, const float* actions, const uint8_t* mask,
                                    int chunk, hipStream_t st) {
    static const WgParams gp0{};
    static const WgPtrs gd0{};
    envb_launch(p, d, 0, mode, actions, mask, chunk, &gp0, &gd0, nullptr, nullptr, nullptr, nullptr, st);
}

extern "C" void wg_launch_step_envb(const FlowP* p, const FlowPtrs* d, const WgParams* gp, const WgPtrs* gd, const float* actions,
                                    float* obs, float* reward, uint8_t* trunc, float* final_obs, hipStream_t st) {
    envb_launch(p, d, gd->multi_out ? 2 : 1, WG_MODE_STEP, actions, nullptr, 0, gp, gd, obs, reward, trunc, final_obs, st);
}
```

### windgym_amd/csrc/wg_flow.h

```cpp
#pragma once
#include "wg_state.h"

#ifndef WG_BOX_WAVES
#define WG_BOX_WAVES 2
#endif
#ifndef WG_FLOW_WAVES_128
#define WG_FLOW_WAVES_128 6
#endif
#ifndef WG_FLOW_WAVES_CG
#define WG_FLOW_WAVES_CG 5
#endif
#ifndef WG_FLOW_WAVES_GL
#define WG_FLOW_WAVES_GL 4
#endif
#ifndef WG_FLOW_WAVES
#define WG_FLOW_WAVES 5
#endif
#ifndef WG_FLOW_WAVES_LF
#define WG_FLOW_WAVES_LF 3
#endif
#define WG_LF_OFF_TM(n) (16 * (size_t)(n))
#define WG_LF_OFF_BASE(n) (32 * (size_t)(n))
#define WG_LF_OFF_CL(n) ((36 * (size_t)(n) + 4 * 8 + 15) & ~(size_t)15)
#define WG_LF_OFF_DEF(n) ((WG_LF_OFF_CL(n) + (size_t)(n) * ((n) - 1) + 15) & ~(size_t)15)

struct FlowP {
    int B, N, F, K, P, S, S_pad, S_shift, NP, n_tab;
    int autoreset, action_method, base_controller, power_avg, script_rows, noise;
    int block;
    int res;
    int pstride;
    int target_chunk;
    int lf_cap;
    int lds_off_turb, lds_off_tab, lds_bytes;
    int rec_il;
    int gl;
    int lds_off_ql, lds_off_gat;
    int ql_shift;
    int ql_lpt_shift;
    int envw, env_lds, env_off_tab;
    int env_cap, envb_off_cl;
    int env_wpe;
    int env_split;
    int env_fused;
    int env_inc;
    float env_eps_max;
    float dt, D, inv_D, hub, dpart_f, R_rot, inv_N, inv_S, inv_P;
    double dt_d, dpart, inv_dpart;
    float yaw_min, yaw_max, yaw_step;
    float ka, kb, eps0, hill, tia, tib, tic, tid;
    float ue_scale;
    float tab_x0, tab_inv_dx;
    int hlen[WG_N_CH], ring_off[WG_N_CH], fring_off[WG_N_CH];
    float inv_hlen[WG_N_CH], inv_power_avg;
    unsigned hmagic[WG_N_CH], pavg_magic;
    int ring_stride, fring_stride;
    float noise_sigma[WG_N_CH];
    int turb_mode, bnx, bny, bnz, box_pow2;
    int coarse, cnx, cny, cnz, cbox_pow2;
    long long box_cells, cbox_cells;
    double inv_bdx, inv_bdy, inv_bdz, fc_scale, D_d, hub_d;
    float inv_sqrt_S;
    int added, anx, any, anz, abox_pow2;
    int no_ti_fold, deficit_model;
    float km1, km2r;
    float sg_af, sg_bf, sg_cf;
    double inv_adx, inv_ady, inv_adz;
    double inv_bn[3], inv_an[3];
    int an_ct, an_ti, an_x, an_r;
    float an_ct0, an_inv_dct, an_lti0, an_inv_dlti, an_inv_dx, an_inv_dr, an_inv_ka;
};

struct FlowPtrs {
    float *py, *pz, *vlp, *wlp;
    unsigned *rec_a, *rec_b;
    const float4* box4;
    const float4* box4c;
    const float4* abox4;
    const float4* box8;
    const float4* abox8;
    const float* dtab;
    float *yaw, *u, *v, *w, *ti_loc, *power, *ct;
    float* bnd;
    WgSlot* slot;
    WgCtx* ctx;
    const WgEnv* env;
    const double *xr, *yr;
    const int* jneed;
    const int* roff;
    const uint8_t* qown;
    int* status;
    float *ring, *fring, *cur_ws, *cur_wd, *pend_farm, *pend_base, *old_yaw, *step_farm_pow, *step_base_pow;
    const float *rotor_dy, *rotor_dz, *tab_power, *tab_ct;
    const float *script_uvw, *script_power;
    long long* dbg;
    const WgParams* gp;
    const WgPtrs* gd;
    WgEnv* env_rw;
};

#define WG_ENV_SLOT_LDS_BYTES 160
#define WG_ENV_FIXED_LDS_BYTES (3 * 64 * 16 + 2 * 64 * 8 + 4 * WG_ENV_SLOT_LDS_BYTES + 128)
#define WG_ENV_CAP 256
#define LEAN_PRE_BYTES 3584
#define WG_ENVB_FIXED_LDS_BYTES(nlp) ((93 + 48) * (nlp) + 4 * 208 + 128)
#define WG_TURB_LDS_BYTES 120
#define WG_GAT_BYTES (2 * 64 * 16 + 2 * 64 * 4)
#define WG_MASK_WORDS 4
```

### windgym_amd/csrc/wg_plan.h

```cpp
#pragma once
#include <algorithm>
#include <cmath>
#include <cstring>
#include <string>
#include <vector>

#ifndef __HIPCC__
struct float4;
#endif
#include "wg_flow.h"

struct WgHookInt {
    bool set = false;
    int v = 0;
};
struct WgHooks {
    WgHookInt flow_block, flow_res, flow_env, env_wpe, env_split, step_fused, sums, lds_pad, lf_cap, pstride_pad, step_graph;
    bool first_obs_gl_only = false, no_box8 = false, debug = false, timeline = false;
    std::string timeline_out;
};

struct WgPlan {
    WgParams p;
    FlowP f;
    int envw_eligible;
    int fused_eligible;
    int first_obs;
    double tab_x0, tab_dx;
    int reset_chunk, reset_launches;
    double alg_bytes;
};

inline double wg_defd(double v, double dflt) { return v == 0.0 ? dflt : v; }

inline int wg_plan_fail(std::string* err, int code, const std::string& msg) {
    if (err) *err = msg;
    return code;
}

inline int wg_validate_config(const wg_config* c, std::string* err) {
    if (!c) return wg_plan_fail(err, WG_ERR_INVALID, "null argument");
    if (c->abi_version != WG_ABI_VERSION) return wg_plan_fail(err, WG_ERR_INVALID, "abi_version mismatch");
    if (c->n_envs < 1 || c->n_turb < 1) return wg_plan_fail(err, WG_ERR_INVALID, "n_envs and n_turb must be >= 1");
    if (c->n_farms != 1 && c->n_farms != 2) return wg_plan_fail(err, WG_ERR_INVALID, "n_farms must be 1 or 2");
    if (c->k_sub < 1) return wg_plan_fail(err, WG_ERR_INVALID, "dt_env must be a multiple of dt_sim");
    if (c->n_particles < 8 || c->n_particles % 4) return wg_plan_fail(err, WG_ERR_INVALID, "n_particles must be a multiple of 4 (>= 8)");
    if (c->n_rotor_pts < 1 || c->n_rotor_pts > 64) return wg_plan_fail(err, WG_ERR_INVALID, "n_rotor_pts must be in [1, 64]");
    if (c->n_turb > 32 * WG_MASK_WORDS) return wg_plan_fail(err, WG_ERR_UNSUPPORTED, "n_turb > 128 is not supported by this build");
    if ((long long)c->n_turb * c->n_particles >= (1ll << 22) || c->n_particles > 16384)
        return wg_plan_fail(err, WG_ERR_UNSUPPORTED, "n_turb * n_particles must stay below 2^22 (and n_particles <= 16384)");
    if (!c->x_pos || !c->y_pos || !c->rotor_dy || !c->rotor_dz || !c->tab_ws || !c->tab_power || !c->tab_ct || c->n_tab < 2)
        return wg_plan_fail(err, WG_ERR_INVALID, "layout / rotor points / turbine table missing");
    if (c->action_method != WG_ACT_YAW && c->action_method != WG_ACT_WIND)
        return wg_plan_fail(err, WG_ERR_UNSUPPORTED, "The ActionMethod must be yaw or wind (absolute is not implemented)");
    if (c->reward_mode < 0 || c->reward_mode > 3)
        return wg_plan_fail(err, WG_ERR_INVALID, "The Power_reward must be either Baseline, Power_avg, None or Power_diff");
    if (c->reward_mode == WG_REW_POWER_DIFF && c->power_avg < 40)
        return wg_plan_fail(err, WG_ERR_INVALID, "The Power_avg must be larger then 40 for the Power_diff reward");
    if (c->reward_mode == WG_REW_BASELINE && c->n_farms != 2)
        return wg_plan_fail(err, WG_ERR_INVALID, "Baseline reward needs the baseline farm (n_farms = 2)");
    if (c->power_avg < 1) return wg_plan_fail(err, WG_ERR_INVALID, "Power_avg must be >= 1");
    if (c->turb_mode < WG_TURB_NONE || c->turb_mode > WG_TURB_BOX_POOL) return wg_plan_fail(err, WG_ERR_INVALID, "Invalid turbulence type specified");
    for (int i = 0; i < WG_N_CH; ++i)
        if (c->ch[i].history_len < 1 || c->ch[i].window_len < 1 || c->ch[i].history_n < 1)
            return wg_plan_fail(err, WG_ERR_INVALID, "sensor history/window lengths must be >= 1");
    {
        const double ka = wg_defd(c->m0_ka, 0.38), kb = wg_defd(c->m0_kb, 0.004), hill = wg_defd(c->m0_hill, 0.4);
        const double tia = c->no_ti_fold ? 0.0 : 0.466 * wg_defd(c->m0_ti_a, 0.73);
        const double k_hi = ka * std::sqrt(c->ti_max * c->ti_max + tia * tia) + kb;
        if (k_hi > 0.25 || std::fabs(hill) * c->ws_max > 16.0)
            return wg_plan_fail(err, WG_ERR_INVALID, "wind ranges exceed the 16-bit emission record: need ka*sqrt(TI_max^2 + 0.34^2) + kb <= 0.25 "
                                                     "(TI_max <= 0.55 with the default constants) and |hill| * ws_max <= 16 m/s");
    }
    if (c->deficit_model < 0 || c->deficit_model > 2)
        return wg_plan_fail(err, WG_ERR_INVALID, "deficit_model must be 0 (Gaussian), 1 (super-Gaussian) or 2 (tabulated eddy-viscosity deficit)");
    return 0;
}

inline int wg_plan_ch_count(const wg_channel& c, int on) { return (c.current && on) + (c.rolling_mean && on) * c.history_n; }

inline void wg_plan_scalars(const wg_config* c, WgParams& p) {
    p.B = c->n_envs; p.N = c->n_turb; p.F = c->n_farms; p.K = c->k_sub; p.P = c->n_particles; p.S = c->n_rotor_pts;
    p.NP = p.N * p.P;
    p.dt = (float)c->dt_sim; p.dt_d = c->dt_sim;
    p.D = (float)c->rotor_diameter; p.D_d = c->rotor_diameter; p.inv_D = 1.0f / (float)c->rotor_diameter;
    p.hub = (float)c->hub_height; p.hub_d = c->hub_height;
    p.dpart = c->d_particle * c->rotor_diameter;
    p.yaw_min = (float)c->yaw_min; p.yaw_max = (float)c->yaw_max; p.yaw_step = (float)c->yaw_step;
    p.yaw_min_d = c->yaw_min; p.yaw_max_d = c->yaw_max; p.yaw_step_d = c->yaw_step; p.yaw_start = c->yaw_start;
    p.action_method = c->action_method; p.base_controller = c->base_controller; p.yaw_init = c->yaw_init;
    p.has_yaw_defined = c->yaw_defined != nullptr;
    p.ws_min = c->ws_min; p.ws_max = c->ws_max; p.ti_min = c->ti_min; p.ti_max = c->ti_max;
    p.wd_min = c->wd_min; p.wd_max = c->wd_max; p.n_passthrough = c->n_passthrough;
    p.never_truncate = c->never_truncate;
    p.full_chains = c->full_chains;
    for (int i = 0; i < WG_N_CH; ++i) p.ch[i] = c->ch[i];
    p.turb_on[WG_CH_WS] = c->turb_ws; p.turb_on[WG_CH_WD] = c->turb_wd; p.turb_on[WG_CH_YAW] = 1;
    p.turb_on[WG_CH_POWER] = c->turb_power;
    p.farm_on[WG_CH_WS] = c->farm_ws; p.farm_on[WG_CH_WD] = c->farm_wd; p.farm_on[WG_CH_YAW] = 0;
    p.farm_on[WG_CH_POWER] = c->farm_power;
    p.turb_ti = c->turb_ti; p.farm_ti = c->farm_ti;
    const double mn[WG_N_CH] = {c->ws_scale_min, c->wd_scale_min, c->yaw_min, 0.0};
    const double mx[WG_N_CH] = {c->ws_scale_max, c->wd_scale_max, c->yaw_max, c->power_max};
    for (int i = 0; i < WG_N_CH; ++i) { p.sc_min[i] = (float)mn[i]; p.sc_rng[i] = (float)(mx[i] - mn[i]); }
    p.sc_rng_farm_power = (float)(c->power_max * c->n_turb);
    p.ti_min_f = (float)c->ti_scale_min; p.ti_rng_f = (float)(c->ti_scale_max - c->ti_scale_min);
    p.noise = c->noise;
    for (int i = 0; i < WG_N_CH; ++i) p.noise_sigma[i] = (float)c->noise_sigma[i];
    p.reward_mode = c->reward_mode; p.power_avg = c->power_avg; p.power_scaling = c->power_scaling;
    p.action_penalty = c->action_penalty; p.penalty_type = c->penalty_type;
    p.fill_a = c->fill_steps_agent; p.fill_b = c->fill_steps_base; p.autoreset = c->autoreset;
    p.extra_inc = c->extra_timestep_inc; p.turb_mode = c->turb_mode;
    p.ka = (float)wg_defd(c->m0_ka, 0.38); p.kb = (float)wg_defd(c->m0_kb, 0.004); p.eps0 = (float)wg_defd(c->m0_eps, 0.2);
    p.hill = (float)wg_defd(c->m0_hill, 0.4);
    p.tia = (float)wg_defd(c->m0_ti_a, 0.73); p.tib = (float)wg_defd(c->m0_ti_b, 0.8325);
    p.tic = (float)wg_defd(c->m0_ti_c, 0.0325); p.tid = (float)wg_defd(c->m0_ti_d, -0.32);
    p.fc_scale = wg_defd(c->m0_fc_scale, 2.0);
    p.n_tab = c->n_tab;
    double sx = 0, sy = 0;
    for (int t = 0; t < p.N; ++t) { sx += c->x_pos[t]; sy += c->y_pos[t]; }
    p.cx0 = sx / p.N; p.cy0 = sy / p.N;
}

inline void wg_plan_obs_layout(const wg_config* c, WgParams& p) {
    p.turb_obs = wg_plan_ch_count(c->ch[WG_CH_WS], c->turb_ws) + wg_plan_ch_count(c->ch[WG_CH_WD], c->turb_wd) +
                 wg_plan_ch_count(c->ch[WG_CH_YAW], 1) + (c->turb_ti ? 1 : 0) + wg_plan_ch_count(c->ch[WG_CH_POWER], c->turb_power);
    p.farm_obs = wg_plan_ch_count(c->ch[WG_CH_WS], c->farm_ws) + wg_plan_ch_count(c->ch[WG_CH_WD], c->farm_wd) +
                 (c->farm_ti ? 1 : 0) + wg_plan_ch_count(c->ch[WG_CH_POWER], c->farm_power);
    p.obs_dim = p.turb_obs * p.N + p.farm_obs;
    p.obs_dim_multi = p.turb_obs + p.farm_obs;
    p.hist_max = std::max(c->ch[WG_CH_WS].history_len, std::max(c->ch[WG_CH_WD].history_len, c->ch[WG_CH_YAW].history_len));
    for (int i = 0; i < WG_N_CH; ++i) {
        const bool on = p.turb_on[i] != 0;
        int st = 0;
        if (on && c->ch[i].current) st = 1;
        if (on && c->ch[i].rolling_mean) st = 2;
        if (i == WG_CH_WS && (c->turb_ti || c->farm_ti)) st = 2;
        p.stage_ch[i] = st;
    }
}

inline void wg_plan_sums(const wg_config* c, const WgHooks& hk, WgParams& p) {
    bool ok = true;
    for (int i = 0; i < WG_N_CH; ++i) {
        const bool used = p.turb_on[i] || (i != WG_CH_YAW && p.farm_on[i]);
        if (used && c->ch[i].rolling_mean && c->ch[i].history_n != 1) ok = false;
    }
    if (hk.sums.set && hk.sums.v == 0) ok = false;
    p.sums_mode = ok ? 1 : 0;
    for (int i = 0; i < WG_N_CH; ++i) {
        p.ring_cap[i] = c->ch[i].history_len + (ok ? 1 : 0);
        p.ring_magic[i] = (unsigned)((1ull << 32) / (unsigned long long)p.ring_cap[i]) + 1u;
    }
    if (ok) {
        for (int i = 0; i < WG_N_CH; ++i) {
            p.sum_w[i] = std::min(c->ch[i].window_len, c->ch[i].history_len);
            if (p.turb_on[i] && c->ch[i].rolling_mean) p.sum_mask_t |= 1u << i;
            if (p.turb_on[i] && c->ch[i].current) p.cur_mask_t |= 1u << i;
            if (i != WG_CH_YAW && p.farm_on[i] && c->ch[i].rolling_mean) p.sum_mask_f |= 1u << i;
            if (i != WG_CH_YAW && p.farm_on[i] && c->ch[i].current) p.cur_mask_f |= 1u << i;
        }
        p.sum_w[WG_SUM_TI1] = p.sum_w[WG_SUM_TI2] = c->ch[WG_CH_WS].history_len;
        if (c->turb_ti || c->farm_ti) p.sum_mask_t |= (1u << WG_SUM_TI1) | (1u << WG_SUM_TI2);
        if (c->farm_ti) p.sum_mask_f |= (1u << WG_SUM_TI1) | (1u << WG_SUM_TI2);
    }
    WgObsCfg& oc = p.oc;
    oc.cur_mask = p.cur_mask_t; oc.rol_mask = p.sum_mask_t & 0xfu;
    oc.turb_ti = c->turb_ti; oc.turb_obs = p.turb_obs; oc.obs_dim = p.obs_dim; oc.obs_dim_multi = p.obs_dim_multi;
    for (int i = 0; i < WG_N_CH; ++i) {
        oc.hlen[i] = c->ch[i].history_len; oc.wlen[i] = c->ch[i].window_len;
        oc.mn[i] = p.sc_min[i]; oc.inv_rng[i] = 1.0f / p.sc_rng[i];
        oc.inv_w[i] = 1.0 / (double)std::min(c->ch[i].window_len, c->ch[i].history_len);
    }
    oc.ti_mn = p.ti_min_f; oc.inv_ti_rng = 1.0f / p.ti_rng_f;
    int off = 0, foff = 0;
    for (int i = 0; i < WG_N_CH; ++i) {
        p.ring_off[i] = off; off += p.N * p.ring_cap[i];
        p.fring_off[i] = foff; foff += p.ring_cap[i];
    }
    p.ring_stride = off; p.fring_stride = foff;
}

inline int wg_plan_pstride(int NP, const WgHooks& hk) {
    size_t pstride = ((size_t)NP + 63) / 64;
    if (pstride % 2 == 0) pstride += 1;
    pstride *= 64;
    if (hk.pstride_pad.set) pstride = (size_t)NP + (size_t)hk.pstride_pad.v;
    return (int)pstride;
}

inline bool wg_uniform_grid(const wg_config* c, int* n, double* x0, double* dx) {
    bool uniform = true;
    const double dx0 = c->tab_ws[1] - c->tab_ws[0];
    for (int i = 2; i < c->n_tab; ++i)
        if (std::fabs((c->tab_ws[i] - c->tab_ws[i - 1]) - dx0) > 1e-9 * std::fabs(dx0)) uniform = false;
    *n = uniform ? c->n_tab : 1024;
    *x0 = c->tab_ws[0];
    *dx = uniform ? dx0 : (c->tab_ws[c->n_tab - 1] - c->tab_ws[0]) / (*n - 1);
    return uniform;
}
inline void wg_uniform_table(const wg_config* c, std::vector<float>* power, std::vector<float>* ct, double* x0, double* dx) {
    int nu = 0;
    const bool uniform = wg_uniform_grid(c, &nu, x0, dx);
    power->clear(); ct->clear();
    if (uniform) {
        for (int i = 0; i < nu; ++i) { power->push_back((float)c->tab_power[i]); ct->push_back((float)c->tab_ct[i]); }
        return;
    }
    int k = 0;
    for (int i = 0; i < nu; ++i) {
        const double x = std::min(*x0 + i * *dx, c->tab_ws[c->n_tab - 1]);
        while (k + 2 < c->n_tab && c->tab_ws[k + 1] <= x) ++k;
        const double f = (x - c->tab_ws[k]) / (c->tab_ws[k + 1] - c->tab_ws[k]);
        power->push_back((float)(c->tab_power[k] + f * (c->tab_power[k + 1] - c->tab_power[k])));
        ct->push_back((float)(c->tab_ct[k] + f * (c->tab_ct[k + 1] - c->tab_ct[k])));
    }
}

struct WgFlowVariant {
    bool small;
    int res, block;
    int tc0;
    int ql_shift, ql_lpt_shift;
};

inline WgFlowVariant wg_plan_flow_variant(const WgParams& p, const WgHooks& hk) {
    WgFlowVariant v;
    int tc = 1024 / p.N; if (tc < 1) tc = 1; if (tc > p.N) tc = p.N;
    v.tc0 = tc;
    v.small = p.N <= 32 && tc == p.N;
    v.res = v.small ? 1 : 0;
    v.block = v.small ? 64 : 256;
    if (!v.small && p.N <= 255 && p.turb_mode == WG_TURB_NONE) v.res = 1;
    if (hk.flow_block.set) {
        const int b = hk.flow_block.v;
        if (b == 256) { v.res = 0; v.block = 256; }
        else if ((b == 64 || b == 128) && v.small) { v.res = 1; v.block = b; }
    }
    if (hk.flow_res.set) {
        if (hk.flow_res.v != 0 && p.N <= 255) { v.res = 1; if (!v.small) v.block = 256; } else if (hk.flow_res.v == 0) { v.res = 0; v.block = 256; }
    }
    v.ql_shift = 0;
    while ((1 << v.ql_shift) < p.P / 4) ++v.ql_shift;
    if (((long)p.N << v.ql_shift) > 65536) { v.res = 0; v.block = 256; }
    v.ql_lpt_shift = 0;
    while (v.ql_lpt_shift < 3 && (p.N << (v.ql_lpt_shift + 1)) <= v.block) ++v.ql_lpt_shift;
    return v;
}

struct WgFlowCarve {
    int target_chunk, lf_cap, gl, lds_off_ql, lds_off_gat, lds_off_turb, lds_off_tab;
    size_t bytes;
};

inline WgFlowCarve wg_plan_flow_carve(const WgParams& p, const WgHooks& hk, const WgFlowVariant& v, int res, int block, int n_tab_u, int S_shift,
                                      int added) {
    WgFlowCarve k;
    int tc = v.tc0;
    k.lf_cap = 0; k.gl = 0; k.lds_off_ql = 0; k.lds_off_gat = 0;
    size_t off = sizeof(float) * 4 * (size_t)tc * p.N;
    if (res) {
        const size_t ql = ((size_t)p.NP / 2 + 15) & ~(size_t)15;
        if (!v.small) {
            const size_t budget = std::max(ql, off) + sizeof(float) * (size_t)tc * p.N;
            const int fit = (int)((budget - 16) / ((added ? 22 : 10) * (size_t)p.N));
            tc = std::max(tc, std::min(p.N, fit));
        }
        off = std::max(ql, ((size_t)(added ? 22 : 10) * tc * p.N + 16 + 15) & ~(size_t)15);
        if (block == 256 && p.turb_mode == WG_TURB_NONE) {
            const size_t fixed = WG_LF_OFF_DEF(p.N);
            off = std::max(off, (fixed + 8 * 512 + 15) & ~(size_t)15);
            k.lf_cap = (int)((off - fixed) / 8);
            if (hk.lf_cap.set) k.lf_cap = std::max(64, std::min(k.lf_cap, hk.lf_cap.v));
        }
        if (block == 64 && p.turb_mode == WG_TURB_NONE) {
            k.gl = 1;
            off = ((size_t)10 * tc * p.N + 16 + 15) & ~(size_t)15;
            k.lds_off_ql = (int)off; off += ql;
            k.lds_off_gat = (int)off; off += WG_GAT_BYTES;
        }
    }
    k.target_chunk = tc;
    k.lds_off_turb = (int)off; off += (size_t)WG_TURB_LDS_BYTES * p.N;
    off = (off + 15) & ~(size_t)15;
    k.lds_off_tab = (int)off;
    off += sizeof(float) * (2 * (size_t)n_tab_u + 2 * (size_t)p.S) + (k.gl ? 0 : sizeof(unsigned) * WG_MASK_WORDS * (size_t)tc) +
           (res ? 0 : sizeof(float) * (size_t)tc * p.N);
    off += sizeof(int) * (4 * (size_t)p.N + 4);
    if (added && res) off += sizeof(float) * 3 * ((size_t)p.N << S_shift) + sizeof(int) * (size_t)tc;
    k.bytes = (off + 15) & ~(size_t)15;
    return k;
}

inline size_t wg_plan_farm_quads(const wg_config* c, const WgParams& p) {
    size_t qf = 0;
    for (int t = 0; t < p.N; ++t) {
        double dm = 0;
        for (int j = 0; j < p.N; ++j) dm = std::max(dm, std::hypot(c->x_pos[j] - c->x_pos[t], c->y_pos[j] - c->y_pos[t]));
        long len = (((long)(dm / p.dpart) + 4) + 3) & ~3L;
        if (len > p.P || p.full_chains) len = p.P;
        qf += (size_t)len / 4;
    }
    return qf;
}

inline bool wg_plan_env(const WgParams& p, FlowP& f, bool small, size_t qf, int lds_limit) {
    const int NSl = 2 * p.F, NL = NSl * p.N;
    const size_t clb = ((size_t)2 * NL * (p.N > 1 ? p.N - 1 : 1) + 15) & ~(size_t)15;
    const size_t stage = std::max((size_t)8 * WG_ENV_CAP + clb, ((size_t)2 * NSl * qf + 15) & ~(size_t)15);
    f.env_off_tab = (int)((WG_ENV_FIXED_LDS_BYTES + stage + 15) & ~(size_t)15);
    const size_t o = (size_t)f.env_off_tab + sizeof(float) * (2 * (size_t)f.n_tab + 2 * (size_t)p.S);
    f.env_lds = (int)((o + 15) & ~(size_t)15);
    return f.res && small && f.block == 64 && f.gl && p.turb_mode == WG_TURB_NONE && NL <= 64 && p.N <= 32 && p.P <= 4096 && !f.added &&
           f.deficit_model == 0 && f.env_lds <= 32768 && f.env_lds <= lds_limit;
}

struct WgEnvbCarve {
    int env_cap, off_cl, off_tab;
    size_t bytes;
};
inline WgEnvbCarve wg_plan_envb_carve(const WgParams& p, int n_tab_u, int wpe) {
    WgEnvbCarve k;
    const int nlp = wpe == 4 ? 16 : 64;
    const int nl_w = (wpe == 4 ? 1 : (wpe == 2 ? p.F : 2 * p.F)) * p.N;
    k.env_cap = wpe == 4 ? 128 : 256;
    size_t ob = WG_ENVB_FIXED_LDS_BYTES(nlp) + (size_t)20 * k.env_cap;
    k.off_cl = (int)ob;
    ob = (ob + (size_t)2 * nl_w * (p.N > 1 ? p.N - 1 : 1) + 15) & ~(size_t)15;
    k.off_tab = (int)ob;
    ob += sizeof(float) * (2 * (size_t)n_tab_u + 2 * (size_t)p.S);
    k.bytes = (ob + 15) & ~(size_t)15;
    return k;
}

inline bool wg_plan_envb(const WgParams& p, const WgHooks& hk, FlowP& f, bool small, int lds_limit, int* wpe) {
    const int NL = 2 * p.F * p.N;
    *wpe = (p.B <= 2048) ? 2 : 1;
    if (hk.env_wpe.set) {
        const int w = hk.env_wpe.v;
        *wpe = (w == 4 && p.F == 2 && p.N <= 16) ? 4 : (w == 2 ? 2 : (w == 4 ? 2 : 1));
    }
    if (!(f.res && small && f.block == 64 && !f.gl && p.turb_mode >= WG_TURB_BOX && NL <= 64 && p.N <= 32 && p.P <= 4096 && f.S_pad <= 16 &&
          f.deficit_model == 0))
        return false;
    WgEnvbCarve k = wg_plan_envb_carve(p, f.n_tab, *wpe);
    while (*wpe > 1 && *wpe * k.bytes + 64 > (size_t)lds_limit) {
        *wpe /= 2;
        k = wg_plan_envb_carve(p, f.n_tab, *wpe);
    }
    f.env_cap = k.env_cap; f.envb_off_cl = k.off_cl; f.env_off_tab = k.off_tab; f.env_lds = (int)k.bytes;
    return f.env_lds <= 32768 && f.env_lds <= lds_limit;
}

inline void wg_plan_step_kernels(const wg_config* c, const WgHooks& hk, const WgParams& p, FlowP& f, bool small, int lds_limit) {
    const size_t qf = wg_plan_farm_quads(c, p);
    const bool env_ok = wg_plan_env(p, f, small, qf, lds_limit);
    int envb_wpe = 1;
    const bool envb_ok = wg_plan_envb(p, hk, f, small, lds_limit, &envb_wpe);
    f.env_inc = 1 + (p.extra_inc ? 1 : 0);
    f.env_eps_max = std::min(1.0f, (float)(p.eps0 * std::sqrt(3.0))) + 2.0f / 65535.0f;
    f.envw = ((env_ok || envb_ok) && !hk.flow_block.set && !hk.flow_res.set) ? 1 : 0;
    if (hk.flow_env.set) f.envw = ((env_ok || envb_ok) && hk.flow_env.v != 0) ? 1 : 0;
    f.env_wpe = (p.B <= 2048 && 2 * f.env_lds <= lds_limit) ? 2 : 1;
    if (hk.env_wpe.set) f.env_wpe = (hk.env_wpe.v == 2 && 2 * f.env_lds <= lds_limit) ? 2 : 1;
    const bool split_ok = env_ok && f.env_wpe == 2 && p.K == 1 && 4 * f.env_lds + 4096 <= lds_limit;
    f.env_split = (split_ok && p.B <= 1024 && qf >= 256) ? (p.B <= 512 ? 2 : 1) : 0;
    if (hk.env_split.set) f.env_split = (hk.env_split.v != 0 && split_ok && p.B <= 2048) ? (hk.env_split.v == 2 ? 2 : 1) : 0;
    if (envb_ok) f.env_wpe = envb_wpe;
    const bool gen = p.turb_ti || p.farm_ti || p.farm_obs > 0 || (p.sum_mask_f | p.cur_mask_f) != 0;
    f.env_fused = (f.envw && p.sums_mode && !gen && p.power_avg <= 64) ? 1 : 0;
    if (hk.step_fused.set) f.env_fused = (f.env_fused && hk.step_fused.v != 0) ? 1 : 0;
}

inline void wg_plan_flow_scalars(const wg_config* c, const WgParams& p, double tab_x0, double tab_dx, FlowP& f) {
    f.B = p.B; f.N = p.N; f.F = p.F; f.K = p.K; f.P = p.P; f.S = p.S; f.NP = p.NP;
    f.S_pad = 1; f.S_shift = 0;
    while (f.S_pad < p.S) { f.S_pad <<= 1; f.S_shift++; }
    f.autoreset = p.autoreset; f.action_method = p.action_method; f.base_controller = p.base_controller;
    f.power_avg = p.power_avg; f.script_rows = 0; f.noise = (p.noise == WG_NOISE_NORMAL);
    f.dt = p.dt; f.D = p.D; f.inv_D = p.inv_D; f.hub = p.hub; f.dpart_f = (float)p.dpart; f.R_rot = 0.5f * p.D;
    f.inv_N = 1.0f / (float)p.N; f.inv_S = 1.0f / (float)p.S; f.inv_P = 1.0f / (float)p.P;
    f.inv_power_avg = 1.0f / (float)(p.power_avg > 0 ? p.power_avg : 1);
    f.pavg_magic = (unsigned)((1ull << 32) / (unsigned long long)(p.power_avg > 0 ? p.power_avg : 1)) + 1u;
    f.dt_d = p.dt_d; f.dpart = p.dpart; f.inv_dpart = 1.0 / p.dpart;
    f.yaw_min = p.yaw_min; f.yaw_max = p.yaw_max; f.yaw_step = p.yaw_step;
    f.ka = p.ka; f.kb = p.kb; f.eps0 = p.eps0; f.hill = p.hill; f.tia = p.tia; f.tib = p.tib; f.tic = p.tic; f.tid = p.tid;
    f.tab_x0 = (float)tab_x0; f.tab_inv_dx = (float)(1.0 / tab_dx);
    f.ue_scale = p.turb_mode == WG_TURB_NONE ? 1.0f : 2.0f;
    for (int i = 0; i < WG_N_CH; ++i) {
        f.hlen[i] = p.ring_cap[i]; f.ring_off[i] = p.ring_off[i]; f.fring_off[i] = p.fring_off[i];
        f.inv_hlen[i] = 1.0f / (float)p.ring_cap[i];
        f.hmagic[i] = (unsigned)((1ull << 32) / (unsigned long long)p.ring_cap[i]) + 1u;
        f.noise_sigma[i] = p.noise_sigma[i];
    }
    f.ring_stride = p.ring_stride; f.fring_stride = p.fring_stride;
    f.turb_mode = p.turb_mode; f.fc_scale = p.fc_scale; f.D_d = p.D_d; f.hub_d = p.hub_d;
    f.inv_sqrt_S = 1.0f / std::sqrt((float)p.S);
    f.added = (c->added_turbulence != 0 && c->turb_mode != WG_TURB_NONE) ? 1 : 0;
    f.no_ti_fold = c->no_ti_fold != 0; f.deficit_model = c->deficit_model;
    f.km1 = (float)wg_defd(c->m0_km1, 0.6); f.km2r = (float)(2.0 * wg_defd(c->m0_km2, 0.35) * 0.5 * p.D_d);
    f.sg_af = (float)wg_defd(c->m0_sg_af, 3.11); f.sg_bf = (float)wg_defd(c->m0_sg_bf, -0.68); f.sg_cf = (float)wg_defd(c->m0_sg_cf, 2.41);
    f.an_inv_ka = (float)(1.0 / wg_defd(c->m0_ka, 0.38));
}

inline int wg_plan_reset_launches(const wg_config* c, const WgParams& p, int reset_chunk) {
    double xmn = 1e300, xmx = -1e300, ymn = 1e300, ymx = -1e300;
    for (int t = 0; t < p.N; ++t) {
        xmn = std::min(xmn, c->x_pos[t]); xmx = std::max(xmx, c->x_pos[t]);
        ymn = std::min(ymn, c->y_pos[t]); ymx = std::max(ymx, c->y_pos[t]);
    }
    const double ext_x = xmx - xmn, ext_y = ymx - ymn;
    const double diag = std::sqrt(ext_x * ext_x + ext_y * ext_y);
    const double ws_lo = std::max(1e-3, std::min(c->ws_min, c->ws_max));
    const long max_dev = (long)std::ceil(2.0 * diag / ws_lo / c->dt_sim) + 2;
    const long max_work = max_dev + (long)p.K * (std::max(p.fill_a, p.fill_b) + 1);
    return (int)((max_work + reset_chunk - 1) / reset_chunk) + 1;
}

inline double wg_plan_alg_bytes(const WgParams& p) {
    const bool turb = p.turb_mode != WG_TURB_NONE, boxm = p.turb_mode >= WG_TURB_BOX;
    const double per_farm_step = (double)p.NP * (4 + 4 + 8 + (turb ? 24 : 0) + (boxm ? 64 : 0)) +
                                 (double)p.N * (7 * 4 * 2 + 16) + (boxm ? (double)p.N * p.S * 96 : 0.0);
    return (double)p.B * ((double)p.K * p.F * per_farm_step + 20.0 * p.N + 12.0 * p.obs_dim + 20.0);
}

inline int wg_plan_create(const wg_config* c, const WgHooks& hk, int lds_limit, WgPlan* out, std::string* err) {
    memset(out, 0, sizeof(*out));
    WgParams& p = out->p;
    FlowP& f = out->f;
    wg_plan_scalars(c, p);
    wg_plan_obs_layout(c, p);
    wg_plan_sums(c, hk, p);
    wg_uniform_grid(c, &f.n_tab, &out->tab_x0, &out->tab_dx);
    wg_plan_flow_scalars(c, p, out->tab_x0, out->tab_dx, f);
    f.pstride = wg_plan_pstride(p.NP, hk);

    const WgFlowVariant v = wg_plan_flow_variant(p, hk);
    f.res = v.res; f.block = v.block; f.ql_shift = v.ql_shift; f.ql_lpt_shift = v.ql_lpt_shift;
    WgFlowCarve k = wg_plan_flow_carve(p, hk, v, f.res, f.block, f.n_tab, f.S_shift, f.added);
    if (f.res && k.bytes > (size_t)lds_limit) {
        f.res = 0; f.block = 256;
        k = wg_plan_flow_carve(p, hk, v, f.res, f.block, f.n_tab, f.S_shift, f.added);
    }
    if (k.bytes > (size_t)lds_limit)
        return wg_plan_fail(err, WG_ERR_UNSUPPORTED, "wg_create: k_flow needs " + std::to_string(k.bytes) + " bytes of LDS per workgroup (limit " +
                                                     std::to_string(lds_limit) + "): too many turbines for one workgroup");
    if (f.deficit_model != 0 && !f.res)
        return wg_plan_fail(err, WG_ERR_UNSUPPORTED, "deficit_model 1 / 2 (super-Gaussian, eddy-viscosity table) are built into the compact k_flow variants only "
                                                     "(farms of up to 32 turbines, larger ones with steady inflow)");
    p.compact = f.res;
    f.target_chunk = k.target_chunk; f.lf_cap = k.lf_cap; f.gl = k.gl; f.lds_off_ql = k.lds_off_ql; f.lds_off_gat = k.lds_off_gat;
    f.lds_off_turb = k.lds_off_turb; f.lds_off_tab = k.lds_off_tab;
    f.lds_bytes = (int)k.bytes;
    if (hk.lds_pad.set) f.lds_bytes = std::min(lds_limit, f.lds_bytes + hk.lds_pad.v);
    f.rec_il = (f.gl || (f.res && f.block == 256 && p.turb_mode == WG_TURB_NONE)) ? 1 : 0;

    wg_plan_step_kernels(c, hk, p, f, v.small, lds_limit);
    out->envw_eligible = f.envw; out->fused_eligible = f.env_fused;
    out->first_obs = (f.gl || (f.res && p.sums_mode && !hk.first_obs_gl_only)) ? 1 : 0;
    out->reset_chunk = 32;
    out->reset_launches = wg_plan_reset_launches(c, p, out->reset_chunk);
    out->alg_bytes = wg_plan_alg_bytes(p);
    return 0;
}

inline void wg_plan_step_path(const WgPlan& plan, long long box_cells, long long abox_cells, int* envw, int* env_fused) {
    const bool big = plan.f.turb_mode != WG_TURB_NONE && (box_cells >= (1ll << 28) || abox_cells >= (1ll << 28));
    *envw = (plan.envw_eligible && !big) ? 1 : 0;
    *env_fused = (plan.fused_eligible && *envw) ? 1 : 0;
}
```

Baseline: 82.76 million.

## Pack four envs per workgroup and share advection work across their waves

Adds an EPW=4 instantiation of the one-wave-per-env flow kernel that places four environments in one workgroup, each wave with its own LDS region plus a small shared counter area. Waves claim 64-quad advection chunks through workgroup-scope atomic counters, so a wave that finishes early can steal chunks from sibling envs, and each wave then waits until the others have completed its own chunks. The planner turns this on by default for large batches (B>2048, F==2, enough quads) when four env LDS regions fit under a residency limit. The aim is to balance load across envs with uneven quad counts and to cut the cost of many tiny workgroups. The price is extra barriers, atomics and spin-waits, plus changed occupancy.

```diff
diff --git a/windgym_amd/build.py b/windgym_amd/build.py
--- a/windgym_amd/build.py
+++ b/windgym_amd/build.py
@@ -7,7 +7,7 @@
 HERE = os.path.dirname(os.path.abspath(__file__))
 CSRC = os.path.join(HERE, "csrc")
 LIB = os.path.join(HERE, "libwindgym_hip.so")
-SOURCES = ["wg_flow.hip", "wg_env.hip", "wg_envb.hip", "wg_kernels.hip", "wg_api.hip", "wg_mann.hip", "wg_steady.hip", "wg_policy.hip", "wg_ppo.hip"]
+SOURCES = ["wg_flow.hip", "wg_env.hip", "wg_env4.hip", "wg_envb.hip", "wg_kernels.hip", "wg_api.hip", "wg_mann.hip", "wg_steady.hip", "wg_policy.hip", "wg_ppo.hip"]
 
 
 def _headers():
diff --git a/windgym_amd/csrc/wg_api.hip b/windgym_amd/csrc/wg_api.hip
--- a/windgym_amd/csrc/wg_api.hip
+++ b/windgym_amd/csrc/wg_api.hip
@@ -37,7 +37,7 @@
     k.flow_block = num("WG_FLOW_BLOCK"); k.flow_res = num("WG_FLOW_RES"); k.flow_env = num("WG_FLOW_ENV");
     k.env_wpe = num("WG_ENV_WPE"); k.env_split = num("WG_ENV_SPLIT"); k.step_fused = num("WG_STEP_FUSED");
     k.sums = num("WG_SUMS"); k.lds_pad = num("WG_LDS_PAD"); k.lf_cap = num("WG_LF_CAP"); k.pstride_pad = num("WG_PSTRIDE_PAD");
-    k.step_graph = num("WG_STEP_GRAPH");
+    k.step_graph = num("WG_STEP_GRAPH"); k.env_epw = num("WG_ENV_EPW");
     k.first_obs_gl_only = wg_hook("WG_FIRST_OBS_GL_ONLY") != nullptr;
     k.no_box8 = wg_hook("WG_NO_BOX8") != nullptr;
     k.debug = wg_hook("WG_DEBUG") != nullptr;
@@ -311,9 +311,9 @@
                        : (f.res ? "compact rings / pair-major" : "uniform rings / sample-major"),
                 f.envw && f.env_split ? " + a pass wave for the running episode's context" : "",
                 f.block, f.envw ? f.env_lds : f.lds_bytes, f.pstride);
-        fprintf(stderr, "[windgym] plan: res %d block %d gl %d rec_il %d target_chunk %d lf_cap %d lds_bytes %d | envw %d env_wpe %d env_split %d env_fused %d "
+        fprintf(stderr, "[windgym] plan: res %d block %d gl %d rec_il %d target_chunk %d lf_cap %d lds_bytes %d | envw %d env_wpe %d env_split %d env_epw %d env_fused %d "
                         "env_lds %d env_off_tab %d | sums_mode %d first_obs %d reset_launches %d\n",
-                f.res, f.block, f.gl, f.rec_il, f.target_chunk, f.lf_cap, f.lds_bytes, f.envw, f.env_wpe, f.env_split, f.env_fused, f.env_lds,
+                f.res, f.block, f.gl, f.rec_il, f.target_chunk, f.lf_cap, f.lds_bytes, f.envw, f.env_wpe, f.env_split, f.env_epw, f.env_fused, f.env_lds,
                 f.env_off_tab, h->p.sums_mode, h->plan.first_obs, h->plan.reset_launches);
     }
     *out = owner.release();
diff --git a/windgym_amd/csrc/wg_device.h b/windgym_amd/csrc/wg_device.h
--- a/windgym_amd/csrc/wg_device.h
+++ b/windgym_amd/csrc/wg_device.h
@@ -228,12 +228,21 @@
 };
 
 #ifdef WG_TIMELINE
+#ifdef WG_STAMP_PER_WAVE
+__shared__ long long wg_stamps_w[4][20];
+__shared__ int wg_counts_w[4][8];
+#define wg_stamps wg_stamps_w[threadIdx.x >> 6]
+#define wg_counts wg_counts_w[threadIdx.x >> 6]
+#define WG_STAMP_LANE0 ((threadIdx.x & 63) == 0)
+#else
 __shared__ long long wg_stamps[20];
 __shared__ int wg_counts[8];
-#define WG_STAMP(k) do { if (threadIdx.x == 0) wg_stamps[k] = clock64(); } while (0)
+#define WG_STAMP_LANE0 (threadIdx.x == 0)
+#endif
+#define WG_STAMP(k) do { if (WG_STAMP_LANE0) wg_stamps[k] = clock64(); } while (0)
 #define WG_STAMP2(k) WG_STAMP(k)
 #define WG_ICLK0() long long wg_iclk_ = clock64()
-#define WG_ICLK(i) do { if (threadIdx.x == 0) { const long long c_ = clock64(); wg_counts[i] = (int)(c_ - wg_iclk_); wg_iclk_ = c_; } } while (0)
+#define WG_ICLK(i) do { if (WG_STAMP_LANE0) { const long long c_ = clock64(); wg_counts[i] = (int)(c_ - wg_iclk_); wg_iclk_ = c_; } } while (0)
 #else
 #define WG_STAMP(k) do { } while (0)
 #define WG_ICLK0() do { } while (0)
diff --git a/windgym_amd/csrc/wg_env.hip b/windgym_amd/csrc/wg_env.hip
--- a/windgym_amd/csrc/wg_env.hip
+++ b/windgym_amd/csrc/wg_env.hip
@@ -2,6 +2,10 @@
 
 #ifndef WG_ENV_ABLATE
 #define WG_ENV_ABLATE 0
+#endif
+#define WG_STAMP_PER_WAVE
+#ifndef WG_ENV_SHARE
+#define WG_ENV_SHARE 2
 #endif
 #include "wg_env_common.h"
 #include "wg_internal.h"
@@ -50,10 +54,11 @@
     return __shfl(s, k << 5, 64);
 }
 
-template <bool NOISE, int WPE, int GLUE, int SPLIT>
+template <bool NOISE, int WPE, int GLUE, int SPLIT, int EPW>
 __device__ __forceinline__ void env_flow(char* const smem, char* const smem_pass, float* const zone, const int wv, const int role, const int mode,
-                                         const float* __restrict__ actions, const uint8_t* __restrict__ mask, const int chunk, EnvFlowOut& out) {
-    const int tid = threadIdx.x & 63, e = blockIdx.x;
+                                         const float* __restrict__ actions, const uint8_t* __restrict__ mask, const int chunk, EnvFlowOut& out,
+                                         const int e, char* const smem_grp, const int wq) {
+    const int tid = threadIdx.x & 63;
     int N, F, NS, NL;
     float inv_N;
     {
@@ -143,6 +148,9 @@
         if (WPE == 2) {
             asm volatile("" : "+s"(env_live), "+s"(env_done), "+s"(env_shadow_iters), "+s"(env_steps_done), "+s"(env_timestep), "+s"(env_time_max_live) : : "memory");
             asm volatile("s_barrier" ::: "memory");
+        }
+        if (EPW > 1) {
+            asm volatile("s_waitcnt lgkmcnt(0)\n\ts_barrier" ::: "memory");
         }
         if (SPLIT && role == 1 && GLUE != 0 && c == env_live) {
             const EnvKArgsPtr kz = (EnvKArgsPtr)wg_cold_args();
@@ -593,25 +601,29 @@
 #endif
 
             const float dpart_f = kp->p.dpart_f, inv_D = kp->p.inv_D, dt = kp->p.dt, eps0 = kp->p.eps0;
+            char* sreg = smem;
+            float* spy = py_env;
+            unsigned* sra = ra_env;
+            int snl = nlist;
             struct QuadReq { float4 py; uint4 ra, rb; int g, kq; unsigned q; };
             auto request = [&](QuadReq& r, const int cidx) __attribute__((always_inline)) {
-                const bool v = cidx < nlist;
-                const unsigned en = v ? ql[cidx] : 0u;
+                const bool v = cidx < snl;
+                const unsigned en = v ? reinterpret_cast<const unsigned short*>(sreg + WG_ENV_OFF_STAGE)[cidx] : 0u;
                 r.g = (int)(en >> 10); r.kq = (int)(en & 1023u);
-                const int4 rg = Lring[r.g];
+                const int4 rg = reinterpret_cast<const int4*>(sreg + WG_ENV_OFF_RING)[r.g];
                 r.q = (((unsigned)rg.w * pstride + (unsigned)rg.x) >> 2) + (unsigned)r.kq;
                 if (v) {
-                    r.py = reinterpret_cast<const float4*>(py_env)[r.q];
-                    r.ra = reinterpret_cast<const uint4*>(ra_env)[2u * r.q];
-                    r.rb = reinterpret_cast<const uint4*>(ra_env)[2u * r.q + 1u];
+                    r.py = reinterpret_cast<const float4*>(spy)[r.q];
+                    r.ra = reinterpret_cast<const uint4*>(sra)[2u * r.q];
+                    r.rb = reinterpret_cast<const uint4*>(sra)[2u * r.q + 1u];
                 }
             };
             auto advect_quad = [&](const QuadReq& cur, const int cidx) __attribute__((always_inline)) {
-                if (cidx >= nlist) return;
+                if (cidx >= snl) return;
                 const int gq = cur.g, kq = cur.kq;
                 const unsigned q = cur.q;
-                const int4 rg = Lring[gq];
-                const EnvSlotLds& sl = SL[rg.w];
+                const int4 rg = reinterpret_cast<const int4*>(sreg + WG_ENV_OFF_RING)[gq];
+                const EnvSlotLds& sl = reinterpret_cast<const EnvSlotLds*>(sreg + WG_ENV_OFF_SL)[rg.w];
                 const int n_emit_q = sl.n_emit, n_valid_q = sl.n_valid;
                 const float sof = sl.s_off_f;
                 const int R = rg.y, hd = rg.z;
@@ -628,9 +640,9 @@
                     const float adv = m0_advect(pyv[i], rav[i], rbv[i], j, sof, dpart_f, inv_D, dt, eps0);
                     pyv[i] = j < n_valid_q ? adv : pyv[i];
                 }
-                const float y0 = Lsrc4[gq].y;
+                const float y0 = reinterpret_cast<const float4*>(sreg + WG_ENV_OFF_SRC4)[gq].y;
                 if (emits) {
-                    const uint4 rn = Lrec4[gq];
+                    const uint4 rn = reinterpret_cast<const uint4*>(sreg + WG_ENV_OFF_REC4)[gq];
 #pragma unroll
                     for (int i = 0; i < 4; ++i) {
                         int ei = e0 + i; if (ei >= R) ei -= R;
@@ -638,28 +650,87 @@
                             pyv[i] = y0; rav[i] = rn.x; rbv[i] = rn.y;
                         }
                     }
-                    reinterpret_cast<uint4*>(ra_env)[2u * q] = make_uint4(rav[0], rbv[0], rav[1], rbv[1]);
-                    reinterpret_cast<uint4*>(ra_env)[2u * q + 1u] = make_uint4(rav[2], rbv[2], rav[3], rbv[3]);
-                }
-                reinterpret_cast<float4*>(py_env)[q] = make_float4(pyv[0], pyv[1], pyv[2], pyv[3]);
+                    reinterpret_cast<uint4*>(sra)[2u * q] = make_uint4(rav[0], rbv[0], rav[1], rbv[1]);
+                    reinterpret_cast<uint4*>(sra)[2u * q + 1u] = make_uint4(rav[2], rbv[2], rav[3], rbv[3]);
+                }
+                reinterpret_cast<float4*>(spy)[q] = make_float4(pyv[0], pyv[1], pyv[2], pyv[3]);
                 float ex = 0.f;
 #pragma unroll
                 for (int i = 0; i < 4; ++i) {
                     int j = j0 - i; if (j < 0) j += R;
                     if (j < n_valid_q) ex = fmaxf(ex, fabsf(pyv[i] - y0));
                 }
-                if (ex > Lsrc2[gq].x) atomicMax(reinterpret_cast<int*>(&Lsrc2[gq].x), __float_as_int(ex));
+                float* const bd = &reinterpret_cast<float2*>(sreg + WG_ENV_OFF_SRC2)[gq].x;
+                if (ex > *bd) atomicMax(reinterpret_cast<int*>(bd), __float_as_int(ex));
             };
             QuadReq qa, qb;
             qa.py = qb.py = make_float4(0.f, 0.f, 0.f, 0.f); qa.ra = qa.rb = qb.ra = qb.rb = make_uint4(0u, 0u, 0u, 0u);
-            request(qa, tid);
-            if (SPLIT && role == 1) {
-                if (!env_flag_wait(reinterpret_cast<int*>(smem + WG_ENV_OFF_HDR))) atomicOr(kp->d.status, WG_STATUS_BIT_STATE);
-            }
-            for (int base = 0; base < nlist; base += 64) {
-                qb = qa;
-                request(qa, base + 64 + tid);
-                advect_quad(qb, base + tid);
+            if constexpr (EPW == 1 || WG_ENV_SHARE == 0) {
+                request(qa, tid);
+                if (SPLIT && role == 1) {
+                    if (!env_flag_wait(reinterpret_cast<int*>(smem + WG_ENV_OFF_HDR))) atomicOr(kp->d.status, WG_STATUS_BIT_STATE);
+                }
+                for (int base = 0; base < nlist; base += 64) {
+                    qb = qa;
+                    request(qa, base + 64 + tid);
+                    advect_quad(qb, base + tid);
+                }
+            } else {
+                unsigned* const shw = reinterpret_cast<unsigned*>(smem_grp + EPW * kp->p.env_lds);
+                if (tid == 0) {
+                    __hip_atomic_store(shw + 2 * wq + 1, 0u, __ATOMIC_RELAXED, __HIP_MEMORY_SCOPE_WORKGROUP);
+                    __hip_atomic_store(shw + 2 * wq, (unsigned)nlist << 10, __ATOMIC_RELAXED, __HIP_MEMORY_SCOPE_WORKGROUP);
+                }
+                const int n_src = (WG_ENV_SHARE == 1 || defer_init || out.truncates || out.bg_init_pending) ? 1 : EPW;
+                int mine = 0;
+                for (int s = 0; s < n_src; ++s) {
+                    const int sw = (wq + s) & (EPW - 1);
+                    unsigned* const cur = shw + 2 * sw;
+                    if (s > 0) {
+                        const unsigned v = __builtin_amdgcn_readfirstlane(__hip_atomic_load(cur, __ATOMIC_RELAXED, __HIP_MEMORY_SCOPE_WORKGROUP));
+                        if ((v & 1023u) >= (((v >> 10) + 63u) >> 6)) continue;
+                        const int es = e - wq + sw;
+                        const size_t pb_s = (size_t)(es * 2 * F) * pstride;
+                        sreg = smem_grp + sw * kp->p.env_lds;
+                        spy = kp->d.py + pb_s;
+                        sra = kp->d.rec_a + 2 * pb_s;
+                    }
+                    auto claim_issue = [&]() __attribute__((always_inline)) {
+                        unsigned v = 0u;
+                        if (tid == 0) v = __builtin_amdgcn_atomic_inc32(cur, 0xFFFFFFFFu, __ATOMIC_RELAXED, "workgroup");
+                        return v;
+                    };
+                    auto claim_take = [&](const unsigned pv) __attribute__((always_inline)) {
+                        const unsigned v = __builtin_amdgcn_readfirstlane(pv);
+                        snl = (int)(v >> 10);
+                        const int kn = (int)(v & 1023u);
+                        return kn < ((snl + 63) >> 6) ? kn : -1;
+                    };
+                    unsigned pv = claim_issue();
+                    int kt = claim_take(pv), n_done = 0;
+                    if (kt < 0) continue;
+                    request(qa, kt * 64 + tid);
+                    pv = claim_issue();
+                    for (;;) {
+                        qb = qa;
+                        const int kc = kt;
+                        kt = claim_take(pv);
+                        if (kt >= 0) { request(qa, kt * 64 + tid); pv = claim_issue(); }
+                        advect_quad(qb, kc * 64 + tid);
+                        ++n_done;
+                        if (kt < 0) break;
+                    }
+                    if (s == 0) mine = n_done;
+                    else {
+                        __builtin_amdgcn_s_waitcnt(0x0070);
+                        if (tid == 0) __hip_atomic_fetch_add(cur + 1, (unsigned)n_done, __ATOMIC_RELAXED, __HIP_MEMORY_SCOPE_WORKGROUP);
+#ifdef WG_TIMELINE
+                        if (tid == 0) atomicAdd(&wg_counts[5], n_done);
+#endif
+                    }
+                }
+                const unsigned others = (unsigned)(((nlist + 63) >> 6) - mine);
+                if (others != 0u && !env_word_wait(shw + 2 * wq + 1, others)) atomicOr(kp->d.status, WG_STATUS_BIT_STATE);
             }
         }
         lds_barrier<64>();
@@ -841,17 +912,29 @@
 }
 
 
-template <bool NOISE, int GLUE, int WPE, int SPLIT = 0>
-__global__ void __launch_bounds__(64 * (WPE + SPLIT), WG_ENV_WAVES)
+template <bool NOISE, int GLUE, int WPE, int SPLIT = 0, int EPW = 1>
+__global__ void __launch_bounds__(64 * (WPE + SPLIT) * EPW, WG_ENV_WAVES)
 k_flow_env(const FlowP p_, const FlowPtrs d_, const int mode, const float* __restrict__ actions,
            const uint8_t* __restrict__ mask, const int chunk, const WgParams gp_, const WgPtrs gd_,
            float* __restrict__ obs_out, float* __restrict__ reward_out, uint8_t* __restrict__ trunc_out,
            float* __restrict__ final_obs_out) {
     extern __shared__ __attribute__((aligned(16))) char smem[];
 #ifdef WG_TIMELINE
-    if (threadIdx.x == 0) { for (int i = 0; i < 20; ++i) wg_stamps[i] = 0; wg_stamps[14] = wall_clock64(); for (int i = 0; i < 8; ++i) wg_counts[i] = 0; }
+    if ((threadIdx.x & 63) == 0) { for (int i = 0; i < 20; ++i) wg_stamps[i] = 0; wg_stamps[14] = wall_clock64(); for (int i = 0; i < 8; ++i) wg_counts[i] = 0; }
     __syncthreads();
 #endif
+    static_assert(EPW == 1 || (EPW == 4 && WPE == 1 && SPLIT == 0), "several envs per workgroup: the unsplit one-wave-per-env instantiations");
+    const int wq = EPW > 1 ? __builtin_amdgcn_readfirstlane((int)(threadIdx.x >> 6)) : 0;
+    const int e = EPW > 1 ? (int)blockIdx.x * EPW + wq : (int)blockIdx.x;
+    if (EPW > 1) {
+        const KArgsPtr k0 = wg_cold_args();
+        if ((threadIdx.x & 63) == 0) {
+            unsigned* const shw = reinterpret_cast<unsigned*>(smem + EPW * k0->p.env_lds);
+            __hip_atomic_store(shw + 2 * wq, 0u, __ATOMIC_RELAXED, __HIP_MEMORY_SCOPE_WORKGROUP);
+            __hip_atomic_store(shw + 2 * wq + 1, 0u, __ATOMIC_RELAXED, __HIP_MEMORY_SCOPE_WORKGROUP);
+        }
+        if (e >= k0->p.B) { asm volatile("s_waitcnt lgkmcnt(0)" ::: "memory"); return; }
+    }
     const int wv4 = WPE == 2 ? __builtin_amdgcn_readfirstlane((int)(threadIdx.x >> 6)) : 0;
     int wv = wv4, role = 0;
     if (SPLIT == 1 && wv4 == 2) {
@@ -859,12 +942,12 @@
         wv = __builtin_amdgcn_readfirstlane(reinterpret_cast<const int*>(wg_cold_args()->d.env + blockIdx.x)[offsetof(WgEnv, live) / 4]) & 1;
     }
     if (SPLIT == 2) { wv = wv4 & 1; role = wv4 >> 1; }
-    const int lds_wave = WPE == 2 ? wg_cold_args()->p.env_lds : 0;
-    char* const sm = smem + wv4 * lds_wave;
+    const int lds_wave = (WPE == 2 || EPW > 1) ? wg_cold_args()->p.env_lds : 0;
+    char* const sm = smem + (EPW > 1 ? wq : wv4) * lds_wave;
     char* const sm_pass = smem + (SPLIT == 2 ? 2 + wv : 2) * lds_wave;
     float* const zone = SPLIT ? reinterpret_cast<float*>(smem + (2 + SPLIT) * lds_wave) : nullptr;
     EnvFlowOut fo;
-    env_flow<NOISE, WPE, GLUE, SPLIT>(sm, sm_pass, zone, wv, role, mode, actions, mask, chunk, fo);
+    env_flow<NOISE, WPE, GLUE, SPLIT, EPW>(sm, sm_pass, zone, wv, role, mode, actions, mask, chunk, fo, e, smem, wq);
     if (SPLIT && role == 1) {
         if (GLUE != 0 && fo.truncates) { __builtin_amdgcn_s_waitcnt(0x0070); __syncthreads(); }
         return;
@@ -874,7 +957,6 @@
         if (WPE == 2) {
             if (wv != fo.env_live) {
                 const EnvKArgsPtr kb = (EnvKArgsPtr)wg_cold_args();
-                const int e = (int)blockIdx.x;
                 if (kb->p.autoreset && !fo.truncates && (threadIdx.x & 63) == 0) {
                     const int F = kb->p.F, K = kb->p.K;
                     const EnvSlotLds* const SLb = reinterpret_cast<const EnvSlotLds*>(sm + WG_ENV_OFF_SL);
@@ -907,19 +989,19 @@
                 fz.yaw = fo.g_yaw; fz.old_yaw = fo.g_old; fz.pw = fo.g_pw; fz.pwb = fo.g_pwb;
             }
             WG_STAMP(12);
-            env_glue<GLUE, WPE>(kg, fz, fp, bp, work, fo, hw);
+            env_glue<GLUE, WPE>(kg, e, fz, fp, bp, work, fo, hw);
             WG_STAMP(13);
         }
     }
 #ifdef WG_TIMELINE
     {
         const KArgsPtr kt = wg_cold_args();
-        if (threadIdx.x == 0 && kt->d.dbg) {
+        if ((EPW > 1 ? (threadIdx.x & 63) == 0 : threadIdx.x == 0) && kt->d.dbg) {
             wg_stamps[15] = wall_clock64();
-            long long* row = kt->d.dbg + (size_t)blockIdx.x * 32;
+            long long* row = kt->d.dbg + (size_t)e * 32;
             for (int kq = 0; kq < 16; ++kq) row[kq] = wg_stamps[kq];
             row[16] = fo.bg_init_pending; row[17] = fo.rounds; row[18] = fo.first_obs;
-            row[19] = GLUE != 0 ? (long long)kt->d.env[blockIdx.x].timestep : 0;
+            row[19] = GLUE != 0 ? (long long)kt->d.env[e].timestep : 0;
             for (int kq = 0; kq < 8; ++kq) row[20 + kq] = wg_counts[kq];
             for (int kq = 0; kq < 4; ++kq) row[28 + kq] = wg_stamps[16 + kq];
         }
@@ -927,6 +1009,14 @@
 #endif
 }
 
+extern "C" EnvKernel wg_env_kernel_epw4(int noise, int glue);
+#ifdef WG_ENV_TU_EPW4
+template <bool NZ>
+static EnvKernel env_kernel_epw4(const int glue) {
+    return glue == 2 ? k_flow_env<NZ, 2, 1, 0, 4> : glue == 1 ? k_flow_env<NZ, 1, 1, 0, 4> : k_flow_env<NZ, 0, 1, 0, 4>;
+}
+extern "C" EnvKernel wg_env_kernel_epw4(int noise, int glue) { return noise ? env_kernel_epw4<true>(glue) : env_kernel_epw4<false>(glue); }
+#else
 template <bool NZ, int G>
 static EnvKernel env_kernel(const int wpe, const int split) {
     if constexpr (G != 0) {
@@ -940,11 +1030,13 @@
                        float* final_obs, hipStream_t st) {
     const int wpe = p->env_wpe == 2 ? 2 : 1;
     const int split = glue != 0 && wpe == 2 && (p->env_split == 1 || p->env_split == 2) ? p->env_split : 0;
-    const size_t lds = (size_t)p->env_lds * (wpe + split) + (split ? LEAN_PRE_BYTES : 0);
-    const EnvKernel k = glue == 2 ? (p->noise ? env_kernel<true, 2>(wpe, split) : env_kernel<false, 2>(wpe, split))
-                      : glue == 1 ? (p->noise ? env_kernel<true, 1>(wpe, split) : env_kernel<false, 1>(wpe, split))
-                                  : (p->noise ? env_kernel<true, 0>(wpe, split) : env_kernel<false, 0>(wpe, split));
-    hipLaunchKernelGGL(k, dim3(p->B), dim3(64 * (wpe + split)), lds, st, *p, *d, mode, actions, mask, chunk, *gp, *gd, obs, reward, trunc, final_obs);
+    const int epw = wpe == 1 && split == 0 && p->env_epw == 4 ? 4 : 1;
+    const size_t lds = (size_t)p->env_lds * (wpe + split) * epw + (split ? LEAN_PRE_BYTES : 0) + (epw > 1 ? WG_ENV_SHARE_BYTES : 0);
+    const EnvKernel k = epw == 4    ? wg_env_kernel_epw4(p->noise, glue)
+                        : glue == 2 ? (p->noise ? env_kernel<true, 2>(wpe, split) : env_kernel<false, 2>(wpe, split))
+                        : glue == 1 ? (p->noise ? env_kernel<true, 1>(wpe, split) : env_kernel<false, 1>(wpe, split))
+                                    : (p->noise ? env_kernel<true, 0>(wpe, split) : env_kernel<false, 0>(wpe, split));
+    hipLaunchKernelGGL(k, dim3((p->B + epw - 1) / epw), dim3(64 * (wpe + split) * epw), lds, st, *p, *d, mode, actions, mask, chunk, *gp, *gd, obs, reward, trunc, final_obs);
 }
 
 extern "C" void wg_launch_flow_env(const FlowP* p, const FlowPtrs* d, int mode, const float* actions, const uint8_t* mask,
@@ -958,3 +1050,4 @@
                                    float* obs, float* reward, uint8_t* trunc, float* final_obs, hipStream_t st) {
     env_launch(p, d, gd->multi_out ? 2 : 1, WG_MODE_STEP, actions, nullptr, 0, gp, gd, obs, reward, trunc, final_obs, st);
 }
+#endif
diff --git a/windgym_amd/csrc/wg_env4.hip b/windgym_amd/csrc/wg_env4.hip
--- /dev/null
+++ b/windgym_amd/csrc/wg_env4.hip
@@ -0,0 +1,2 @@
+#define WG_ENV_TU_EPW4
+#include "wg_env.hip"
diff --git a/windgym_amd/csrc/wg_env_common.h b/windgym_amd/csrc/wg_env_common.h
--- a/windgym_amd/csrc/wg_env_common.h
+++ b/windgym_amd/csrc/wg_env_common.h
@@ -134,6 +134,13 @@
     }
     return false;
 }
+__device__ __forceinline__ bool env_word_wait(unsigned* const f, const unsigned want) {
+    for (int n = 0; n < (1 << 22); ++n) {
+        if (__hip_atomic_load(f, __ATOMIC_RELAXED, __HIP_MEMORY_SCOPE_WORKGROUP) == want) { asm volatile("" ::: "memory"); return true; }
+        __builtin_amdgcn_s_sleep(2);
+    }
+    return false;
+}
 
 struct EnvFlowOut {
     int env_live, bg_init_pending;
@@ -152,13 +159,13 @@
 }
 
 template <int GLUE, int WPE>
-__device__ __forceinline__ void env_glue(const EnvKArgsPtr kg, LeanFused& fz, const float fp, const float bp, const int work,
+__device__ __forceinline__ void env_glue(const EnvKArgsPtr kg, const int e, LeanFused& fz, const float fp, const float bp, const int work,
                                          const EnvFlowOut& fo, const int hw) {
     fz.fp = fp; fz.bp = bp; fz.work = work;
     fz.bg_init_pending = WPE >= 2 ? 0 : fo.bg_init_pending;
     fz.plan_elsewhere = WPE >= 2;
     fz.hw = hw;
-    lean_step<GLUE == 2, false, true>(*(const WgParams*)&kg->gp, *(const WgPtrs*)&kg->gd, kg->d.gp, kg->d.gd, (int)blockIdx.x,
+    lean_step<GLUE == 2, false, true>(*(const WgParams*)&kg->gp, *(const WgPtrs*)&kg->gd, kg->d.gp, kg->d.gd, e,
                                       (int)(threadIdx.x & 63), kg->obs, kg->reward, kg->trunc, kg->final_obs, nullptr, fz);
 }
 
diff --git a/windgym_amd/csrc/wg_envb.hip b/windgym_amd/csrc/wg_envb.hip
--- a/windgym_amd/csrc/wg_envb.hip
+++ b/windgym_amd/csrc/wg_envb.hip
@@ -998,7 +998,7 @@
             }
             LeanFused fz;
             fz.pre = nullptr;
-            env_glue<GLUE, WPE>(kg, fz, fp, bp, work, fo, reinterpret_cast<const int*>(sm + LO::HDR)[threadIdx.x & 31]);
+            env_glue<GLUE, WPE>(kg, (int)blockIdx.x, fz, fp, bp, work, fo, reinterpret_cast<const int*>(sm + LO::HDR)[threadIdx.x & 31]);
         }
     }
 }
diff --git a/windgym_amd/csrc/wg_flow.h b/windgym_amd/csrc/wg_flow.h
--- a/windgym_amd/csrc/wg_flow.h
+++ b/windgym_amd/csrc/wg_flow.h
@@ -46,6 +46,7 @@
     int env_inc;
     float env_eps_max;
     float dt, D, inv_D, hub, dpart_f, R_rot, inv_N, inv_S, inv_P;
+    int env_epw;
     double dt_d, dpart, inv_dpart;
     float yaw_min, yaw_max, yaw_step;
     float ka, kb, eps0, hill, tia, tib, tic, tid;
@@ -103,6 +104,8 @@
 #define WG_ENV_FIXED_LDS_BYTES (3 * 64 * 16 + 2 * 64 * 8 + 4 * WG_ENV_SLOT_LDS_BYTES + 128)
 #define WG_ENV_CAP 256
 #define LEAN_PRE_BYTES 3584
+#define WG_ENV_SHARE_BYTES 64
+#define WG_ENV_RESIDENT4_LDS 39424
 #define WG_ENVB_FIXED_LDS_BYTES(nlp) ((93 + 48) * (nlp) + 4 * 208 + 128)
 #define WG_TURB_LDS_BYTES 120
 #define WG_GAT_BYTES (2 * 64 * 16 + 2 * 64 * 4)
diff --git a/windgym_amd/csrc/wg_plan.h b/windgym_amd/csrc/wg_plan.h
--- a/windgym_amd/csrc/wg_plan.h
+++ b/windgym_amd/csrc/wg_plan.h
@@ -16,6 +16,7 @@
 };
 struct WgHooks {
     WgHookInt flow_block, flow_res, flow_env, env_wpe, env_split, step_fused, sums, lds_pad, lf_cap, pstride_pad, step_graph;
+    WgHookInt env_epw;
     bool first_obs_gl_only = false, no_box8 = false, debug = false, timeline = false;
     std::string timeline_out;
 };
@@ -352,6 +353,13 @@
     return f.env_lds <= 32768 && f.env_lds <= lds_limit;
 }
 
+inline int wg_plan_env_epw(const WgHooks& hk, const WgParams& p, const FlowP& f, bool env_ok, size_t qf, int lds_limit) {
+    const size_t lds4 = (size_t)4 * f.env_lds + WG_ENV_SHARE_BYTES;
+    const bool can = env_ok && f.env_wpe == 1 && f.env_split == 0 && lds4 <= (size_t)lds_limit;
+    if (hk.env_epw.set) return (can && hk.env_epw.v == 4) ? 4 : 1;
+    return (can && p.B > 2048 && p.F == 2 && qf >= 256 && lds4 <= WG_ENV_RESIDENT4_LDS) ? 4 : 1;
+}
+
 inline void wg_plan_step_kernels(const wg_config* c, const WgHooks& hk, const WgParams& p, FlowP& f, bool small, int lds_limit) {
     const size_t qf = wg_plan_farm_quads(c, p);
     const bool env_ok = wg_plan_env(p, f, small, qf, lds_limit);
@@ -366,6 +374,7 @@
     const bool split_ok = env_ok && f.env_wpe == 2 && p.K == 1 && 4 * f.env_lds + 4096 <= lds_limit;
     f.env_split = (split_ok && p.B <= 1024 && qf >= 256) ? (p.B <= 512 ? 2 : 1) : 0;
     if (hk.env_split.set) f.env_split = (hk.env_split.v != 0 && split_ok && p.B <= 2048) ? (hk.env_split.v == 2 ? 2 : 1) : 0;
+    f.env_epw = wg_plan_env_epw(hk, p, f, env_ok && !envb_ok, qf, lds_limit);
     if (envb_ok) f.env_wpe = envb_wpe;
     const bool gen = p.turb_ti || p.farm_ti || p.farm_obs > 0 || (p.sum_mask_f | p.cur_mask_f) != 0;
     f.env_fused = (f.envw && p.sums_mode && !gen && p.power_avg <= 64) ? 1 : 0;
```

Result: faster. 84.06 million (median of 6 runs) (+1.6%).
